# indianajohn/akaze-rust

Hardware: AMD Instinct MI355X
Metric: Mpix/s through extract_features (4 oct x 4 sub) (higher is better)
Workload: dtype f32

## Files before the change

akaze-rust_amd/csrc/akz_extract.hpp:

```cpp
#pragma once
#include "akz_ctx.hpp"
#include "akz_frames.hpp"

struct akz_result {
    akz_ctx* ctx = nullptr;
    akz_config cfg;
    uint32_t w = 0, h = 0, n = 0, flags = 0;
    uint64_t big_px = 0;
    std::vector<LevelPlan> plan;
    void* slab = nullptr;
    size_t slab_bytes = 0;
    float* planes[kMaxLevels][10];
    double* d_k = nullptr;
    std::vector<double> k_host;
    std::vector<std::vector<akz_keypoint>> kps;
    std::vector<uint8_t> rows64;
    uint8_t* d_desc64 = nullptr;
    size_t desc_block_bytes = 0;
    std::vector<uint64_t> desc_off;
    std::vector<uint64_t> n_extrema;
};

struct MaskSpec {
    const uint8_t* d = nullptr;
    uint64_t row_pitch = 0, frame_stride = 0;
};

struct ResultDeleter {
    void operator()(akz_result* r) const;
};
struct akz_job {
    std::unique_ptr<akz_result, ResultDeleter> r;
    int slot = -1;
    uint32_t cap = 0;
    Event nms_done;
    uint64_t seq = 0;
    double t_begin_ms = 0.0;
    std::shared_ptr<Finisher> fin;
    bool finished = false;
    int rc = 0;
    akz_result* out = nullptr;
    std::string err;
    std::shared_ptr<std::atomic<int>> in_hand;
    bool alone_at_begin = true;
    hipStream_t done_stream = nullptr;
    MaskSpec mask;
    ~akz_job() {
        if (in_hand) --*in_hand;
    }
};

inline uint64_t shape_key(uint32_t w, uint32_t h, uint32_t n) { return ((uint64_t)w << 40) | ((uint64_t)h << 16) | n; }
inline uint32_t like_last_job(uint32_t last, uint32_t pad, uint32_t cap) { return std::min<uint32_t>(cap, last + last / 4 + pad); }

constexpr uint32_t kSelHdrWords = 16;
enum SelHdr : uint32_t {
    kSelHdrKeypoints = 0,
    kSelHdrExtrema = 1,
    kSelHdrFallback = 2,
    kSelHdrRounds = 3,
    kSelHdrTicks = 4,
    kSelHdrTotal = 8,
    kSelHdrFlags = 9,
    kSelHdrContrast = 10,
};
inline const uint32_t* sel_hdr(const akz_ctx* c, uint32_t img) { return (const uint32_t*)c->pin[PIN_SEL_HDR].p + (size_t)img * kSelHdrWords; }

inline LevelTable level_table(const akz_result* r) {
    LevelTable tab;
    std::memset(&tab, 0, sizeof(tab));
    for (size_t l = 0; l < r->plan.size(); ++l)
        tab.lv[l] = {r->planes[l][AKZ_LT], r->planes[l][AKZ_LX], r->planes[l][AKZ_LY], r->plan[l].w, r->plan[l].h, (uint64_t)r->plan[l].w * r->plan[l].h};
    return tab;
}
inline KpParam kp_param(float x, float y, float size, uint32_t octave, uint32_t level, uint32_t img) {
    const float ratio = (float)(1u << octave);
    return KpParam{x / ratio, y / ratio, std::round(0.5f * size / ratio), level, img, {0, 0, 0}};
}

inline size_t align_up(size_t v, size_t a) { return (v + a - 1) / a * a; }
AKZ_LOCAL int slab_acquire(akz_ctx* c, size_t bytes, void** p, size_t* got);
AKZ_LOCAL void slab_release(akz_ctx* c, void* p, size_t bytes);
AKZ_LOCAL void result_delete(akz_result* r);
AKZ_LOCAL void job_release(akz_job* j);
AKZ_LOCAL void job_wait(akz_job* j);
AKZ_LOCAL void job_destroy(akz_job* j);
struct JobOpening {
    std::unique_ptr<akz_job> job;
    int slot = -1;
    bool drain_side = false;
    bool laid_out = false;
    ~JobOpening();
    akz_job* keep(uint32_t cap);
};
AKZ_LOCAL int free_slot(const akz_ctx* c, int want = -1);
AKZ_LOCAL int job_open(akz_ctx* c, const char* who, int want_slot, uint32_t w, uint32_t h, uint32_t n, uint32_t flags, const akz_config& cfg,
                       JobOpening& o);
AKZ_LOCAL int job_layout(JobOpening& o, const std::vector<std::pair<uint32_t, int>>& wanted);
AKZ_LOCAL int place_lanes(akz_ctx* c);
template <typename T>
AKZ_LOCAL int extract_begin(akz_ctx* c, const T* d_imgs, uint32_t w, uint32_t h, uint32_t n, const akz_config* cfgp, uint32_t flags, akz_job** out,
                            int want_slot = -1, hipEvent_t input_ready = nullptr, bool sync_call = false, const MaskSpec* mask = nullptr);
AKZ_LOCAL int mask_enqueue(akz_ctx* c, hipStream_t s, const akz_result* r, const MaskSpec& m, int slot, uint32_t cap, uint32_t* d_count);
AKZ_LOCAL int extract_finish_body(akz_job* jobp, akz_result** out);
AKZ_LOCAL int extract_begin_frames(akz_ctx* c, const uint8_t* d_src, const FrameSpec& fs, uint32_t n, const akz_config* cfg, uint32_t flags, akz_job** out,
                                   const MaskSpec* mask = nullptr);
AKZ_LOCAL int extract_frames(akz_ctx* c, const uint8_t* d_src, const FrameSpec& fs, uint32_t n, const akz_config* cfg, uint32_t flags, akz_result** out,
                             const MaskSpec* mask = nullptr);
AKZ_LOCAL int frames_enqueue(akz_ctx* c, hipStream_t s, const uint8_t* d_src, const FrameSpec& fs, uint32_t n, uint8_t* d_luma);
```

akaze-rust_amd/csrc/akz_extract_finish.cpp:

```cpp
#include "akz_extract.hpp"

int device_libm_mode(akz_ctx* c) {
    if (c->settings.dbg_device_libm == 0) return 0;
    static std::mutex m;
    static int mode = -1;
    std::lock_guard<std::mutex> lk(m);
    if (mode >= 0) return mode;
    mode = 0;
#if defined(__x86_64__) && defined(__GLIBC__)
    __builtin_cpu_init();
    const bool fma = __builtin_cpu_supports("fma") && __builtin_cpu_supports("avx2");
    if (!fma && __builtin_cpu_supports("fma4")) return mode;
    constexpr size_t kN = 1u << 21;
    std::vector<float> a(kN), b(kN);
    uint64_t st = 0x9E3779B97F4A7C15ull;
    auto next = [&]() {
        uint64_t z = (st += 0x9E3779B97F4A7C15ull);
        z = (z ^ (z >> 30)) * 0xBF58476D1CE4E5B9ull;
        z = (z ^ (z >> 27)) * 0x94D049BB133111EBull;
        return z ^ (z >> 31);
    };
    const float special[] = {0.0f, -0.0f, 1.0f, -1.0f, INFINITY, -INFINITY, NAN, 0x1p-126f, -0x1p-126f, 0x1p-149f, 0x1.fffffep127f, 0x1p-12f,
                             0x1.921fb6p-1f, 0x1.921fb6p0f, 0x1.921fb6p1f, -0x1.921fb6p1f, 0.4375f, 0.6875f, 1.1875f, 2.4375f, 0x1p25f, 0x1p-29f,
                             119.99f, 120.0f, 1e10f};
// ... 16 lines not shown
            std::memcpy(&a[i], &u, 4);
            std::memcpy(&b[i], &v, 4);
        }
    }
    DevBuf d_a, d_b, d_o;
    std::vector<float> got(3 * kN);
    const bool ok_dev = d_a.acquire(kN * 4, false) == hipSuccess && d_b.acquire(kN * 4, false) == hipSuccess &&
                        d_o.acquire(3 * kN * 4, false) == hipSuccess &&
                        hipMemcpy(d_a.p, a.data(), kN * 4, hipMemcpyHostToDevice) == hipSuccess &&
                        hipMemcpy(d_b.p, b.data(), kN * 4, hipMemcpyHostToDevice) == hipSuccess;
    if (ok_dev) {
        launch::libm_eval(nullptr, (const float*)d_a.p, (const float*)d_b.p, (float*)d_o.p, kN, fma, nullptr);
        const bool ran = hipGetLastError() == hipSuccess && hipMemcpy(got.data(), d_o.p, 3 * kN * 4, hipMemcpyDeviceToHost) == hipSuccess;
        std::atomic<uint64_t> bad{ran ? 0u : 1u};
        if (ran) {
            const size_t pieces = 64;
            c->pool().run(pieces, [&](size_t p) {
                uint64_t mine = 0;
                auto bits = [](float f) { uint32_t u; std::memcpy(&u, &f, 4); return u; };
                auto same = [&](float x, float y) { return bits(x) == bits(y) || (x != x && y != y); };
                for (size_t i = kN * p / pieces; i < kN * (p + 1) / pieces; ++i) {
                    mine += !same(got[3 * i], atan2f(a[i], b[i]));
                    if (std::fabs(a[i]) < 119.9f) mine += !same(got[3 * i + 1], cosf(a[i])) + !same(got[3 * i + 2], sinf(a[i]));
                }
                bad += mine;
            });
        }
        if (bad.load() == 0) mode = fma ? 1 : 2;
    }
    (void)hipGetLastError();
#endif
    return mode;
}


namespace {
constexpr size_t kRelRow = (size_t)(kRel1 + kRel2) * sizeof(uint16_t);

struct FinishState {
    explicit FinishState(akz_job* j) : job(j), r(j->r.get()), c(r->ctx), n(r->n), s(c->stream), cap(j->cap), d_count((uint32_t*)c->count_slot[j->slot].p) {}
    akz_job* job;
    akz_result* r;
    akz_ctx* c;
    uint32_t n;
    hipStream_t s;
    uint32_t cap;
    uint32_t* d_count;
    bool waited_for = false, want_rel = false, want_dev = false, device_sort = false;
    uint64_t shape = 0;
    bool sorted = false, dev_sel = false;
    uint32_t mldb_spec = 0;
    int libm_dev = 0;
    bool dev_angles_ok = true;
    bool mirrored = false;
    uint16_t* d_rel = nullptr;
    uint32_t* d_rel_flags = nullptr;
    uint32_t *d_sel_hdr = nullptr, *d_sel_total = nullptr;
    std::vector<float> lsize, lratio;
    LevelTable tab;
    unsigned long long wmask = 0;
    uint32_t nwin = 0;
    const Candidate* hc = nullptr;
    uint32_t total_c = 0, spec_kp = 0;
    uint64_t total_kp = 0;
    double t_counts = 0.0;
    std::vector<std::vector<Candidate>> cands;
    std::vector<std::pair<const Candidate*, size_t>> span;
    std::vector<std::vector<HostKeypoint>> hk;
    bool host_rows() const { return !(r->flags & AKZ_NO_HOST_DESCRIPTORS); }
    const Candidate* d_unsorted() const { return (const Candidate*)(job->mask.d ? c->cand_mask_slot : c->cand_slot)[job->slot].p; }
    uint32_t mask_redone = 0;
};

int grow_pinned_keep(akz_ctx* c, DevBuf& buf, size_t keep_bytes, size_t want_bytes) {
    std::vector<uint8_t> keep;
    if (keep_bytes) keep.assign((const uint8_t*)buf.p, (const uint8_t*)buf.p + keep_bytes);
    AKZ_TRY(ensure_pinned(c, buf, want_bytes));
    if (keep_bytes) std::memcpy(buf.p, keep.data(), keep_bytes);
    return AKZ_OK;
}
int fetch_rest(akz_ctx* c, hipStream_t s, DevBuf& buf, const void* d_src, size_t elem, size_t have, size_t total) {
    AKZ_TRY(grow_pinned_keep(c, buf, have * elem, total * elem));
    AKZ_HIP_TRY(hipMemcpyAsync((uint8_t*)buf.p + have * elem, (const uint8_t*)d_src + have * elem, (total - have) * elem, hipMemcpyDeviceToHost, s));
    return AKZ_OK;
}
void rows_to_result(akz_ctx* c, akz_result* r, uint64_t total_kp) {
    const uint8_t* rows = (const uint8_t*)c->pin[PIN_ROWS].p;
    r->rows64.resize(total_kp * 64);
    const size_t kRowChunk = 8192;
    c->pool().run((total_kp + kRowChunk - 1) / kRowChunk, [&](size_t j) {
        const size_t b = j * kRowChunk * 64, e = std::min<size_t>(total_kp * 64, b + kRowChunk * 64);
        std::memcpy(r->rows64.data() + b, rows + b, e - b);
    });
}
int hold_behind_next_fed(akz_ctx* c, const akz_job* job, hipStream_t s) {
    const akz_result* r = job->r.get();
    if ((uint64_t)r->w * r->h * r->n >= r->big_px && c->begin_seq.load() > job->seq)
        AKZ_HIP_TRY(hipStreamWaitEvent(s, c->fed_ev[(job->seq + 1) % akz_ctx::kFedRing], 0));
    return AKZ_OK;
}

int choose_paths(FinishState& f) {
    akz_ctx* c = f.c;
    akz_job* job = f.job;
    akz_result* r = f.r;
    const uint32_t n = f.n;
    f.s = c->stream;
    const bool in_order = !c->is_lane && job->done_stream && job->alone_at_begin && job->in_hand && job->in_hand->load() == 1 && (c->settings.sched[SCHED_FINISH_FORM] & 2) == 0;
    if (in_order) {
        f.s = job->done_stream;
    } else if (!(c->is_lane && job->fin)) {
        AKZ_TRY(ensure_aux(c));
        f.s = c->aux;
    }
    AKZ_HIP_TRY(hipStreamWaitEvent(f.s, job->nms_done, 0));
    f.waited_for = !c->is_lane && job->alone_at_begin;
    f.want_rel = c->settings.dbg_select == 1 || (c->settings.dbg_select < 0 && (c->pool().size() < gates::kFewHostThreads || (uint64_t)r->w * r->h * n < r->big_px ||
                                                                (uint64_t)r->w * r->h >= gates::kSelectDevicePx || n < gates::kFewHostThreads || f.waited_for));
    f.shape = shape_key(r->w, r->h, n);
    bool skip_dev = false;
    if (c->sel_skip.load() > 0 && c->sel_skip_shape.load() == f.shape) {
        skip_dev = true;
        --c->sel_skip;
    }
    f.want_dev = c->settings.dbg_select == 2 || (c->settings.dbg_select < 0 && f.want_rel && !skip_dev && (c->pool().size() < gates::kFewHostThreads || f.waited_for));
    if (!f.want_dev) {
        c->sel_last_rounds = 0;
        c->sel_last_fallback = 0;
    }
    f.device_sort = c->settings.dbg_host_sort == 0 || (c->settings.dbg_host_sort < 0 && (c->pool().size() < gates::kFewHostThreads || f.want_rel)) || f.want_dev;
    selection_level_constants(r->plan, r->cfg, f.lsize, f.lratio);
    f.tab = level_table(r);
    orientation_windows(&f.wmask, &f.nwin);
    return AKZ_OK;
}

int enqueue_device_descriptors(FinishState& f) {
    akz_ctx* c = f.c;
    akz_result* r = f.r;
    f.libm_dev = device_libm_mode(c);
    if (!f.libm_dev) return AKZ_OK;
    void* blk = nullptr;
    AKZ_TRY(slab_acquire(c, (size_t)f.cap * 64, &blk, &r->desc_block_bytes));
    r->d_desc64 = (uint8_t*)blk;
    f.mldb_spec = like_last_job(c->last_total_kp.load(), 256u, f.cap);
    launch::MldbMirror mir{};
    if ((c->settings.sched[SCHED_FINISH_FORM] & 1) == 0) {
        AKZ_TRY(ensure_pinned(c, c->pin[PIN_SEL_HDR], (size_t)f.n * 64));
        AKZ_TRY(ensure_pinned(c, c->pin[PIN_LIST], (size_t)f.mldb_spec * sizeof(SelKpHost)));
        if (f.host_rows()) AKZ_TRY(ensure_pinned(c, c->pin[PIN_ROWS], (size_t)f.mldb_spec * 64));
        mir = launch::MldbMirror{c->pin[PIN_LIST].p, f.d_sel_hdr, c->pin[PIN_SEL_HDR].p, f.n * 64u, f.host_rows() ? (uint8_t*)c->pin[PIN_ROWS].p : nullptr};
        f.mirrored = true;
    }
    launch::mldb_counted(f.s, f.tab, (const KpParam*)c->kp_in.p, f.d_sel_total, 0, f.mldb_spec, &((SelKpHost*)c->sel_recs.p)->sums, 2,
                         f.libm_dev == 1, nullptr, (uint32_t)r->cfg.descriptor_channels, r->d_desc64, f.mirrored ? &mir : nullptr);
    AKZ_HIP_TRY(hipGetLastError());
    return AKZ_OK;
}

int enqueue_device_side(FinishState& f) {
    if (!f.device_sort) return AKZ_OK;
    akz_ctx* c = f.c;
    akz_result* r = f.r;
    hipStream_t s = f.s;
    const uint32_t n = f.n, cap = f.cap, L = (uint32_t)r->plan.size();
    const uint64_t max_px = (uint64_t)r->plan[0].w * r->plan[0].h;
    Candidate* d_sorted = nullptr;
    AKZ_TRY(ensure(c, c->cand_sorted, (size_t)cap * sizeof(Candidate)));
    d_sorted = (Candidate*)c->cand_sorted.p;
    void* selp = nullptr;
    if (f.want_dev) {
        AKZ_TRY(ensure(c, c->sel_scratch, launch::select_device_bytes(cap, n)));
        selp = c->sel_scratch.p;
    }
    std::vector<uint32_t> lw(L), lh(L);
    for (size_t l = 0; l < L; ++l) {
        lw[l] = r->plan[l].w;
        lh[l] = r->plan[l].h;
    }
    uint32_t* d_zero = selp ? launch::select_device_revcnt(selp, cap, n) : nullptr;
    const bool want_lists = f.want_rel || f.want_dev;
    if (want_lists) AKZ_TRY(ensure(c, c->rel_scratch, launch::candidate_relations_bytes(cap, lh.data(), L, n)));
    const bool rows_sort = n == 1 && (f.waited_for || c->settings.dbg_select == 2) &&
                           launch::sort_candidates_rows(s, f.d_unsorted(), cap, f.d_count, lw.data(), lh.data(), L, d_sorted, d_zero,
                                                        want_lists ? c->rel_scratch.p : nullptr);
    f.sorted = rows_sort;
    bool buckets_sort = false;
    if (!f.sorted) {
        AKZ_TRY(ensure(c, c->bucket_scratch, launch::sort_candidates_buckets_scratch(cap)));
        buckets_sort = launch::sort_candidates_buckets(s, f.d_unsorted(), cap, f.d_count, lw.data(), lh.data(), L, n, c->bucket_scratch.p,
                                                       &c->bucket_scratch.known, d_sorted, d_zero, want_lists ? c->rel_scratch.p : nullptr);
        f.sorted = buckets_sort;
    }
    if (!f.sorted) {
        AKZ_TRY(ensure(c, c->sort_scratch, launch::sort_candidates_scratch(cap, max_px, L, n)));
        f.sorted = launch::sort_candidates_device(s, f.d_unsorted(), cap, f.d_count, max_px, L, n, c->sort_scratch.p, d_sorted, d_zero);
    }
    if (f.sorted)
        kernel_row_count(c, kStageSort, rows_sort ? AKZ_KR_SORT_ROWS : (buckets_sort ? AKZ_KR_SORT_BUCKETS : AKZ_KR_SORT_RADIX), r->plan[0].w,
                         r->plan[0].h, n, rows_sort ? 1 : (buckets_sort ? 4 : 3), cap);
    AKZ_HIP_TRY(hipGetLastError());
    if (!f.sorted || !want_lists) return AKZ_OK;
    launch::candidate_relations(s, d_sorted, cap, f.d_count, f.lsize.data(), f.lratio.data(), lw.data(), lh.data(), L, n, c->rel_scratch.p,
                                &f.d_rel, &f.d_rel_flags, selp, rows_sort || buckets_sort);
    AKZ_HIP_TRY(hipGetLastError());
    if (!f.want_dev) return AKZ_OK;
    AKZ_TRY(ensure(c, c->sel_recs, (size_t)cap * sizeof(SelKpHost)));
    AKZ_TRY(ensure(c, c->kp_in, (size_t)cap * sizeof(KpParam)));
    launch::select_device(s, d_sorted, cap, f.d_count, f.lsize.data(), f.lratio.data(), lw.data(), lh.data(), L, n, c->rel_scratch.p, selp,
                          r->d_k, c->sel_recs.p, (KpParam*)c->kp_in.p, &f.d_sel_hdr, &f.d_sel_total);
    AKZ_TRY(hold_behind_next_fed(c, f.job, s));
    launch::orientation_counted(s, f.tab, (const KpParam*)c->kp_in.p, f.d_sel_total, cap, f.wmask, f.nwin, &((SelKpHost*)c->sel_recs.p)->sums, 2);
    AKZ_HIP_TRY(hipGetLastError());
    f.dev_sel = true;
    return enqueue_device_descriptors(f);
}

int adopt_device_selection(FinishState& f) {
    akz_ctx* c = f.c;
    akz_result* r = f.r;
    hipStream_t s = f.s;
    uint32_t max_rounds = 0, fallen = 0;
    for (uint32_t img = 0; img < f.n; ++img) {
        const uint32_t* hdr = sel_hdr(c, img);
        if (hdr[kSelHdrFallback] != 0) {
            f.dev_sel = false;
            ++fallen;
            fallen |= hdr[kSelHdrFallback] << 16;
        }
        f.total_kp += hdr[kSelHdrKeypoints];
        max_rounds = std::max(max_rounds, hdr[kSelHdrRounds]);
    }
    for (int k = 0; k < 4; ++k) c->sel_last_ticks[k] = sel_hdr(c, 0)[kSelHdrTicks + k];
    c->sel_last_rounds = max_rounds;
    c->sel_last_fallback = fallen;
    if (fallen) {
        c->sel_skip = 8;
        c->sel_skip_shape = f.shape;
    }
    if (f.dev_sel && f.libm_dev && f.total_kp > f.mldb_spec) {
        launch::mldb_counted(s, f.tab, (const KpParam*)c->kp_in.p, f.d_sel_total, f.mldb_spec, (uint32_t)f.total_kp, &((SelKpHost*)c->sel_recs.p)->sums, 2,
                             f.libm_dev == 1, nullptr, (uint32_t)r->cfg.descriptor_channels, r->d_desc64);
        AKZ_HIP_TRY(hipGetLastError());
    }
    if (f.dev_sel && f.total_kp > f.spec_kp) {
        AKZ_TRY(fetch_rest(c, s, c->pin[PIN_LIST], c->sel_recs.p, sizeof(SelKpHost), f.spec_kp, f.total_kp));
        if (f.libm_dev && f.host_rows()) AKZ_TRY(fetch_rest(c, s, c->pin[PIN_ROWS], r->d_desc64, 64, f.spec_kp, f.total_kp));
        AKZ_HIP_TRY(hipStreamSynchronize(s));
    }
    if (!f.dev_sel) f.total_kp = 0;
    return AKZ_OK;
}

int fetch_candidates(FinishState& f) {
    akz_ctx* c = f.c;
    akz_job* job = f.job;
    akz_result* r = f.r;
    hipStream_t s = f.s;
    const uint32_t n = f.n;
    const std::vector<LevelPlan>& plan = r->plan;
    for (int attempt = 0;; ++attempt) {
        const Candidate* d_list = f.sorted ? (const Candidate*)c->cand_sorted.p : f.d_unsorted();
        AKZ_TRY(ensure_pinned(c, c->pin[PIN_COUNT_SUMS], 256));
        uint32_t* total_p = (uint32_t*)c->pin[PIN_COUNT_SUMS].p;
        const bool dev_fetch = attempt == 0 && f.dev_sel;
        const bool masked = job->mask.d != nullptr;
        if (!dev_fetch) AKZ_HIP_TRY(hipMemcpyAsync(total_p, f.d_count, (masked ? 2 : 1) * sizeof(uint32_t), hipMemcpyDeviceToHost, s));
        else if (masked) AKZ_HIP_TRY(hipMemcpyAsync(total_p + 1, f.d_count + 1, sizeof(uint32_t), hipMemcpyDeviceToHost, s));
        uint32_t spec = 0;
        if (dev_fetch) {
            f.spec_kp = f.libm_dev ? f.mldb_spec : like_last_job(c->last_total_kp.load(), 256u, f.cap);
            if (!f.mirrored) {
                AKZ_TRY(ensure_pinned(c, c->pin[PIN_SEL_HDR], (size_t)n * 64));
                AKZ_HIP_TRY(hipMemcpyAsync(c->pin[PIN_SEL_HDR].p, f.d_sel_hdr, (size_t)n * 64, hipMemcpyDeviceToHost, s));
                AKZ_TRY(ensure_pinned(c, c->pin[PIN_LIST], (size_t)f.spec_kp * sizeof(SelKpHost)));
                AKZ_HIP_TRY(hipMemcpyAsync(c->pin[PIN_LIST].p, c->sel_recs.p, (size_t)f.spec_kp * sizeof(SelKpHost), hipMemcpyDeviceToHost, s));
                if (f.libm_dev && f.host_rows()) {
                    AKZ_TRY(ensure_pinned(c, c->pin[PIN_ROWS], (size_t)f.spec_kp * 64));
                    AKZ_HIP_TRY(hipMemcpyAsync(c->pin[PIN_ROWS].p, r->d_desc64, (size_t)f.spec_kp * 64, hipMemcpyDeviceToHost, s));
                }
            }
            AKZ_TRY(ensure_pinned(c, c->pin[PIN_CONTRAST], (size_t)n * sizeof(double)));
            AKZ_TRY(ensure_pinned(c, c->pin[PIN_REL_FLAGS], (size_t)n * sizeof(uint32_t)));
        } else if (attempt == 0) {
            spec = like_last_job(c->last_total_cands.load(), 64u, f.cap);
            if ((size_t)spec * sizeof(Candidate) > (1u << 20)) spec = 0;
            AKZ_TRY(ensure_pinned(c, c->pin[PIN_CONTRAST], (size_t)n * sizeof(double)));
            AKZ_HIP_TRY(hipMemcpyAsync(c->pin[PIN_CONTRAST].p, r->d_k, (size_t)n * sizeof(double), hipMemcpyDeviceToHost, s));
            if (spec) {
                AKZ_TRY(ensure_pinned(c, c->pin[PIN_LIST], (size_t)spec * sizeof(Candidate)));
                AKZ_HIP_TRY(hipMemcpyAsync(c->pin[PIN_LIST].p, d_list, (size_t)spec * sizeof(Candidate), hipMemcpyDeviceToHost, s));
                if (f.d_rel) {
                    AKZ_TRY(ensure_pinned(c, c->pin[PIN_REL], (size_t)spec * kRelRow));
                    AKZ_HIP_TRY(hipMemcpyAsync(c->pin[PIN_REL].p, f.d_rel, (size_t)spec * kRelRow, hipMemcpyDeviceToHost, s));
                }
            }
            if (f.d_rel) {
                AKZ_TRY(ensure_pinned(c, c->pin[PIN_REL_FLAGS], (size_t)n * sizeof(uint32_t)));
                AKZ_HIP_TRY(hipMemcpyAsync(c->pin[PIN_REL_FLAGS].p, f.d_rel_flags, (size_t)n * sizeof(uint32_t), hipMemcpyDeviceToHost, s));
            }
        }
        AKZ_HIP_TRY(hipStreamSynchronize(s));
        f.t_counts = now_ms();
        if (dev_fetch) {
            *total_p = sel_hdr(c, 0)[kSelHdrTotal];
            for (uint32_t img = 0; img < n; ++img) {
                ((uint32_t*)c->pin[PIN_REL_FLAGS].p)[img] = sel_hdr(c, img)[kSelHdrFlags];
                std::memcpy((double*)c->pin[PIN_CONTRAST].p + img, &sel_hdr(c, img)[kSelHdrContrast], sizeof(double));
            }
        }
        f.total_c = *total_p;
        if (attempt == 0) r->k_host.assign((const double*)c->pin[PIN_CONTRAST].p, (const double*)c->pin[PIN_CONTRAST].p + n);
        const uint32_t unfiltered = masked ? std::max(total_p[1], f.total_c) : f.total_c;
        c->last_total_cands = unfiltered;
        c->last_cand_shape = f.shape;
        c->cand_cap_hint = std::max(c->cand_cap_hint.load(), (uint32_t)((uint64_t)unfiltered * 5 / 4 / n) + 64u);
        if (masked) {
            static std::atomic<uint64_t> stamp{0};
            c->mask_last[0] = unfiltered, c->mask_last[1] = f.total_c, c->mask_last[2] = f.mask_redone;
            c->mask_stamp = ++stamp;
        }
        if (f.total_c > f.cap) {
            if (attempt >= 3) {
                set_error("NMS candidate buffer overflow");
                return AKZ_ERR_OVERFLOW;
            }
            f.cap = f.total_c + f.total_c / 8;
            f.sorted = false;
            f.dev_sel = false;
            f.d_rel = nullptr;
            AKZ_HIP_TRY(hipStreamSynchronize(c->stream));
            AKZ_TRY(ensure(c, c->cand_slot[job->slot], (size_t)f.cap * sizeof(Candidate)));
            if (masked) AKZ_TRY(ensure(c, c->cand_mask_slot[job->slot], (size_t)f.cap * sizeof(Candidate)));
            AKZ_HIP_TRY(hipMemsetAsync(f.d_count, 0, sizeof(uint32_t), s));
            for (size_t l = 0; l < plan.size(); ++l)
                launch::nms(s, r->planes[l][AKZ_LDET], plan[l].w, plan[l].h, n, (uint64_t)plan[l].w * plan[l].h, (uint32_t)l,
                            (float)r->cfg.detector_threshold, border_margin(plan[l], r->cfg), (Candidate*)c->cand_slot[job->slot].p, f.cap, f.d_count);
            AKZ_HIP_TRY(hipGetLastError());
            if (masked) {
                AKZ_TRY(mask_enqueue(c, s, r, job->mask, job->slot, f.cap, f.d_count));
                ++f.mask_redone;
            }
            continue;
        }
        if (f.dev_sel) {
            AKZ_TRY(adopt_device_selection(f));
            if (f.dev_sel) return AKZ_OK;
        }
        const uint32_t have = std::min(spec, f.total_c);
        if (f.total_c > have) {
            AKZ_TRY(fetch_rest(c, s, c->pin[PIN_LIST], d_list, sizeof(Candidate), have, f.total_c));
            if (f.d_rel) AKZ_TRY(fetch_rest(c, s, c->pin[PIN_REL], f.d_rel, kRelRow, have, f.total_c));
            AKZ_HIP_TRY(hipStreamSynchronize(s));
        }
        AKZ_TRY(ensure_pinned(c, c->pin[PIN_LIST], sizeof(Candidate)));
        f.hc = (const Candidate*)c->pin[PIN_LIST].p;
        return AKZ_OK;
    }
}

void candidates_per_image(FinishState& f) {
    akz_ctx* c = f.c;
    const uint32_t n = f.n, total_c = f.total_c;
    const Candidate* hc = f.hc;
    f.span.assign(n, {nullptr, 0});
    if (f.dev_sel) {
    } else if (f.sorted) {
        size_t at = 0;
        for (uint32_t img = 0; img < n; ++img) {
            const Candidate* b = hc + at;
            const Candidate* e = std::partition_point(b, hc + total_c, [&](const Candidate& x) { return x.img <= img; });
            f.span[img] = {b, (size_t)(e - b)};
            at += (size_t)(e - b);
        }
    } else {
        f.cands.resize(n);
        const unsigned slices = (unsigned)std::min<size_t>((size_t)total_c / 16384 + 1, (size_t)c->pool().size());
        std::vector<std::vector<uint32_t>> at(slices, std::vector<uint32_t>(n, 0));
        auto slice_range = [&](unsigned t, size_t* b, size_t* e) {
            *b = (size_t)total_c * t / slices;
            *e = (size_t)total_c * (t + 1) / slices;
        };
        auto run_slices = [&](auto&& fn) { c->pool().run(slices, [&](size_t t) { fn((unsigned)t); }); };
        run_slices([&](unsigned t) {
            size_t b, e;
            slice_range(t, &b, &e);
            for (size_t i = b; i < e; ++i)
                if (hc[i].img < n) at[t][hc[i].img]++;
        });
        for (uint32_t img = 0; img < n; ++img) {
            uint32_t run = 0;
            for (unsigned t = 0; t < slices; ++t) {
                const uint32_t cnt = at[t][img];
                at[t][img] = run;
                run += cnt;
            }
            f.cands[img].resize(run);
        }
        run_slices([&](unsigned t) {
            size_t b, e;
            slice_range(t, &b, &e);
            for (size_t i = b; i < e; ++i)
                if (hc[i].img < n) f.cands[hc[i].img][at[t][hc[i].img]++] = hc[i];
        });
    }
    c->sel_last_mode = f.dev_sel ? 2 : (f.d_rel && f.sorted ? 1 : 0);
    c->slot_busy[f.job->slot] = false;
    f.job->slot = -1;
    if (c->settings.profiling) c->prof.ms[AKZ_ST_NMS] += now_ms() - f.t_counts;
}

void select_keypoints_stage(FinishState& f) {
    akz_ctx* c = f.c;
    akz_result* r = f.r;
    const uint32_t n = f.n;
    const std::vector<LevelPlan>& plan = r->plan;
    const double t_host0 = now_ms();
    f.hk.resize(n);
    r->n_extrema.assign(n, 0);
    r->desc_off.assign(n + 1, 0);
    if (f.dev_sel) {
        const SelKpHost* recs = (const SelKpHost*)c->pin[PIN_LIST].p;
        std::vector<uint64_t> first(n + 1, 0);
        for (uint32_t img = 0; img < n; ++img) first[img + 1] = first[img] + sel_hdr(c, img)[kSelHdrKeypoints];
        c->pool().run(n, [&](size_t img) {
            r->n_extrema[img] = sel_hdr(c, (uint32_t)img)[kSelHdrExtrema];
            f.hk[img].resize(sel_hdr(c, (uint32_t)img)[kSelHdrKeypoints]);
            for (size_t i = 0; i < f.hk[img].size(); ++i) {
                const sel::KpRec& q = recs[first[img] + i].rec;
                HostKeypoint& k = f.hk[img][i];
                k.x = q.x; k.y = q.y; k.response = q.response;
                k.size = f.lsize[q.level];
                k.octave = plan[q.level].octave;
                k.class_id = q.level;
                k.angle = 0.0f;
                if (f.libm_dev) std::memcpy(&k.angle, &recs[first[img] + i].sums.angle_bits, 4);
                k.lx = k.ly = 0;
                k.xp = k.xm = k.yp = k.ym = 0.0f;
            }
        });
        if (f.libm_dev)
            for (uint32_t img = 0; img < n && f.dev_angles_ok; ++img)
                for (const HostKeypoint& k : f.hk[img])
                    if (!(std::fabs(k.angle) < 119.9f)) {
                        f.dev_angles_ok = false;
                        break;
                    }
        c->last_total_kp = (uint32_t)f.total_kp;
    } else {
        c->pool().run(n, [&](size_t img) {
            if (!f.sorted) {
                sort_candidates(f.cands[img], plan);
                f.span[img] = {f.cands[img].data(), f.cands[img].size()};
            }
            if (f.d_rel && f.sorted && (((const uint32_t*)c->pin[PIN_REL_FLAGS].p)[img] & 1u) == 0)
                select_keypoints_rel(f.span[img].first, f.span[img].second, (const uint16_t*)c->pin[PIN_REL].p + (size_t)(f.span[img].first - f.hc) * (kRel1 + kRel2),
                                     kRel1, kRel2, plan, r->cfg, f.hk[img], &r->n_extrema[img]);
            else
                select_keypoints(f.span[img].first, f.span[img].second, plan, r->cfg, f.hk[img], &r->n_extrema[img]);
        });
    }
    f.total_kp = 0;
    for (uint32_t img = 0; img < n; ++img) {
        r->desc_off[img] = f.total_kp;
        f.total_kp += f.hk[img].size();
    }
    r->desc_off[n] = f.total_kp;
    if (c->settings.profiling) c->prof.ms[AKZ_ST_HOST_KP] += now_ms() - t_host0;
}

int describe_with_host_libm(FinishState& f, const KpParam* params) {
    akz_ctx* c = f.c;
    akz_result* r = f.r;
    hipStream_t s = f.s;
    const uint64_t total_kp = f.total_kp;
    const double t_or0 = now_ms();
    KpParam* d_kp = (KpParam*)c->kp_in.p;
    OrientOut* oo = nullptr;
    size_t oo_stride = 1;
    AKZ_TRY(ensure(c, c->cosi, total_kp * 2 * sizeof(float)));
    if (f.dev_sel) {
        oo = &((SelKpHost*)c->pin[PIN_LIST].p)->sums;
        oo_stride = 2;
    } else {
        AKZ_TRY(ensure(c, c->kp_in, total_kp * sizeof(KpParam)));
        AKZ_TRY(ensure(c, c->kp_out, total_kp * sizeof(OrientOut)));
        AKZ_TRY(ensure_pinned(c, c->pin[PIN_COUNT_SUMS], total_kp * std::max(sizeof(OrientOut), 2 * sizeof(float))));
        d_kp = (KpParam*)c->kp_in.p;
        OrientOut* d_oo = (OrientOut*)c->kp_out.p;
        AKZ_HIP_TRY(hipMemcpyAsync(d_kp, params, total_kp * sizeof(KpParam), hipMemcpyHostToDevice, s));
        AKZ_TRY(hold_behind_next_fed(c, f.job, s));
        launch::orientation(s, f.tab, d_kp, (uint32_t)total_kp, f.wmask, f.nwin, d_oo);
        AKZ_HIP_TRY(hipGetLastError());
        oo = (OrientOut*)c->pin[PIN_COUNT_SUMS].p;
        AKZ_HIP_TRY(hipMemcpyAsync(oo, d_oo, total_kp * sizeof(OrientOut), hipMemcpyDeviceToHost, s));
        AKZ_HIP_TRY(hipStreamSynchronize(s));
    }
    AKZ_TRY(ensure_pinned(c, c->pin[PIN_COSI], total_kp * 2 * sizeof(float)));
    float* cosi = (float*)c->pin[PIN_COSI].p;
    std::vector<float> angles(total_kp);
    const size_t kAngleChunk = 4096;
    c->pool().run((total_kp + kAngleChunk - 1) / kAngleChunk, [&](size_t j) {
        const size_t b = j * kAngleChunk, e = std::min<size_t>(total_kp, b + kAngleChunk);
        for (size_t g = b; g < e; ++g) {
            const OrientOut& og = oo[g * oo_stride];
            const float ang = og.found ? atan2f(og.sum_y, og.sum_x) : 0.0f;
            angles[g] = ang;
            cosi[2 * g] = cosf(ang);
            cosi[2 * g + 1] = sinf(ang);
        }
    });
    c->pool().run(f.n, [&](size_t img) {
        for (size_t i = 0; i < f.hk[img].size(); ++i) f.hk[img][i].angle = angles[r->desc_off[img] + i];
    });
    AKZ_HIP_TRY(hipMemcpyAsync(c->cosi.p, cosi, total_kp * 2 * sizeof(float), hipMemcpyHostToDevice, s));
    const double t_ml0 = now_ms();
    if (c->settings.profiling) c->prof.ms[AKZ_ST_ORIENT] += t_ml0 - t_or0;
    if (r->d_desc64 && r->desc_block_bytes < total_kp * 64) {
        slab_release(c, r->d_desc64, r->desc_block_bytes);
        r->d_desc64 = nullptr;
    }
    if (!r->d_desc64) {
        void* blk = nullptr;
        AKZ_TRY(slab_acquire(c, total_kp * 64, &blk, &r->desc_block_bytes));
        r->d_desc64 = (uint8_t*)blk;
    }
    launch::mldb(s, f.tab, d_kp, (const float*)c->cosi.p, (uint32_t)total_kp, (uint32_t)r->cfg.descriptor_channels, r->d_desc64);
    AKZ_HIP_TRY(hipGetLastError());
    if (f.host_rows()) {
        AKZ_TRY(ensure_pinned(c, c->pin[PIN_ROWS], total_kp * 64));
        AKZ_HIP_TRY(hipMemcpyAsync(c->pin[PIN_ROWS].p, r->d_desc64, total_kp * 64, hipMemcpyDeviceToHost, s));
        AKZ_HIP_TRY(hipStreamSynchronize(s));
        rows_to_result(c, r, total_kp);
    } else {
        AKZ_HIP_TRY(hipStreamSynchronize(s));
    }
    if (c->settings.profiling) c->prof.ms[AKZ_ST_MLDB] += now_ms() - t_ml0;
    return AKZ_OK;
}

int describe(FinishState& f) {
    akz_ctx* c = f.c;
    akz_result* r = f.r;
    KpParam* params = nullptr;
    if (!f.dev_sel) {
        AKZ_TRY(ensure_pinned(c, c->pin[PIN_PARAMS], std::max<size_t>(1, f.total_kp) * sizeof(KpParam)));
        params = (KpParam*)c->pin[PIN_PARAMS].p;
        c->pool().run(f.n, [&](size_t img) {
            for (size_t i = 0; i < f.hk[img].size(); ++i) {
                const HostKeypoint& k = f.hk[img][i];
                params[r->desc_off[img] + i] = kp_param(k.x, k.y, k.size, k.octave, k.class_id, (uint32_t)img);
            }
        });
    }
    r->kps.assign(f.n, {});
    const bool dev_desc = f.dev_sel && f.libm_dev != 0 && f.dev_angles_ok;
    c->libm_last = dev_desc ? f.libm_dev : 0;
    if (f.total_kp && dev_desc) {
        const double t_ml0 = now_ms();
        if (f.host_rows()) rows_to_result(c, r, f.total_kp);
        if (c->settings.profiling) c->prof.ms[AKZ_ST_MLDB] += now_ms() - t_ml0;
    } else if (f.total_kp) {
        AKZ_TRY(describe_with_host_libm(f, params));
    }
    return AKZ_OK;
}

void publish(FinishState& f) {
    akz_ctx* c = f.c;
    akz_result* r = f.r;
    c->pool().run(f.n, [&](size_t img) {
        r->kps[img].resize(f.hk[img].size());
        for (size_t i = 0; i < f.hk[img].size(); ++i) {
            const HostKeypoint& k = f.hk[img][i];
            r->kps[img][i] = akz_keypoint{k.x, k.y, k.response, k.size, k.octave, k.class_id, k.angle, 0};
        }
    });
    if (c->settings.profiling) {
        resolve_spans(c);
        c->prof.ms[AKZ_ST_TOTAL] += now_ms() - f.job->t_begin_ms;
        c->prof.calls += 1;
        c->prof.pixels += (uint64_t)r->w * r->h * f.n;
    }
    ev_put(c, std::move(f.job->nms_done));
}
}

int extract_finish_body(akz_job* jobp, akz_result** out) {
    *out = nullptr;
    std::unique_ptr<akz_job, void (*)(akz_job*)> job(jobp, job_release);
    AKZ_TRY(bind(job->r->ctx, false));
    FinishState f(jobp);
    AKZ_TRY(choose_paths(f));
    AKZ_TRY(enqueue_device_side(f));
    AKZ_TRY(fetch_candidates(f));
    candidates_per_image(f);
    select_keypoints_stage(f);
    AKZ_TRY(describe(f));
    publish(f);
    *out = job->r.release();
    (void)job.release();
    return AKZ_OK;
}
```

akaze-rust_amd/csrc/akz_internal.hpp:

```cpp
#pragma once
#include <hip/hip_runtime.h>

#include <cstdint>
#include <functional>
#include <string>
#include <vector>

#include "../../include/akaze_hip.h"
#include "../../include/akaze_hip_debug.h"

namespace akz {

void set_error(const std::string& msg);
unsigned host_cpu_share();

using TrialsOnDevice = std::function<int(const float*, const float*, const float*, const float*, uint32_t, const uint32_t*, uint32_t,
                                         float, float, float*, int32_t*)>;
int remove_outliers_impl(const akz_keypoint* keypoints_0, uint64_t n0, const akz_keypoint* keypoints_1, uint64_t n1,
                         const akz_match* matches, uint64_t n_matches, uint64_t num_trials, float epsilon_model,
                         float epsilon_inlier, akz_match* out, uint64_t* n_out, const TrialsOnDevice& trials_on_device);

#define AKZ_HIP_TRY(expr)                                                                          \
    do {                                                                                           \
        hipError_t _e = (expr);                                                                    \
        if (_e != hipSuccess) {                                                                    \
            ::akz::set_error(std::string(#expr) + " failed: " + hipGetErrorString(_e));            \
            return AKZ_ERR_HIP;                                                                    \
        }                                                                                          \
    } while (0)

struct DefaultSource {
    uint64_t s0 = 42, s1 = 69;
    uint64_t next() {
        uint64_t x = s0;
        const uint64_t y = s1;
        s0 = y;
        x ^= x << 23;
        x ^= x >> 17;
        x ^= y ^ (y >> 26);
        s1 = x;
        return x + y;
    }
};
DefaultSource& default_source();
template <int K, class T>
void draw_samples(DefaultSource& src, uint64_t n_matches, uint64_t trials, T* out);

int refuse_bad_matches(const char* name, const akz_keypoint* keypoints_0, uint64_t n0, const akz_keypoint* keypoints_1, uint64_t n1,
                       const akz_match* matches, uint64_t n_matches, const akz_match* out, const uint64_t* n_out);
struct MatchPoints {
    std::vector<float> v;
    const float *x0, *y0, *x1, *y1;
    MatchPoints(const akz_keypoint* keypoints_0, const akz_keypoint* keypoints_1, const akz_match* matches, uint64_t n) : v((size_t)n * 4) {
        float* p = v.data();
        x0 = p; y0 = p + n; x1 = p + 2 * n; y1 = p + 3 * n;
        for (uint64_t i = 0; i < n; ++i) {
            p[i] = keypoints_0[matches[i].index_0].x; p[n + i] = keypoints_0[matches[i].index_0].y;
            p[2 * n + i] = keypoints_1[matches[i].index_1].x; p[3 * n + i] = keypoints_1[matches[i].index_1].y;
        }
    }
};


#define AKZ_TRY(expr)            \
    do {                         \
        int _s = (expr);         \
        if (_s != AKZ_OK) return _s; \
    } while (0)

int match_sets_at(akz_ctx* c, const uint8_t* d_q, uint64_t n0, const uint8_t* d_rows, const uint64_t* set_first,
                  const uint64_t* set_rows, uint64_t n_sets, uint64_t distance_threshold, double lowes_ratio, akz_match* d_out,
                  uint64_t* d_n_out, akz_match* d_out_cols, uint64_t* d_n_cols, int side = 0);
hipStream_t match_side_stream(akz_ctx* c);

int place_streams_beside(akz_ctx* c, hipStream_t* slots, int n_slots, int* still_shared);
enum { kPlaceQueue = 1, kPlacePipe = 2, kPlaceAmbiguous = 4 };
int placement_verdict(float spin_pair_ms, float tiny_pair_ms, float tiny_alone_ms, float spin_ms);

struct LevelPlan {
    double etime = 0, esigma = 0;
    uint32_t octave = 0, sublevel = 0, sigma_size = 0;
    uint32_t w = 0, h = 0;
    uint32_t det_sigma = 0;
    std::vector<double> tau;
};
int config_validate(const akz_config& c);
int fed_tau_by_process_time(double T, int M, double tau_max, bool reordering, std::vector<double>& tau);
std::vector<float> gaussian_kernel(float sigma, size_t kernel_size);
size_t gaussian_kernel_size(float sigma);
void scharr_kernels(uint32_t scale, std::vector<float>& main_axis, std::vector<float>& off_axis);
int build_plan(uint32_t w, uint32_t h, const akz_config& cfg, std::vector<LevelPlan>& plan);

constexpr int kMaxTaps = 13;
struct Taps {
    int n = 0;
    int hw = 0;
    int off[kMaxTaps] = {0};
    float wgt[kMaxTaps] = {0};
};
int taps_from_dense(const float* k, uint32_t ntaps, Taps& t);
Taps taps_scharr_main(uint32_t scale);
Taps taps_scharr_off(uint32_t scale);

struct Candidate {
    uint32_t level;
    uint32_t idx;
    float v, xp, xm, yp, ym;
    uint32_t img;
};
struct KpParam {
    float xf, yf;
    float scale;
    uint32_t level;
    uint32_t img;
    uint32_t _pad[3];
};
struct OrientOut {
    float sum_x, sum_y;
    uint32_t found;
    uint32_t angle_bits;
};
struct MatchRec {
    uint32_t min_d, second_d, min_j, _pad;
};
struct LevelPtrs {
    const float* lt;
    const float* lx;
    const float* ly;
    uint32_t w, h;
    uint64_t stride;
};
constexpr int kMaxLevels = 64;
constexpr int kRel1 = 12, kRel2 = 6;
struct LevelTable {
    LevelPtrs lv[kMaxLevels];
};

namespace launch {
void filter_h_f32(hipStream_t s, const float* in, float* out, uint32_t w, uint32_t h, uint32_t n, const Taps& t);
void filter_h_u8(hipStream_t s, const uint8_t* in, float* out, uint32_t w, uint32_t h, uint32_t n, const Taps& t);
void filter_v_f32(hipStream_t s, const float* in, float* out, uint32_t w, uint32_t h, uint32_t n, const Taps& t);
void delay(hipStream_t s, uint32_t microseconds);
void half_size(hipStream_t s, const float* in, float* out, uint32_t w, uint32_t h, uint32_t n);
void pm_g2(hipStream_t s, const float* lx, const float* ly, float* out, uint32_t w, uint32_t h, uint32_t n,
           const double* d_k, uint32_t k_scale_pow);
void flow(hipStream_t s, const float* lsmooth, float* lflow, uint32_t w, uint32_t h, uint32_t n, const double* d_k,
          uint32_t k_scale_pow);
void fed_step(hipStream_t s, const float* lt_in, const float* lflow, float* lt_out, float* lstep, uint32_t w,
              uint32_t h, uint32_t n, float half_tau);
struct FedNextPrep {
    float* lsmooth;
    float* lflow;
    const float* g3;
    const double* d_k;
    uint32_t k_pow;
};
bool fed_epilogue_supported(uint32_t w, uint32_t h, uint32_t n_steps);
void fed_fused(hipStream_t s, const float* lt_in, const float* lflow, float* lt_out, float* lstep, uint32_t w, uint32_t h,
               uint32_t n, const float* half_taus, uint32_t n_steps, const FedNextPrep* next = nullptr);
uint64_t fed_deep_workgroups(uint32_t w, uint32_t h, uint32_t n);
void contrast_max(hipStream_t s, const float* blurred, uint32_t w, uint32_t h, uint32_t n,
                  unsigned long long* d_hmax_bits);
void contrast_hist(hipStream_t s, const float* blurred, uint32_t w, uint32_t h, uint32_t n,
                   const unsigned long long* d_hmax_bits, uint32_t nbins, uint32_t* d_hist);
void contrast_final(hipStream_t s, const unsigned long long* d_hmax_bits, const uint32_t* d_hist, uint32_t nbins,
                    double percentile, uint32_t n, double* d_k);
bool blur_fused_supported(uint32_t ntaps);
void blur_fused_f32(hipStream_t s, const float* in, float* out, uint32_t w, uint32_t h, uint32_t n, const float* k,
                    uint32_t ntaps);
void blur_fused_u8(hipStream_t s, const uint8_t* in, float* out, uint32_t w, uint32_t h, uint32_t n, const float* k,
                   uint32_t ntaps);
void prep_fused(hipStream_t s, const float* prev, bool half, float* lt_out, float* lsmooth, float* lflow, uint32_t w,
                uint32_t h, uint32_t pw, uint32_t ph, uint32_t n, const float* g3, const double* d_k, uint32_t k_pow);
bool detector_fused_supported(uint32_t sigma);
void detector_fused(hipStream_t s, const float* lsmooth, uint32_t sigma, float* lx, float* ly, float* lxx, float* lyy,
                    float* lxy, float* ldet_out, uint32_t w, uint32_t h, uint32_t n);
bool detector_tiled_fused_supported(uint32_t sigma);
struct DetLevelDesc {
    const float* lsmooth;
    float *lx, *ly, *lxx, *lyy, *lxy, *ldet;
    uint32_t w, h, level;
    float border_m;
};
uint32_t detector_tiled_set_max();
void detector_tiled_set(hipStream_t s, uint32_t sigma, const DetLevelDesc* levels, uint32_t nlevels, uint32_t n, float thr,
                        Candidate* d_cand, uint32_t cap, uint32_t* d_count);
void detector_tiled_fused(hipStream_t s, const float* lsmooth, uint32_t sigma, float* lx, float* ly, float* lxx,
                          float* lyy, float* lxy, float* ldet_out, uint32_t w, uint32_t h, uint32_t n, uint32_t level,
                          float thr, float border_m, Candidate* d_cand, uint32_t cap, uint32_t* d_count);
bool blur5_stream_supported(uint32_t w, uint32_t h, uint32_t ntaps, bool is_u8);
void blur5_stream_u8(hipStream_t s, const uint8_t* in, float* out, uint32_t w, uint32_t h, uint32_t n, const float* k);
void blur5_stream_f32(hipStream_t s, const float* in, float* out, uint32_t w, uint32_t h, uint32_t n, const float* k);
uint32_t march_band_rows(int kind, uint32_t w, uint32_t h, uint32_t n, int S, int32_t* cs_ce, uint32_t cap);
bool blur5_march_supported(uint32_t w, uint32_t h, uint32_t ntaps);
void blur5_march_u8(hipStream_t s, const uint8_t* in, float* out, uint32_t w, uint32_t h, uint32_t n, const float* k);
void blur5_march_f32(hipStream_t s, const float* in, float* out, uint32_t w, uint32_t h, uint32_t n, const float* k);
bool contrast_march_supported(uint32_t w, uint32_t h, uint32_t ntaps, uint32_t nbins);
void contrast_march(hipStream_t s, const float* in, uint32_t w, uint32_t h, uint32_t n, const float* g3,
                    unsigned long long* d_hmax_bits, uint32_t nbins, uint32_t* d_hist, double* d_thr);
void contrast_thresholds(hipStream_t s, const unsigned long long* d_hmax_bits, uint32_t nbins, uint32_t n, double* d_thr);
bool contrast_stream_supported(uint32_t w, uint32_t h, uint32_t ntaps, uint32_t nbins);
void contrast_stream(hipStream_t s, const float* in, uint32_t w, uint32_t h, uint32_t n, const float* g3,
                     unsigned long long* d_hmax_bits, uint32_t nbins, uint32_t* d_hist, double* d_thr);
bool prep_stream_supported(uint32_t w, uint32_t h);
void prep_stream(hipStream_t s, const float* prev, bool half, float* lt_out, float* lsmooth, float* lflow, uint32_t w,
                 uint32_t h, uint32_t pw, uint32_t ph, uint32_t n, const float* g3, const double* d_k, uint32_t k_pow);
bool detector_march_supported(uint32_t sigma, uint32_t w, uint32_t h, float border_m, bool nms);
void detector_march(hipStream_t s, const float* lsmooth, uint32_t sigma, float* lx, float* ly, float* lxx, float* lyy,
                    float* lxy, float* ldet_out, uint32_t w, uint32_t h, uint32_t n, uint32_t level, float thr,
                    float border_m, Candidate* d_cand, uint32_t cap, uint32_t* d_count);
uint32_t detector_march_set_max();
void detector_march_set(hipStream_t s, uint32_t sigma, const DetLevelDesc* levels, uint32_t nlevels, uint32_t n, float thr,
                        Candidate* d_cand, uint32_t cap, uint32_t* d_count);
void detector_set_waves(int waves);
uint32_t detector_set_cells(int S, const uint32_t* w, const uint32_t* h, uint32_t nlv, uint32_t n, int32_t* cells, uint32_t cap,
                            int32_t* grids);
bool head_fused_supported(uint32_t w, uint32_t h, uint32_t ntaps0, uint32_t ntaps1);
void head_fused_u8(hipStream_t s, const uint8_t* in, float* lt0, float* blurred, float* gx, float* gy, uint32_t w, uint32_t h, uint32_t n,
                   const float* k5, const float* g3, unsigned long long* d_smax_bits, uint32_t* d_zero_word = nullptr);
void head_fused_f32(hipStream_t s, const float* in, float* lt0, float* blurred, float* gx, float* gy, uint32_t w, uint32_t h, uint32_t n,
                    const float* k5, const float* g3, unsigned long long* d_smax_bits, uint32_t* d_zero_word = nullptr);
void contrast_hist_final(hipStream_t s, const float* gx, const float* gy, uint32_t w, uint32_t h, uint32_t n, unsigned long long* d_smax_bits,
                         uint32_t nbins, uint32_t* d_hist, uint32_t* d_done, double percentile, double* d_k);
void flow_from_pair(hipStream_t s, const float* gx, const float* gy, float* lflow, uint32_t w, uint32_t h, uint32_t n, const double* d_k,
                    uint32_t k_pow);
void march_min_band_rows(int detector, int level);
bool level_march_supported(uint32_t w, uint32_t h);
bool level_march_half_supported(uint32_t w, uint32_t h, uint32_t pw, uint32_t ph, uint32_t n_steps);
void level_march(hipStream_t s, const float* prev, float* lsmooth, float* lflow, float* lt_out, float* lstep, uint32_t w,
                 uint32_t h, uint32_t n, const float* g3, const double* d_k, uint32_t k_pow, const float* half_taus,
                 uint32_t n_steps, uint32_t pw = 0, uint32_t ph = 0);
struct ResidentLevel {
    float *lt, *lsmooth, *lflow, *lstep;
    uint32_t w, h;
    bool half;
    uint32_t n_tau;
    const float* half_tau;
    uint32_t k_pow;
};
constexpr int kResidentMaxLevels = 10;
constexpr int kResidentMaxSteps = 448;
bool octave_resident_supported(uint32_t w, uint32_t h);
void octave_resident(hipStream_t s, const float* prev, uint32_t pw, uint32_t ph, uint32_t n, const ResidentLevel* levels,
                     uint32_t n_levels, const float* g3, const double* d_k);
bool detector_nms_fused_supported(uint32_t sigma);
void detector_nms_fused(hipStream_t s, const float* lsmooth, uint32_t sigma, float* lx, float* ly, float* lxx,
                        float* lyy, float* lxy, float* ldet_out, uint32_t w, uint32_t h, uint32_t n, uint32_t level,
                        float thr, float border_m, Candidate* d_cand, uint32_t cap, uint32_t* d_count);
void rcp_f64_to_f32(hipStream_t s, const double* x, float* out, uint64_t n);
void accumulate(hipStream_t s, float* a, const float* b, uint64_t count);
void ldet(hipStream_t s, const float* lxx, const float* lyy, const float* lxy, float* out, uint64_t count,
          float sigma_quat);
size_t sort_candidates_scratch(uint32_t cap, uint64_t max_px, uint32_t n_levels, uint32_t n_images);
uint32_t sort_small_capacity();
size_t sort_candidates_buckets_scratch(uint32_t cap);
size_t sort_candidates_buckets_counters();
bool sort_candidates_buckets(hipStream_t s, const Candidate* d_cand, uint32_t cap, const uint32_t* d_count, const uint32_t* level_w,
                             const uint32_t* level_h, uint32_t n_levels, uint32_t n_images, void* scratch, size_t* counters_zero,
                             Candidate* d_sorted, uint32_t* d_zero, void* rel_scratch);
bool sort_candidates_rows(hipStream_t s, const Candidate* d_cand, uint32_t cap, const uint32_t* d_count, const uint32_t* level_w,
                          const uint32_t* level_h, uint32_t n_levels, Candidate* d_sorted, uint32_t* d_zero, void* rel_scratch);
bool sort_candidates_device(hipStream_t s, const Candidate* d_cand, uint32_t cap, const uint32_t* d_count, uint64_t max_px,
                            uint32_t n_levels, uint32_t n_images, void* scratch, Candidate* d_sorted, uint32_t* d_zero = nullptr);
size_t candidate_relations_bytes(uint32_t cap, const uint32_t* level_h, uint32_t n_levels, uint32_t n_images);
void candidate_relations(hipStream_t s, const Candidate* d_sorted, uint32_t cap, const uint32_t* d_count, const float* size, const float* ratio,
                         const uint32_t* level_w, const uint32_t* level_h, uint32_t n_levels, uint32_t n_images, void* scratch,
                         uint16_t** d_rel_out, uint32_t** d_flags_out, void* sel_scratch = nullptr, bool tables_ready = false);
size_t select_device_bytes(uint32_t cap, uint32_t n_images);
uint32_t* select_device_revcnt(void* sel_scratch, uint32_t cap, uint32_t n_images);
void select_device(hipStream_t s, const Candidate* d_sorted, uint32_t cap, const uint32_t* d_count, const float* size, const float* ratio,
                   const uint32_t* level_w, const uint32_t* level_h, uint32_t n_levels, uint32_t n_images, const void* rel_scratch,
                   void* sel_scratch, const double* d_k, void* d_recs, KpParam* d_pars, uint32_t** d_hdr_out, uint32_t** d_total_out);
void nms(hipStream_t s, const float* ldet, uint32_t w, uint32_t h, uint32_t n, uint64_t img_stride, uint32_t level,
         float thr, float border_m, Candidate* d_cand, uint32_t cap, uint32_t* d_count);
void mask_candidates(hipStream_t s, const Candidate* d_in, Candidate* d_out, uint32_t cap, uint32_t* d_cnt, const uint8_t* d_mask,
                     uint64_t row_pitch, uint64_t frame_stride, const uint32_t* level_w, const uint32_t* level_h,
                     const uint32_t* level_octave, uint32_t n_levels, uint32_t n_images);
void orientation(hipStream_t s, const LevelTable& lt, const KpParam* d_kp, uint32_t nkp,
                 unsigned long long window_mask, uint32_t n_windows, OrientOut* d_out);
void orientation_counted(hipStream_t s, const LevelTable& lt, const KpParam* d_kp, const uint32_t* d_nkp, uint32_t max_kp,
                         unsigned long long window_mask, uint32_t n_windows, OrientOut* d_out, uint32_t out_stride);
void mldb(hipStream_t s, const LevelTable& lt, const KpParam* d_kp, const float* d_cosi, uint32_t nkp,
          uint32_t channels, uint8_t* d_desc64);
struct MldbMirror {
    void* host_recs;
    const void* d_hdr;
    void* host_hdr;
    uint32_t hdr_bytes;
    uint8_t* host_desc;
};
void mldb_counted(hipStream_t s, const LevelTable& lt, const KpParam* d_kp, const uint32_t* d_nkp, uint32_t first, uint32_t last, OrientOut* d_sums,
                  uint32_t sums_stride, bool libm_fma, uint32_t* d_flag, uint32_t channels, uint8_t* d_desc64, const MldbMirror* mirror = nullptr);
void libm_eval(hipStream_t s, const float* a, const float* b, float* out3, uint64_t n, bool fma, uint32_t* d_flag);
uint32_t match_num_chunks(uint32_t n0, uint32_t n1);
void match(hipStream_t s, const uint8_t* d0, uint32_t n0, const uint8_t* d1, uint32_t n1, uint32_t threshold,
           bool rows_le_61, uint32_t chunks, MatchRec* d_rec);
uint32_t match_mfma_rows(uint32_t n, bool queries);
uint32_t match_mfma_chunks(uint32_t n0, uint32_t n1, uint32_t forced = 0);
uint32_t match_mfma_multi_chunks(uint32_t n0, uint32_t n_sets, uint32_t avg_tiles, uint32_t forced = 0);
void unpack_bits(hipStream_t s, const uint8_t* d, uint32_t n, uint32_t n_pad, bool query, uint8_t* out8, uint32_t* pop,
                 uint32_t* bound, uint32_t threshold, uint32_t n_bound, const uint32_t* d_tiles, bool fp4 = false);
void ransac_trials(hipStream_t s, const float* d_pts, uint32_t n_matches, const uint32_t* d_samples, uint32_t trials, float epsilon_model,
                   float epsilon_inlier, float* d_models, int32_t* d_inliers);
struct PairJobHost {
    uint64_t raw_off, kp0_off, kp1_off, trial_off, keep_off, n_trials;
    uint32_t cnt_idx, pad;
};
static_assert(sizeof(PairJobHost) == 56, "the device reads 56-byte pair records");
enum class RansacModel { Fundamental, Homography, FundamentalNormalised };
void pair_points(hipStream_t s, const PairJobHost* d_pairs, uint32_t n_pairs, const void* d_raw, const uint64_t* d_raw_cnt,
                 const float* d_kx, const float* d_ky, float* d_pts, uint64_t pts_stride);
void pairs_trials(hipStream_t s, RansacModel model, const PairJobHost* d_pairs, const uint32_t* d_trials, uint64_t first_trial,
                  uint32_t n_trials, const uint64_t* d_raw_cnt, const float* d_pts, uint64_t pts_stride, float epsilon_model,
                  float epsilon_inlier, float* d_models, int32_t* d_inliers);
void pairs_pick_filter(hipStream_t s, RansacModel model, const PairJobHost* d_pairs, uint32_t n_pairs, const void* d_raw,
                       const uint64_t* d_raw_cnt, const float* d_pts, uint64_t pts_stride, const float* d_models, const int32_t* d_inliers,
                       float epsilon_inlier, void* d_keep, uint64_t* d_keep_cnt, float* d_h, int32_t* d_found);
void model_refit(hipStream_t s, RansacModel model, const PairJobHost* d_pairs, uint32_t n_pairs, const void* d_raw, const uint64_t* d_raw_cnt,
                      const float* d_pts, uint64_t pts_stride, float epsilon_model, float epsilon_inlier, uint32_t max_iterations,
                      void* d_keep, uint64_t* d_keep_cnt, float* d_h, const int32_t* d_found, uint32_t* d_iterations);
void pairs_pose(hipStream_t s, const PairJobHost* d_pairs, uint32_t n_pairs, const akz_camera* d_cameras,
                const float* d_kx, const float* d_ky, const float* d_f, const int32_t* d_found, void* d_keep, uint64_t* d_keep_cnt,
                akz_pose* d_poses, float* d_points);
void seeded_round(hipStream_t s, RansacModel model, const PairJobHost* d_pairs, uint32_t n_pairs, const uint32_t* d_done, uint64_t k1,
                  uint64_t stream_base, uint32_t round, uint32_t max_trials, const uint64_t* d_raw_cnt, const float* d_pts, uint64_t pts_stride,
                  float epsilon_model, float epsilon_inlier, float* d_ring_mdl, int32_t* d_ring_inl);
void seeded_update(hipStream_t s, uint32_t n_pairs, uint32_t round, uint32_t max_trials, const uint32_t* d_need, uint32_t need_stride,
                   uint32_t need_index, const float* d_ring_mdl, const int32_t* d_ring_inl, uint32_t* d_done, int32_t* d_best_inl, float* d_best_mdl,
                   uint32_t* d_trials_run, uint32_t* d_running);
void unpack_pair(hipStream_t s, const uint8_t* dq, uint32_t nq, uint32_t q_pad, uint8_t* outq, uint32_t* popq, uint32_t* bound, uint32_t threshold,
                 const uint8_t* dt, uint32_t nt, uint32_t t_pad, uint8_t* outt, uint32_t* popt, bool fp4);
uint32_t match_mfma_tile_rows();
uint32_t match_mfma_query_block();
struct MatchChunkHost {
    uint32_t t_begin, t_end, row0, n_rows, bound_off, record;
};
void match_mfma_multi(hipStream_t s, const uint8_t* q8, const uint32_t* qpop, uint32_t n0, const uint8_t* t8,
                      const void* d_table, uint32_t n_chunks, uint32_t threshold, uint32_t* bound, MatchRec* d_out, bool fp4 = false);
void match_mfma(hipStream_t s, const uint8_t* q8, const uint32_t* qpop, uint32_t n0, const uint8_t* t8, uint32_t n1,
                uint32_t threshold, uint32_t* bound, uint32_t chunks, MatchRec* d_rec, bool fp4 = false);
struct MatchColSetHost {
    uint32_t row0, rows, out0;
};
uint32_t match_cols_seed_rows(uint32_t n0);
void match_cols_seed(hipStream_t s, const uint8_t* q4, uint32_t n0, const uint8_t* t4, uint32_t t_rows, uint32_t threshold,
                     uint32_t* d_bound, MatchRec* d_seed, unsigned long long* cbest, uint32_t* csecond);
void match_fp4_multi_mutual(hipStream_t s, const uint8_t* q4, uint32_t n0, const uint8_t* t4, const void* d_table, uint32_t n_chunks,
                            uint32_t threshold, uint32_t* bound, MatchRec* d_out, unsigned long long* cbest, uint32_t* csecond);
void match_compact_cols(hipStream_t s, const unsigned long long* cbest, const uint32_t* csecond, const void* d_sets, uint32_t n_sets,
                        uint32_t threshold, double ratio2, akz_match* d_out, unsigned long long* d_n_out);
void match_compact_sets(hipStream_t s, const MatchRec* d_rec, uint32_t n0, uint32_t n_sets, uint32_t chunks, uint32_t threshold,
                        double ratio2, akz_match* d_out, unsigned long long* d_n_out);
void match_compact(hipStream_t s, const MatchRec* d_rec, uint32_t n0, uint32_t chunks, uint32_t threshold, double ratio2,
                   akz_match* d_out, unsigned long long* d_n_out);
void match_merge(hipStream_t s, const MatchRec* d_part, uint32_t n0, uint32_t chunks, uint32_t threshold, MatchRec* d_out);
size_t match_merge_compact_state_bytes(uint32_t n0);
void match_merge_compact(hipStream_t s, const MatchRec* d_part, uint32_t n0, uint32_t chunks, uint32_t threshold, double ratio2,
                         akz_match* d_out, unsigned long long* d_n_out, void* d_state, uint32_t epoch);
struct GuidedPairHost {
    uint64_t rec_off;
    uint32_t q_row0, n0, t_row0, n1, wg0, chunks, chunk_rows, model;
};
uint32_t match_guided_block();
void match_guided(hipStream_t s, int kind, const uint8_t* d_rows, const float* d_kx, const float* d_ky, const GuidedPairHost* d_tab,
                  uint32_t n_tab, uint32_t n_workgroups, const float* d_models, const int32_t* d_found, float radius,
                  uint32_t threshold, MatchRec* d_rec);
struct CrossJobHost {
    uint64_t fwd_off, rev_off;
    uint32_t fwd_cnt_idx, rev_cnt_idx, fwd_cap, rev_cap;
};
static_assert(sizeof(CrossJobHost) == 32, "the device reads 32-byte cross records");
void pairs_cross_filter(hipStream_t s, const CrossJobHost* d_tab, uint32_t n_pairs, akz_match* d_fwd, uint64_t* d_fwd_cnt,
                        const akz_match* d_rev, const uint64_t* d_rev_cnt);
void pair_cross_filter(hipStream_t s, const CrossJobHost& job, akz_match* d_fwd, uint64_t* d_fwd_cnt, const akz_match* d_rev,
                       const uint64_t* d_rev_cnt);
struct BankSeg {
    const uint8_t* src_rows;
    uint64_t n_rows, dst_row0;
};
static_assert(sizeof(BankSeg) == 24, "the device reads 24-byte segment records");
constexpr uint64_t kBankMaxRows = 0x7fffffffull * 64;
void bank_gather(hipStream_t s, const BankSeg* d_tab, uint32_t n_seg, uint64_t total_rows, uint32_t desc_bytes, uint8_t* d_dst);
uint32_t knn_list_len(uint32_t k);
uint32_t knn_chunks(uint32_t n0, uint32_t n1, uint32_t forced = 0);
size_t knn_part_bytes(uint32_t n0, uint32_t chunks, uint32_t k);
bool knn(hipStream_t s, const uint8_t* q4, uint32_t n0, const uint8_t* t4, uint32_t n1, uint32_t threshold, uint32_t chunks, uint32_t k,
         uint32_t* d_part, akz_match* d_out, uint32_t* d_counts);
struct BudgetSet {
    uint32_t base, n, keep, out_off;
};
struct BudgetBlock {
    uint32_t set, q0, t0, t1;
};
static_assert(sizeof(BudgetSet) == 16 && sizeof(BudgetBlock) == 16, "the device reads 16-byte budget records");
uint32_t budget_query_tile();
uint32_t budget_train_tile();
void budget(hipStream_t s, bool spread, float robust, const float* d_x, const float* d_y, const float* d_r, uint32_t total,
            const BudgetSet* d_sets, uint32_t n_sets, const BudgetBlock* d_blocks, uint32_t n_blocks, float* d_radius2, uint32_t* d_rank,
            uint32_t* d_idx);
}

struct HostKeypoint {
    float x, y, response, size;
    uint32_t octave, class_id;
    float angle;
    uint32_t lx, ly;
    float xp, xm, yp, ym;
};
void sort_candidates(std::vector<Candidate>& cands, const std::vector<LevelPlan>& plan);
void select_keypoints(const Candidate* cands_sorted, size_t n_cands, const std::vector<LevelPlan>& plan,
                      const akz_config& cfg, std::vector<HostKeypoint>& out, uint64_t* n_extrema);
void select_keypoints_rel(const Candidate* cands_sorted, size_t n_cands, const uint16_t* rel, int k1, int k2, const std::vector<LevelPlan>& plan,
                          const akz_config& cfg, std::vector<HostKeypoint>& out, uint64_t* n_extrema);
void selection_level_constants(const std::vector<LevelPlan>& plan, const akz_config& cfg, std::vector<float>& size, std::vector<float>& ratio);
void orientation_windows(unsigned long long* mask, uint32_t* n_windows);
float border_margin(const LevelPlan& lv, const akz_config& cfg);

}

#if defined(__HIPCC__)
namespace akz {
typedef float akz_f4a __attribute__((ext_vector_type(4)));
typedef float akz_f4u __attribute__((ext_vector_type(4), aligned(4)));
__device__ __forceinline__ void plane_store(float* p, float v) { *p = v; }
__device__ __forceinline__ void plane_store4(float* p, float a, float b, float c, float d) {
    const akz_f4a t = {a, b, c, d};
    *reinterpret_cast<akz_f4a*>(p) = t;
}
__device__ __forceinline__ void plane_store4u(float* p, akz_f4a t) {
    *reinterpret_cast<akz_f4u*>(p) = t;
}
}
#endif
```

akaze-rust_amd/csrc/akz_kernels.hip:

```cpp
#include <hip/hip_runtime.h>

#include <algorithm>
#include <cstdlib>

#include "akz_internal.hpp"
#include "akz_pm_g2.hpp"
#include "akz_libm.hpp"
#include "akz_prep_passes.hpp"

namespace akz {
namespace {

constexpr int BX = 64, BY = 4;

__device__ __forceinline__ int clampi(int v, int lo, int hi) { return v < lo ? lo : (v > hi ? hi : v); }

__device__ __forceinline__ float px(const float* p, long i) { return p[i]; }
__device__ __forceinline__ float px(const uint8_t* p, long i) { return ((float)p[i] * 1.0f) / 255.0f; }

template <typename T>
__global__ void k_filter_h(const T* __restrict__ in, float* __restrict__ out, int w, int h, Taps t) {
    const int x = blockIdx.x * BX + threadIdx.x, y = blockIdx.y * BY + threadIdx.y;
    if (x >= w || y >= h) return;
    const size_t base = (size_t)blockIdx.z * (size_t)w * (size_t)h;
// ... 469 lines not shown
            const float4 a = *reinterpret_cast<const float4*>(GX + i0), b = *reinterpret_cast<const float4*>(GY + i0);
            ax[0] = a.x; ax[1] = a.y; ax[2] = a.z; ax[3] = a.w;
            ay[0] = b.x; ay[1] = b.y; ay[2] = b.z; ay[3] = b.w;
        } else {
#pragma unroll
            for (int e = 0; e < 4; ++e) {
                ax[e] = i0 + e < px ? GX[i0 + e] : 0.0f;
                ay[e] = i0 + e < px ? GY[i0 + e] : 0.0f;
            }
        }
        int y = (int)(i0 / (size_t)w), x = (int)(i0 - (size_t)y * w);
#pragma unroll
        for (int e = 0; e < 4; ++e) {
            if (x >= 1 && x < w - 1 && y >= 1 && y < h - 1) {
                const double dx = (double)ax[e], dy = (double)ay[e];
                const double g = sqrt(dx * dx + dy * dy);
                if (g != 0.0) {
                    const double f = floor((double)nbins * (g / hmax));
                    const unsigned b = f >= (double)nbins ? nbins - 1u : (f > 0.0 ? (unsigned)f : 0u);
                    atomicAdd(&mine[b], 1u);
                }
            }
            if (++x == w) {
                x = 0;
                ++y;
            }
        }
    }
    __syncthreads();
    unsigned* hist = d_hist + (size_t)img * nbins;
    for (unsigned b = tid; b < nbins; b += NTH) {
        unsigned v = 0;
        for (unsigned c = 0; c < copies; ++c) v += s_hist[c * nbins + b];
        if (v) {
            const unsigned before = atomicAdd(&hist[b], v);
            asm volatile("" ::"v"(before));
        }
    }
    __builtin_amdgcn_fence(__ATOMIC_RELEASE, "workgroup");
    __builtin_amdgcn_s_waitcnt(0);
    __syncthreads();
    if (tid == 0) s_last = atomicAdd(&d_done[img], 1u) == gridDim.x - 1u ? 1u : 0u;
    __syncthreads();
    if (!s_last) return;
    for (unsigned b = tid; b < nbins; b += NTH) {
        s_hist[b] = __hip_atomic_load(&hist[b], __ATOMIC_RELAXED, __HIP_MEMORY_SCOPE_AGENT);
        hist[b] = 0u;
    }
    __syncthreads();
    if (tid != 0) return;
    unsigned long long num_points = 0;
    for (unsigned b = 0; b < nbins; ++b) num_points += s_hist[b];
    const unsigned long long threshold = sat_usize((double)num_points * percentile);
    unsigned long long k = 0, num_elements = 0;
    while (num_elements < threshold && k < nbins) {
        num_elements += s_hist[k];
        k += 1;
    }
    d_k[img] = num_elements >= threshold ? hmax * (double)k / (double)nbins : 0.03;
    d_smax_bits[img] = 0ull;
    d_done[img] = 0u;
}
__global__ void __launch_bounds__(256)
k_flow_pair(const float* __restrict__ gxp, const float* __restrict__ gyp, float* __restrict__ lflow, size_t px, const double* __restrict__ d_k,
            unsigned k_pow) {
    const unsigned img = blockIdx.z;
    const double kc = octave_contrast(d_k[img], k_pow);
    const double inverse_k = 1.0 / (kc * kc);
    const float* GX = gxp + (size_t)img * px;
    const float* GY = gyp + (size_t)img * px;
    float* out = lflow + (size_t)img * px;
    const size_t i0 = ((size_t)blockIdx.x * 256 + threadIdx.x) * 4;
    if (i0 >= px) return;
    if ((px & 3u) == 0) {
        const float4 a = *reinterpret_cast<const float4*>(GX + i0), b = *reinterpret_cast<const float4*>(GY + i0);
        float4 o;
        o.x = pm_g2_px(a.x, b.x, inverse_k);
        o.y = pm_g2_px(a.y, b.y, inverse_k);
        o.z = pm_g2_px(a.z, b.z, inverse_k);
        o.w = pm_g2_px(a.w, b.w, inverse_k);
        *reinterpret_cast<float4*>(out + i0) = o;
    } else {
        for (size_t i = i0; i < i0 + 4 && i < px; ++i) out[i] = pm_g2_px(GX[i], GY[i], inverse_k);
    }
}

__global__ void k_ldet(const float* __restrict__ lxx, const float* __restrict__ lyy, const float* __restrict__ lxy,
                       float* __restrict__ out, size_t count, float q) {
    const size_t i = (size_t)blockIdx.x * blockDim.x + threadIdx.x;
    if (i >= count) return;
    out[i] = ((lxx[i] * lyy[i]) - (lxy[i] * lxy[i])) * q;
}

__global__ void k_accumulate(float* a, const float* b, size_t count) {
    const size_t i = (size_t)blockIdx.x * blockDim.x + threadIdx.x;
    if (i >= count) return;
    a[i] = a[i] + b[i];
}

__device__ __forceinline__ void nms_emit(float v, float xp, float xm, float yp, float ym, int x, int y, int w, int h,
                                         unsigned level, unsigned img, float thr, float border_m,
                                         Candidate* __restrict__ cand, unsigned cap, unsigned* __restrict__ count) {
    if (!(v > thr)) return;
    if (!(v > xp && v > xm && v > ym && v > yp)) return;
    const float fx = (float)x, fy = (float)y;
    const bool is_out = (roundf(fx - border_m) - 1.0f) < 0.0f || (roundf(fx + border_m) + 1.0f) >= (float)w ||
                        (roundf(fy - border_m) - 1.0f) < 0.0f || (roundf(fy + border_m) + 1.0f) >= (float)h;
    if (is_out) return;
    const unsigned slot = atomicAdd(count, 1u);
    if (slot < cap) {
        Candidate c;
        c.level = level;
        c.idx = (unsigned)(y * w + x);
        c.v = v; c.xp = xp; c.xm = xm; c.yp = yp; c.ym = ym;
        c.img = img;
        cand[slot] = c;
    }
}
__global__ void k_nms(const float* __restrict__ ldet, int w, int h, size_t img_stride, unsigned level, float thr,
                      float border_m, Candidate* __restrict__ cand, unsigned cap, unsigned* __restrict__ count) {
    const int x0 = (blockIdx.x * BX + threadIdx.x) * 4, y = blockIdx.y * BY + threadIdx.y;
    if (x0 >= w || y < 1 || y >= h - 1) return;
    const float* D = ldet + (size_t)blockIdx.z * img_stride;
    const float* row = D + (size_t)y * w;
    float c[6], up[4], dn[4];
    if ((w & 3) == 0 && x0 + 3 < w) {
        const float4 vc = *reinterpret_cast<const float4*>(row + x0);
        const float4 vu = *reinterpret_cast<const float4*>(row - w + x0);
        const float4 vd = *reinterpret_cast<const float4*>(row + w + x0);
        c[1] = vc.x; c[2] = vc.y; c[3] = vc.z; c[4] = vc.w;
        up[0] = vu.x; up[1] = vu.y; up[2] = vu.z; up[3] = vu.w;
        dn[0] = vd.x; dn[1] = vd.y; dn[2] = vd.z; dn[3] = vd.w;
    } else {
#pragma unroll
        for (int e = 0; e < 4; ++e) {
            const bool in = x0 + e < w;
            c[e + 1] = in ? row[x0 + e] : 0.0f;
            up[e] = in ? row[x0 + e - w] : 0.0f;
            dn[e] = in ? row[x0 + e + w] : 0.0f;
        }
    }
    c[0] = x0 > 0 ? row[x0 - 1] : 0.0f;
    c[5] = (x0 + 4 < w) ? row[x0 + 4] : 0.0f;
    const long last = (long)w * h - w - 1;
#pragma unroll
    for (int e = 0; e < 4; ++e) {
        const int x = x0 + e;
        if (x < 1 || x >= w) continue;
        if ((long)y * w + x >= last) continue;
        nms_emit(c[e + 1], c[e + 2], c[e], dn[e], up[e], x, y, w, h, level, blockIdx.z, thr, border_m, cand, cap, count);
    }
}

__constant__ float c_gauss25[7][7] = {
    {0.02546481f, 0.02350698f, 0.01849125f, 0.01239505f, 0.00708017f, 0.00344629f, 0.00142946f},
    {0.02350698f, 0.02169968f, 0.01706957f, 0.01144208f, 0.00653582f, 0.00318132f, 0.00131956f},
    {0.01849125f, 0.01706957f, 0.01342740f, 0.00900066f, 0.00514126f, 0.00250252f, 0.00103800f},
    {0.01239505f, 0.01144208f, 0.00900066f, 0.00603332f, 0.00344629f, 0.00167749f, 0.00069579f},
    {0.00708017f, 0.00653582f, 0.00514126f, 0.00344629f, 0.00196855f, 0.00095820f, 0.00039744f},
    {0.00344629f, 0.00318132f, 0.00250252f, 0.00167749f, 0.00095820f, 0.00046640f, 0.00019346f},
    {0.00142946f, 0.00131956f, 0.00103800f, 0.00069579f, 0.00039744f, 0.00019346f, 0.00008024f}};

struct OriTable {
    signed char a[112], b[112];
};
constexpr OriTable make_ori_table() {
    OriTable t{};
    int idx = 0;
    for (int i = -6; i <= 6; ++i)
        for (int j = -6; j <= 6; ++j)
            if (i * i + j * j < 36) {
                t.a[idx] = (signed char)i;
                t.b[idx] = (signed char)j;
                ++idx;
            }
    for (; idx < 112; ++idx) { t.a[idx] = 0; t.b[idx] = 0; }
    return t;
}
__constant__ OriTable c_ori = make_ori_table();
struct OriOrder {
    unsigned char k[112];
};
constexpr OriOrder make_ori_order() {
    OriOrder o{};
    const OriTable t = make_ori_table();
    int n = 0;
    for (int b = -6; b <= 6; ++b)
        for (int a = -6; a <= 6; ++a)
            for (int k = 0; k < 109; ++k)
                if (t.a[k] == a && t.b[k] == b) o.k[n++] = (unsigned char)k;
    for (; n < 112; ++n) o.k[n] = 0;
    return o;
}
__constant__ OriOrder c_ori_rows = make_ori_order();

__device__ __forceinline__ unsigned xcd_contiguous_group(unsigned b, unsigned nb) {
    return (b & 7u) * (nb >> 3) + (b >> 3);
}

constexpr int ORI_KPB = 32, ORI_NS = 109, ORI_NT = 256;
__global__ void __launch_bounds__(ORI_NT)
k_orientation(LevelTable tab, const KpParam* __restrict__ kps, unsigned nkp, const unsigned* __restrict__ d_nkp,
              unsigned long long window_mask, unsigned n_windows, OrientOut* __restrict__ out, unsigned out_stride) {
    __shared__ float s_rx[ORI_KPB * ORI_NS];
    __shared__ float s_ry[ORI_KPB * ORI_NS + 16];
    if (d_nkp) nkp = min(nkp, *d_nkp);
    const unsigned base = xcd_contiguous_group(blockIdx.x, gridDim.x) * ORI_KPB;
    if (base >= nkp) return;
    constexpr int ORI_IT = (ORI_KPB * ORI_NS + ORI_NT - 1) / ORI_NT, ORI_UB = 7;
    static_assert(ORI_IT % ORI_UB == 0, "whole batches");
    for (int it0 = 0; it0 < ORI_IT; it0 += ORI_UB) {
        float vx[ORI_UB], vy[ORI_UB], gw[ORI_UB];
        unsigned slot[ORI_UB];
#pragma unroll
        for (int u = 0; u < ORI_UB; ++u) {
            const unsigned idx = threadIdx.x + (unsigned)(it0 + u) * ORI_NT;
            const unsigned j = idx / ORI_NS, k = c_ori_rows.k[idx - j * ORI_NS];
            vx[u] = 0.0f; vy[u] = 0.0f; gw[u] = 0.0f;
            slot[u] = j * ORI_NS + k;
            if (idx < ORI_KPB * ORI_NS && base + j < nkp) {
                const KpParam kp = kps[base + j];
                const LevelPtrs lv = tab.lv[kp.level];
                const float* lx = lv.lx + (size_t)kp.img * lv.stride;
                const float* ly = lv.ly + (size_t)kp.img * lv.stride;
                const int a = c_ori.a[k], b = c_ori.b[k];
                const float fy = roundf(kp.yf + (float)b * kp.scale);
                const float fx = roundf(kp.xf + (float)a * kp.scale);
                const int iy = clampi(fy > 0.0f ? (int)fy : 0, 0, (int)lv.h - 1);
                const int ix = clampi(fx > 0.0f ? (int)fx : 0, 0, (int)lv.w - 1);
                gw[u] = c_gauss25[a < 0 ? -a : a][b < 0 ? -b : b];
                const size_t p = (size_t)iy * lv.w + ix;
                vx[u] = lx[p];
                vy[u] = ly[p];
            }
        }
#pragma unroll
        for (int u = 0; u < ORI_UB; ++u) {
            const unsigned idx = threadIdx.x + (unsigned)(it0 + u) * ORI_NT;
            const unsigned j = idx / ORI_NS;
            if (idx < ORI_KPB * ORI_NS) {
                const bool have = base + j < nkp;
                s_rx[slot[u]] = have ? gw[u] * vx[u] : 0.0f;
                s_ry[slot[u]] = have ? gw[u] * vy[u] : 0.0f;
            }
        }
    }
    __syncthreads();
    if (threadIdx.x >= 64) return;
    const unsigned lane = threadIdx.x, j = lane >> 1;
    const bool is_y = (lane & 1u) != 0;
    const float* py = s_ry + j * ORI_NS;
    const float* pa = is_y ? py : s_rx + j * ORI_NS;
    float t[ORI_NS];
#pragma unroll
    for (int k = 0; k < ORI_NS; ++k) t[k] = py[k] > 0.0f ? pa[k] : -0.0f;
    float sum = 0.0f, maxv = 0.0f, bx = 0.0f, by = 0.0f;
    unsigned found = 0;
    for (unsigned wdw = 0; wdw < n_windows; ++wdw) {
        if ((window_mask >> wdw) & 1ull) {
#pragma unroll
            for (int k = 0; k < ORI_NS; ++k) sum = sum + t[k];
        }
        const float other = __shfl_xor(sum, 1, 64);
        const float sx = is_y ? other : sum, sy = is_y ? sum : other;
        const float val = sx * sx + sy * sy;
        if (val > maxv) {
            maxv = val;
            bx = sx;
            by = sy;
            found = 1;
        }
    }
    if (!is_y && base + j < nkp) {
        OrientOut o;
        o.sum_x = bx; o.sum_y = by; o.found = found; o.angle_bits = 0;
        out[(size_t)(base + j) * out_stride] = o;
    }
}

struct PairTable {
    unsigned char a[162], b[162];
};
constexpr PairTable make_pairs() {
    PairTable t{};
    int p = 0;
    const int counts[3] = {4, 9, 16}, base[3] = {0, 4, 13};
    for (int g = 0; g < 3; ++g)
        for (int i = 0; i < counts[g]; ++i)
            for (int j = i + 1; j < counts[g]; ++j) {
                t.a[p] = (unsigned char)(base[g] + i);
                t.b[p] = (unsigned char)(base[g] + j);
                ++p;
            }
    return t;
}
__constant__ PairTable c_pairs = make_pairs();
struct BitTable3 {
    unsigned short e[512];
};
constexpr BitTable3 make_bits3() {
    BitTable3 t{};
    const PairTable p = make_pairs();
    const int npairs[3] = {6, 36, 120}, pbase[3] = {0, 6, 42};
    int b = 0;
    for (int g = 0; g < 3; ++g)
        for (int pos = 0; pos < 3; ++pos)
            for (int q = 0; q < npairs[g]; ++q)
                t.e[b++] = (unsigned short)((pos << 10) | (p.a[pbase[g] + q] << 5) | p.b[pbase[g] + q]);
    for (; b < 512; ++b) t.e[b] = 0;
    return t;
}
__constant__ BitTable3 c_bits3 = make_bits3();

constexpr int MLDB_KPB = 4;
constexpr int MLDB_LAT = 21, MLDB_NS = MLDB_LAT * MLDB_LAT;
struct DeviceAngles {
    OrientOut* sums;
    unsigned stride;
    unsigned fma;
    unsigned* flag;
};
struct MldbHostMirror {
    uint4* recs;
    const uint4* hdr;
    uint4* hdr_host;
    unsigned hdr_vec;
    uint8_t* desc;
};
__device__ __forceinline__ float2 device_angle(const DeviceAngles& da, unsigned kpi, bool write, const MldbHostMirror& hm) {
    OrientOut* o = da.sums + (size_t)kpi * da.stride;
    const float ang = o->found ? libm::atan2f_glibc(o->sum_y, o->sum_x) : 0.0f;
    bool bad = false;
    float co, si;
    if (da.fma) {
        co = libm::cosf_glibc<true>(ang, &bad);
        si = libm::sinf_glibc<true>(ang, &bad);
    } else {
        co = libm::cosf_glibc<false>(ang, &bad);
        si = libm::sinf_glibc<false>(ang, &bad);
    }
    if (write) {
        o->angle_bits = __float_as_uint(ang);
        if (bad && da.flag) atomicOr(da.flag, 1u);
        if (hm.recs) {
            const uint4* rec = reinterpret_cast<const uint4*>(da.sums) + (size_t)kpi * 2u - 1u;
            uint4 r0 = rec[0], r1 = rec[1];
            r1.w = __float_as_uint(ang);
            hm.recs[(size_t)kpi * 2u] = r0;
            hm.recs[(size_t)kpi * 2u + 1u] = r1;
        }
    }
    return float2{co, si};
}
__global__ void __launch_bounds__(64 * MLDB_KPB)
k_mldb(LevelTable tab, const KpParam* __restrict__ kps, const float2* __restrict__ cosi, unsigned nkp, const unsigned* __restrict__ d_nkp,
       DeviceAngles da, unsigned channels, uint8_t* __restrict__ desc64, unsigned first, MldbHostMirror hm) {
    __shared__ float s_win[MLDB_KPB][3][MLDB_NS + 7];
    __shared__ float s_val[MLDB_KPB][3][32];
    if (hm.recs && blockIdx.x == 0)
        for (unsigned i = threadIdx.x; i < hm.hdr_vec; i += 64 * MLDB_KPB) hm.hdr_host[i] = hm.hdr[i];
    if (d_nkp) nkp = min(nkp, *d_nkp);
    const unsigned lane = threadIdx.x & 63u, wv = threadIdx.x >> 6;
    const unsigned group0 = first + xcd_contiguous_group(blockIdx.x, gridDim.x) * MLDB_KPB;
    const unsigned kpi = group0 + wv;
    if (group0 >= nkp) return;
    const bool live = kpi < nkp;
    KpParam kp = kps[live ? kpi : 0];
    const float2 cs = da.sums ? device_angle(da, live ? kpi : 0, live && lane == 0, hm) : cosi[live ? kpi : 0];
    const LevelPtrs lv = tab.lv[__builtin_amdgcn_readfirstlane(kp.level)];
    const size_t ioff = (size_t)kp.img * lv.stride;
    const float* Lt = lv.lt + ioff;
    const float* Lx = lv.lx + ioff;
    const float* Ly = lv.ly + ioff;
    const float co = cs.x, si = cs.y, scale = kp.scale;
    unsigned short bits3[8];
#pragma unroll
    for (int r = 0; r < 8; ++r) bits3[r] = c_bits3.e[r * 64 + (int)lane];
    if (live) {
        constexpr int NIT = (MLDB_NS + 63) / 64;
        const bool k_fast = fabsf(co) >= fabsf(si);
        unsigned pidx[NIT];
        int widx[NIT];
#pragma unroll
        for (int it = 0; it < NIT; ++it) {
            const int sidx = min((int)lane + 64 * it, MLDB_NS - 1);
            const int qa = sidx / MLDB_LAT, qb = sidx - qa * MLDB_LAT;
            const int kk = k_fast ? qb : qa, ll = k_fast ? qa : qb;
            const int k = kk - 10, l = ll - 10;
            const float lf = (float)l + 0.5f, kf = (float)k + 0.5f;
            const float sample_y = kp.yf + (lf * co * scale + kf * si * scale);
            const float sample_x = kp.xf + (-lf * si * scale + kf * co * scale);
            const int y1 = clampi((int)roundf(sample_y), 0, (int)lv.h - 1);
            const int x1 = clampi((int)roundf(sample_x), 0, (int)lv.w - 1);
            pidx[it] = (unsigned)y1 * (unsigned)lv.w + (unsigned)x1;
            widx[it] = kk * MLDB_LAT + ll;
        }
        float vt[NIT], vx[NIT], vy[NIT];
#pragma unroll
        for (int it = 0; it < NIT; ++it) {
            vt[it] = Lt[pidx[it]];
            vx[it] = channels > 1 ? Lx[pidx[it]] : 0.0f;
            vy[it] = channels > 1 ? Ly[pidx[it]] : 0.0f;
        }
#pragma unroll
        for (int it = 0; it < NIT; ++it) {
            const int sidx = (int)lane + 64 * it;
            if (sidx >= MLDB_NS) continue;
            float v1 = 0.0f, v2 = 0.0f;
            if (channels > 1) {
                const float rx = vx[it], ry = vy[it];
                if (channels == 2) {
                    v1 = sqrtf(rx * rx + ry * ry);
                } else {
                    v2 = rx * co + ry * si;
                    v1 = -rx * si + ry * co;
                }
            }
            s_win[wv][0][widx[it]] = vt[it];
            s_win[wv][1][widx[it]] = v1;
            s_win[wv][2][widx[it]] = v2;
        }
    }
    __syncthreads();
    const unsigned cl = lane & 31u, ckp = 2u * wv + (lane >> 5);
    if (wv < MLDB_KPB / 2 && cl < 29 && group0 + ckp < nkp) {
        const int g = cl < 4 ? 0 : (cl < 13 ? 1 : 2);
        const int step = g == 0 ? 10 : (g == 1 ? 7 : 5), ng = g + 2;
        const int ci = (int)cl - (g == 0 ? 0 : (g == 1 ? 4 : 13));
        const int kk0 = (ci / ng) * step, ll0 = (ci % ng) * step;
        const int per_cell = step * step;
        const float* b0 = &s_win[ckp][0][0];
        const float* b1 = &s_win[ckp][1][0];
        const float* b2 = &s_win[ckp][2][0];
        float di = 0.0f, dx = 0.0f, dy = 0.0f;
#pragma unroll
        for (int dk = 0; dk < 10; ++dk) {
            const int o = (kk0 + min(dk, step - 1)) * MLDB_LAT + ll0;
            float r0[10], r1[10], r2[10];
#pragma unroll
            for (int dl = 0; dl < 10; ++dl) {
                r0[dl] = b0[o + dl];
                r1[dl] = b1[o + dl];
                r2[dl] = b2[o + dl];
            }
#pragma unroll
            for (int dl = 0; dl < 10; ++dl)
                if (dk < step && dl < step) {
                    di = di + r0[dl];
                    dx = dx + r1[dl];
                    dy = dy + r2[dl];
                }
        }
        const float ns = (float)per_cell;
        s_val[ckp][0][cl] = di / ns;
        s_val[ckp][1][cl] = dx / ns;
        s_val[ckp][2][cl] = dy / ns;
    }
    __syncthreads();
    const unsigned seg0 = 6u * channels, seg1 = seg0 + 36u * channels, total = seg1 + 120u * channels;
    unsigned long long words[8];
#pragma unroll
    for (int r = 0; r < 8; ++r) {
        const unsigned b = (unsigned)r * 64u + lane;
        bool bit = false;
        if (channels == 3) {
            const unsigned e = bits3[r];
            bit = s_val[wv][e >> 10][(e >> 5) & 31u] > s_val[wv][e >> 10][e & 31u];
        } else if (b < total) {
            unsigned rel, npairs, pbase;
            if (b < seg0) { rel = b; npairs = 6; pbase = 0; }
            else if (b < seg1) { rel = b - seg0; npairs = 36; pbase = 6; }
            else { rel = b - seg1; npairs = 120; pbase = 42; }
            const unsigned pos = rel / npairs, p = rel % npairs;
            bit = s_val[wv][pos][c_pairs.a[pbase + p]] > s_val[wv][pos][c_pairs.b[pbase + p]];
        }
        words[r] = __ballot(bit);
    }
    if (live && lane < 8) {
        unsigned long long wvw = words[0];
#pragma unroll
        for (int r = 1; r < 8; ++r)
            if (lane == (unsigned)r) wvw = words[r];
        reinterpret_cast<unsigned long long*>(desc64 + (size_t)kpi * 64)[lane] = wvw;
        if (hm.desc) reinterpret_cast<unsigned long long*>(hm.desc + (size_t)kpi * 64)[lane] = wvw;
    }
}

constexpr int MT = 256;

__device__ __forceinline__ unsigned hamming64(const uint4 (&q)[4], const uint4* __restrict__ row, unsigned tail_mask) {
    unsigned d = 0;
#pragma unroll
    for (int k = 0; k < 4; ++k) {
        const uint4 t = row[k];
        d += __popc(q[k].x ^ t.x);
        d += __popc(q[k].y ^ t.y);
        d += __popc(q[k].z ^ t.z);
        d += __popc((q[k].w ^ t.w) & (k == 3 ? tail_mask : 0xffffffffu));
    }
    return d;
}
__device__ __forceinline__ void top2_feed(unsigned d, unsigned j, unsigned& min_d, unsigned& second, unsigned& min_j) {
    if (d < min_d) {
        second = min_d;
        min_d = d;
        min_j = j;
    } else if (d < second) {
        second = d;
    }
}
__global__ void __launch_bounds__(MT) k_match(const uint4* __restrict__ d0, unsigned n0, const uint4* __restrict__ d1,
                                             unsigned n1, unsigned chunk_rows, unsigned threshold, unsigned tail_mask,
                                             MatchRec* __restrict__ out) {
    __shared__ uint4 s_tile[MT * 4];
    const unsigned i = blockIdx.x * MT + threadIdx.x;
    uint4 q[4];
    const bool live = i < n0;
#pragma unroll
    for (int k = 0; k < 4; ++k) q[k] = live ? d0[(size_t)i * 4 + k] : make_uint4(0, 0, 0, 0);
    unsigned min_d = threshold, second = threshold, min_j = 0;
    const unsigned begin = blockIdx.y * chunk_rows, end = min(n1, begin + chunk_rows);
    for (unsigned base = begin; base < end; base += MT) {
        const unsigned rows = min((unsigned)MT, end - base);
        __syncthreads();
        for (unsigned e = threadIdx.x; e < rows * 4; e += MT) s_tile[e] = d1[(size_t)base * 4 + e];
        __syncthreads();
        unsigned r = 0;
        for (; r + 4 <= rows; r += 4) {
            const unsigned da = hamming64(q, s_tile + (r + 0) * 4, tail_mask), db = hamming64(q, s_tile + (r + 1) * 4, tail_mask);
            const unsigned dc = hamming64(q, s_tile + (r + 2) * 4, tail_mask), dd = hamming64(q, s_tile + (r + 3) * 4, tail_mask);
            top2_feed(da, base + r + 0, min_d, second, min_j);
            top2_feed(db, base + r + 1, min_d, second, min_j);
            top2_feed(dc, base + r + 2, min_d, second, min_j);
            top2_feed(dd, base + r + 3, min_d, second, min_j);
        }
        for (; r < rows; ++r) top2_feed(hamming64(q, s_tile + r * 4, tail_mask), base + r, min_d, second, min_j);
    }
    if (live) {
        MatchRec m;
        m.min_d = min_d; m.second_d = second; m.min_j = min_j; m._pad = 0;
        out[(size_t)blockIdx.y * n0 + i] = m;
    }
}
__global__ void k_match_merge(const MatchRec* __restrict__ part, unsigned n0, unsigned chunks, unsigned threshold,
                              MatchRec* __restrict__ out) {
    const unsigned i = blockIdx.x * blockDim.x + threadIdx.x;
    if (i >= n0) return;
    unsigned min_d = threshold, second = threshold, min_j = 0;
    for (unsigned c = 0; c < chunks; ++c) {
        const MatchRec m = part[(size_t)c * n0 + i];
        top2_feed(m.min_d, m.min_j, min_d, second, min_j);
        if (m.second_d < second) second = m.second_d;
    }
    MatchRec o;
    o.min_d = min_d; o.second_d = second; o.min_j = min_j; o._pad = 0;
    out[i] = o;
}

__global__ void __launch_bounds__(1024) k_match_compact(const MatchRec* __restrict__ rec, unsigned n0, unsigned chunks,
                                                        unsigned threshold, double ratio2,
                                                        akz_match* __restrict__ out,
                                                        unsigned long long* __restrict__ n_out) {
    constexpr int IT = 16;
    __shared__ unsigned s_cnt[IT][16];
    __shared__ unsigned s_base;
    rec += (size_t)blockIdx.x * chunks * n0;
    out += (size_t)blockIdx.x * n0;
    n_out += blockIdx.x;
    const unsigned lane = threadIdx.x & 63u, wave = threadIdx.x >> 6;
    if (threadIdx.x == 0) s_base = 0;
    __syncthreads();
    for (unsigned start = 0; start < n0; start += IT * 1024u) {
        unsigned md[IT], mj[IT], keepmask = 0u;
#pragma unroll
        for (int it = 0; it < IT; ++it) {
            const unsigned i = start + (unsigned)it * 1024u + threadIdx.x;
            bool keep = false;
            md[it] = mj[it] = 0u;
            if (i < n0) {
                unsigned min_d = threshold, second = threshold, min_j = 0;
                for (unsigned c = 0; c < chunks; ++c) {
                    const MatchRec p = rec[(size_t)c * n0 + i];
                    top2_feed(p.min_d, p.min_j, min_d, second, min_j);
                    if (p.second_d < second) second = p.second_d;
                }
                md[it] = min_d; mj[it] = min_j;
                keep = ((double)min_d < (double)second * ratio2) && (min_d < threshold);
            }
            const unsigned long long bal = __ballot(keep);
            if (lane == 0) s_cnt[it][wave] = (unsigned)__popcll(bal);
            keepmask |= keep ? 1u << it : 0u;
        }
        __syncthreads();
        unsigned off = s_base;
#pragma unroll
        for (int it = 0; it < IT; ++it) {
            unsigned row = 0, below = 0;
#pragma unroll
            for (unsigned w = 0; w < 16; ++w) {
                const unsigned c = s_cnt[it][w];
                row += c;
                below += w < wave ? c : 0u;
            }
            const bool keep = (keepmask >> it) & 1u;
            const unsigned long long bal = __ballot(keep);
            if (keep) {
                akz_match o;
                o.index_0 = start + (unsigned)it * 1024u + threadIdx.x; o.index_1 = mj[it]; o.distance = (double)md[it];
                out[off + below + (unsigned)__popcll(bal & ((1ull << lane) - 1ull))] = o;
            }
            off += row;
        }
        __syncthreads();
        if (threadIdx.x == 0) s_base = off;
        __syncthreads();
    }
    if (threadIdx.x == 0) *n_out = s_base;
}

__global__ void __launch_bounds__(256) k_match_merge_compact(const MatchRec* __restrict__ part, unsigned n0, unsigned chunks,
                                                             unsigned threshold, double ratio2, akz_match* __restrict__ out,
                                                             unsigned long long* __restrict__ n_out,
                                                             unsigned long long* __restrict__ state, unsigned epoch) {
    __shared__ unsigned s_cnt[4];
    __shared__ unsigned s_prefix;
    const unsigned b = blockIdx.x, tid = threadIdx.x, lane = tid & 63u, wave = tid >> 6;
    const unsigned i = b * 256u + tid;
    unsigned min_d = threshold, second = threshold, min_j = 0;
    bool keep = false;
    if (i < n0) {
        for (unsigned c = 0; c < chunks; ++c) {
// ... 40 lines not shown

inline dim3 grid2d(uint32_t w, uint32_t h, uint32_t n) { return dim3((w + BX - 1) / BX, (h + BY - 1) / BY, n); }

}

namespace launch {

static Scharr1 scharr1() {
    const Taps m = taps_scharr_main(1);
    return Scharr1{m.wgt[0], m.wgt[1]};
}

void filter_h_f32(hipStream_t s, const float* in, float* out, uint32_t w, uint32_t h, uint32_t n, const Taps& t) {
    hipLaunchKernelGGL(k_filter_h<float>, grid2d(w, h, n), dim3(BX, BY), 0, s, in, out, (int)w, (int)h, t);
}
void filter_h_u8(hipStream_t s, const uint8_t* in, float* out, uint32_t w, uint32_t h, uint32_t n, const Taps& t) {
    hipLaunchKernelGGL(k_filter_h<uint8_t>, grid2d(w, h, n), dim3(BX, BY), 0, s, in, out, (int)w, (int)h, t);
}
void filter_v_f32(hipStream_t s, const float* in, float* out, uint32_t w, uint32_t h, uint32_t n, const Taps& t) {
    hipLaunchKernelGGL(k_filter_v, grid2d(w, h, n), dim3(BX, BY), 0, s, in, out, (int)w, (int)h, t);
}
void delay(hipStream_t s, uint32_t microseconds) {
    hipLaunchKernelGGL(k_delay, dim3(1), dim3(64), 0, s, (unsigned long long)microseconds * 100ull, (unsigned*)nullptr);
}
void half_size(hipStream_t s, const float* in, float* out, uint32_t w, uint32_t h, uint32_t n) {
    if ((w & 7u) == 0 && (((uintptr_t)in | (uintptr_t)out) & 15u) == 0) {
        hipLaunchKernelGGL(k_half_size4, grid2d(w / 4, h / 2, n), dim3(BX, BY), 0, s, in, out, (int)w, (int)h);
        return;
    }
    hipLaunchKernelGGL(k_half_size, grid2d(w / 2, h / 2, n), dim3(BX, BY), 0, s, in, out, (int)w, (int)h);
}
void pm_g2(hipStream_t s, const float* lx, const float* ly, float* out, uint32_t w, uint32_t h, uint32_t n,
           const double* d_k, uint32_t k_scale_pow) {
    const size_t plane = (size_t)w * h;
    hipLaunchKernelGGL(k_pm_g2, dim3((unsigned)((plane + 255) / 256), 1, n), dim3(256), 0, s, lx, ly, out, plane, d_k,
                       k_scale_pow);
}
void flow(hipStream_t s, const float* lsmooth, float* lflow, uint32_t w, uint32_t h, uint32_t n, const double* d_k,
          uint32_t k_scale_pow) {
    hipLaunchKernelGGL(k_flow, grid2d(w, h, n), dim3(BX, BY), 0, s, lsmooth, lflow, (int)w, (int)h, scharr1(), d_k,
                       k_scale_pow);
}
void fed_step(hipStream_t s, const float* lt_in, const float* lflow, float* lt_out, float* lstep, uint32_t w,
              uint32_t h, uint32_t n, float half_tau) {
    hipLaunchKernelGGL(k_fed_step, grid2d(w, h, n), dim3(BX, BY), 0, s, lt_in, lflow, lt_out, lstep, (int)w, (int)h,
                       half_tau);
}
constexpr int kFedDeepTh = 10;
uint64_t fed_deep_workgroups(uint32_t w, uint32_t h, uint32_t n) {
    return (uint64_t)((w + 63) / 64) * ((h + kFedDeepTh - 1) / kFedDeepTh) * n;
}
bool fed_epilogue_supported(uint32_t w, uint32_t h, uint32_t n_steps) {
    if (n_steps == 0 || n_steps > 14 || w < 8 || h < 8 || (w - 1) % 64 == 0) return false;
    const uint32_t th = n_steps <= 6 ? 32u : (uint32_t)kFedDeepTh;
    return (h - 1) % th != 0;
}
void fed_fused(hipStream_t s, const float* lt_in, const float* lflow, float* lt_out, float* lstep, uint32_t w,
               uint32_t h, uint32_t n, const float* half_taus, uint32_t n_steps, const FedNextPrep* next) {
    constexpr int TW = 64, TH = 32, NT = 512;
    FedTaus ht;
    ht.n = (int)n_steps;
    for (uint32_t i = 0; i < 16; ++i) ht.half_tau[i] = i < n_steps ? half_taus[i] : 0.0f;
    const dim3 grid((w + TW - 1) / TW, (h + TH - 1) / TH, n);
    FedEpi ep{};
    if (next) {
        const Taps m = taps_scharr_main(1);
        ep.lsmooth = next->lsmooth;
        ep.lflow = next->lflow;
        ep.taps = PrepTaps{next->g3[0], next->g3[1], next->g3[2], m.wgt[0], m.wgt[1]};
        ep.d_k = next->d_k;
        ep.k_pow = next->k_pow;
        if (n_steps <= 6) {
            hipLaunchKernelGGL((k_fed_own<TW, TH, 8, NT, true>), grid, dim3(NT), 0, s, lt_in, lflow, lt_out, lstep, (int)w, (int)h, ht, ep);
        } else {
            const dim3 g10((w + TW - 1) / TW, (h + kFedDeepTh - 1) / kFedDeepTh, n);
            hipLaunchKernelGGL((k_fed_own<TW, kFedDeepTh, 16, NT, true>), g10, dim3(NT), 0, s, lt_in, lflow, lt_out, lstep, (int)w, (int)h, ht,
                               ep);
        }
        return;
    }
    {
        if (n_steps <= 4) {
            if (h >= 48) {
                const dim3 g48((w + TW - 1) / TW, (h + 47) / 48, n);
                hipLaunchKernelGGL((k_fed_own<TW, 48, 4, NT>), g48, dim3(NT), 0, s, lt_in, lflow, lt_out, lstep, (int)w,
                                   (int)h, ht, ep);
            } else
                hipLaunchKernelGGL((k_fed_own<TW, TH, 4, NT>), grid, dim3(NT), 0, s, lt_in, lflow, lt_out, lstep, (int)w,
                                   (int)h, ht, ep);
        } else if (n_steps <= 8)
            hipLaunchKernelGGL((k_fed_own<TW, TH, 8, NT>), grid, dim3(NT), 0, s, lt_in, lflow, lt_out, lstep, (int)w,
                               (int)h, ht, ep);
        else {
            const dim3 g10((w + TW - 1) / TW, (h + kFedDeepTh - 1) / kFedDeepTh, n);
            hipLaunchKernelGGL((k_fed_own<TW, kFedDeepTh, 16, NT>), g10, dim3(NT), 0, s, lt_in, lflow, lt_out, lstep,
                               (int)w, (int)h, ht, ep);
        }
    }
}
#ifndef AKZ_HIST_BLOCKS
#define AKZ_HIST_BLOCKS 128u
#endif
static unsigned contrast_blocks(uint32_t h, uint32_t n) {
    constexpr uint32_t target = 512u;
    const uint32_t per_image = std::max<uint32_t>(128u, target / std::max<uint32_t>(n, 1u));
    return h > 2 ? std::min<uint32_t>(h - 2, per_image) : 1u;
}
void contrast_max(hipStream_t s, const float* blurred, uint32_t w, uint32_t h, uint32_t n,
                  unsigned long long* d_hmax_bits) {
    hipLaunchKernelGGL(k_contrast_max, dim3(contrast_blocks(h, n), 1, n), dim3(CT), 0, s, blurred, (int)w, (int)h,
                       scharr1(), d_hmax_bits);
}
void contrast_hist(hipStream_t s, const float* blurred, uint32_t w, uint32_t h, uint32_t n,
                   const unsigned long long* d_hmax_bits, uint32_t nbins, uint32_t* d_hist) {
    const unsigned copies = nbins <= 512 ? 8u : (nbins <= 2048 ? 2u : 1u);
    hipLaunchKernelGGL(k_contrast_hist, dim3(contrast_blocks(h, n), 1, n), dim3(CT), nbins * copies * sizeof(unsigned), s,
                       blurred, (int)w, (int)h, scharr1(), d_hmax_bits, nbins, copies, d_hist);
}
void contrast_final(hipStream_t s, const unsigned long long* d_hmax_bits, const uint32_t* d_hist, uint32_t nbins,
                    double percentile, uint32_t n, double* d_k) {
    hipLaunchKernelGGL(k_contrast_final, dim3(n), dim3(256), nbins * sizeof(unsigned), s, d_hmax_bits, d_hist, nbins, percentile,
                       n, d_k);
}
constexpr int HT = 1024;
void contrast_hist_final(hipStream_t s, const float* gx, const float* gy, uint32_t w, uint32_t h, uint32_t n, unsigned long long* d_smax_bits,
                         uint32_t nbins, uint32_t* d_hist, uint32_t* d_done, double percentile, double* d_k) {
    const unsigned copies = nbins <= 512 ? 8u : (nbins <= 2048 ? 2u : 1u);
    const uint64_t quads = ((uint64_t)w * h + 3) / 4;
    const unsigned blocks = (unsigned)std::max<uint64_t>(1, std::min<uint64_t>((quads + HT - 1) / HT, std::max<uint32_t>(32u, AKZ_HIST_BLOCKS / std::max<uint32_t>(n, 1u))));
    hipLaunchKernelGGL(k_contrast_hist_final<HT>, dim3(blocks, 1, n), dim3(HT), nbins * copies * sizeof(unsigned), s, gx, gy, (int)w, (int)h,
                       d_smax_bits, nbins, copies, d_hist, d_done, percentile, d_k);
}
void flow_from_pair(hipStream_t s, const float* gx, const float* gy, float* lflow, uint32_t w, uint32_t h, uint32_t n, const double* d_k,
                    uint32_t k_pow) {
    const uint64_t px = (uint64_t)w * h;
    hipLaunchKernelGGL(k_flow_pair, dim3((unsigned)((px + 1023) / 1024), 1, n), dim3(256), 0, s, gx, gy, lflow, (size_t)px, d_k, k_pow);
}
void ldet(hipStream_t s, const float* lxx, const float* lyy, const float* lxy, float* out, uint64_t count,
          float sigma_quat) {
    hipLaunchKernelGGL(k_ldet, dim3((unsigned)((count + 255) / 256)), dim3(256), 0, s, lxx, lyy, lxy, out,
                       (size_t)count, sigma_quat);
}
void rcp_f64_to_f32(hipStream_t s, const double* x, float* out, uint64_t n) {
    hipLaunchKernelGGL(k_rcp_f64_to_f32, dim3((unsigned)((n + 255) / 256)), dim3(256), 0, s, x, out, (size_t)n);
}
void accumulate(hipStream_t s, float* a, const float* b, uint64_t count) {
    hipLaunchKernelGGL(k_accumulate, dim3((unsigned)((count + 255) / 256)), dim3(256), 0, s, a, b, (size_t)count);
}
void nms(hipStream_t s, const float* ldet_p, uint32_t w, uint32_t h, uint32_t n, uint64_t img_stride, uint32_t level,
         float thr, float border_m, Candidate* d_cand, uint32_t cap, uint32_t* d_count) {
    hipLaunchKernelGGL(k_nms, grid2d((w + 3) / 4, h, n), dim3(BX, BY), 0, s, ldet_p, (int)w, (int)h, (size_t)img_stride,
                       level, thr, border_m, d_cand, cap, d_count);
}
void orientation(hipStream_t s, const LevelTable& lt, const KpParam* d_kp, uint32_t nkp,
                 unsigned long long window_mask, uint32_t n_windows, OrientOut* d_out) {
    if (nkp == 0) return;
    const uint32_t groups = (nkp + ORI_KPB - 1) / ORI_KPB;
    hipLaunchKernelGGL(k_orientation, dim3((groups + 7u) / 8u * 8u), dim3(ORI_NT), 0, s, lt, d_kp, nkp, (const unsigned*)nullptr,
                       window_mask, n_windows, d_out, 1u);
}
void orientation_counted(hipStream_t s, const LevelTable& lt, const KpParam* d_kp, const uint32_t* d_nkp, uint32_t max_kp,
                         unsigned long long window_mask, uint32_t n_windows, OrientOut* d_out, uint32_t out_stride) {
    if (max_kp == 0) return;
    const uint32_t groups = (max_kp + ORI_KPB - 1) / ORI_KPB;
    hipLaunchKernelGGL(k_orientation, dim3((groups + 7u) / 8u * 8u), dim3(ORI_NT), 0, s, lt, d_kp, max_kp, d_nkp, window_mask, n_windows,
                       d_out, out_stride);
}

void mldb(hipStream_t s, const LevelTable& lt, const KpParam* d_kp, const float* d_cosi, uint32_t nkp,
          uint32_t channels, uint8_t* d_desc64) {
    if (nkp == 0) return;
    const uint32_t groups = (nkp + MLDB_KPB - 1) / MLDB_KPB;
    hipLaunchKernelGGL(k_mldb, dim3((groups + 7u) / 8u * 8u), dim3(64 * MLDB_KPB), 0, s, lt, d_kp,
                       reinterpret_cast<const float2*>(d_cosi), nkp, (const unsigned*)nullptr, DeviceAngles{nullptr, 0u, 0u, nullptr}, channels,
                       d_desc64, 0u, MldbHostMirror{nullptr, nullptr, nullptr, 0u, nullptr});
}
void mldb_counted(hipStream_t s, const LevelTable& lt, const KpParam* d_kp, const uint32_t* d_nkp, uint32_t first, uint32_t last, OrientOut* d_sums,
                  uint32_t sums_stride, bool libm_fma, uint32_t* d_flag, uint32_t channels, uint8_t* d_desc64, const MldbMirror* mirror) {
    first = first / MLDB_KPB * MLDB_KPB;
    MldbHostMirror hm{nullptr, nullptr, nullptr, 0u, nullptr};
    if (mirror && sums_stride == 2)
        hm = MldbHostMirror{(uint4*)mirror->host_recs, (const uint4*)mirror->d_hdr, (uint4*)mirror->host_hdr, mirror->hdr_bytes / 16u, mirror->host_desc};
    if (last <= first && !hm.recs) return;
    const uint32_t groups = last > first ? (last - first + MLDB_KPB - 1) / MLDB_KPB : 1u;
    hipLaunchKernelGGL(k_mldb, dim3((groups + 7u) / 8u * 8u), dim3(64 * MLDB_KPB), 0, s, lt, d_kp, (const float2*)nullptr, last, d_nkp,
                       DeviceAngles{d_sums, sums_stride, libm_fma ? 1u : 0u, d_flag}, channels, d_desc64, first, hm);
}
void libm_eval(hipStream_t s, const float* a, const float* b, float* out3, uint64_t n, bool fma, uint32_t* d_flag) {
    if (n == 0) return;
    hipLaunchKernelGGL(k_libm_eval, dim3((unsigned)((n + 255) / 256)), dim3(256), 0, s, a, b, out3, (size_t)n, fma ? 1u : 0u, d_flag);
}
uint32_t match_num_chunks(uint32_t n0, uint32_t n1) {
    const uint32_t qblocks = (n0 + MT - 1) / MT, tiles = std::max<uint32_t>(1, (n1 + MT - 1) / MT);
    const uint32_t want = std::max<uint32_t>(1, 2048u / std::max<uint32_t>(1, qblocks));
    return std::max<uint32_t>(1, std::min<uint32_t>({want, (tiles + 3) / 4, 64u}));
}
void match(hipStream_t s, const uint8_t* d0, uint32_t n0, const uint8_t* d1, uint32_t n1, uint32_t threshold,
           bool rows_le_61, uint32_t chunks, MatchRec* d_rec) {
    if (n0 == 0) return;
    const uint32_t tiles = std::max<uint32_t>(1, (n1 + MT - 1) / MT);
    const uint32_t chunk_rows = ((tiles + chunks - 1) / chunks) * MT;
    hipLaunchKernelGGL(k_match, dim3((n0 + MT - 1) / MT, chunks), dim3(MT), 0, s, reinterpret_cast<const uint4*>(d0), n0,
                       reinterpret_cast<const uint4*>(d1), n1, chunk_rows, threshold, rows_le_61 ? 0xffu : 0xffffffffu, d_rec);
}
size_t match_merge_compact_state_bytes(uint32_t n0) { return ((size_t)(n0 + 255) / 256 + 1) * sizeof(unsigned long long); }
void match_merge_compact(hipStream_t s, const MatchRec* d_part, uint32_t n0, uint32_t chunks, uint32_t threshold, double ratio2,
                         akz_match* d_out, unsigned long long* d_n_out, void* d_state, uint32_t epoch) {
    hipLaunchKernelGGL(k_match_merge_compact, dim3((n0 + 255) / 256), dim3(256), 0, s, d_part, n0, chunks, threshold, ratio2, d_out,
                       d_n_out, (unsigned long long*)d_state, epoch);
}
void match_merge(hipStream_t s, const MatchRec* d_part, uint32_t n0, uint32_t chunks, uint32_t threshold, MatchRec* d_out) {
    hipLaunchKernelGGL(k_match_merge, dim3((n0 + 255) / 256), dim3(256), 0, s, d_part, n0, chunks, threshold, d_out);
}
void match_compact(hipStream_t s, const MatchRec* d_rec, uint32_t n0, uint32_t chunks, uint32_t threshold, double ratio2,
                   akz_match* d_out, unsigned long long* d_n_out) {
    hipLaunchKernelGGL(k_match_compact, dim3(1), dim3(1024), 0, s, d_rec, n0, chunks, threshold, ratio2, d_out, d_n_out);
}
void match_compact_sets(hipStream_t s, const MatchRec* d_rec, uint32_t n0, uint32_t n_sets, uint32_t chunks, uint32_t threshold,
                        double ratio2, akz_match* d_out, unsigned long long* d_n_out) {
    hipLaunchKernelGGL(k_match_compact, dim3(n_sets), dim3(1024), 0, s, d_rec, n0, chunks, threshold, ratio2, d_out, d_n_out);
}

}
}
```

akaze-rust_amd/csrc/akz_result.cpp:

```cpp
#include "akz_extract.hpp"

int slab_acquire(akz_ctx* c, size_t bytes, void** p, size_t* got) {
    bytes = align_up(std::max<size_t>(bytes, 256), 256);
    std::lock_guard<std::mutex> lk(c->slab_m);
    DevBuf b;
    for (size_t i = 0; i < c->slab_pool.size() && !b.p; ++i)
        if (c->slab_pool[i].bytes >= bytes && c->slab_pool[i].bytes <= bytes + bytes / 4 + 65536) {
            b = std::move(c->slab_pool[i]);
            c->slab_pool.erase(c->slab_pool.begin() + (long)i);
        }
    if (!b.p) {
        bytes += bytes / 8;
        AKZ_HIP_TRY(b.acquire(bytes, false));
        AKZ_HIP_TRY(alloc_fill(c, b.p, bytes));
    }
    *got = b.bytes;
    *p = b.detach();
    return AKZ_OK;
}
void slab_release(akz_ctx* c, void* p, size_t bytes) {
    std::lock_guard<std::mutex> lk(c->slab_m);
    if (c->slab_pool.size() >= 8) {
        (void)sync_all_streams(c);
        c->slab_pool.erase(c->slab_pool.begin());
// ... 27 lines not shown
    if (j->slot >= 0) c->slot_busy[j->slot] = false;
    j->slot = -1;
    ev_put(c, std::move(j->nms_done));
    result_release_device(j->r.get());
}
void job_wait(akz_job* j) {
    if (!j->fin) return;
    std::unique_lock<std::mutex> lk(j->fin->m);
    j->fin->done.wait(lk, [&] { return j->finished; });
}
void job_destroy(akz_job* j) {
    if (!j) return;
    if (j->fin) {
        job_wait(j);
        if (j->out) result_delete(j->out);
    } else {
        job_release(j);
    }
    delete j;
}

int free_slot(const akz_ctx* c, int want) {
    for (int i = 0; i < akz_ctx::kSlots && want < 0; ++i)
        if (!c->slot_busy[i]) want = i;
    return want >= 0 && !c->slot_busy[want] ? want : -1;
}
int job_open(akz_ctx* c, const char* who, int want_slot, uint32_t w, uint32_t h, uint32_t n, uint32_t flags, const akz_config& cfg, JobOpening& o) {
    o.slot = free_slot(c, want_slot);
    if (o.slot < 0) {
        set_error(std::string(who) + ": too many extractions in flight on this context (finish one first)");
        return AKZ_ERR_INVALID_ARG;
    }
    o.job.reset(new akz_job);
    o.job->in_hand = c->in_hand;
    o.job->alone_at_begin = o.job->in_hand->fetch_add(1) == 0;
    o.job->r.reset(new akz_result);
    akz_result* r = o.job->r.get();
    r->ctx = c;
    ++c->live_results;
    r->cfg = cfg;
    r->w = w; r->h = h; r->n = n; r->flags = flags;
    return build_plan(w, h, r->cfg, r->plan);
}
int job_layout(JobOpening& o, const std::vector<std::pair<uint32_t, int>>& wanted) {
    akz_result* r = o.job->r.get();
    std::memset(r->planes, 0, sizeof(r->planes));
    size_t off = 0;
    std::vector<size_t> at;
    for (const auto& lp : wanted) {
        at.push_back(off);
        off += align_up(plane_bytes(r->plan[lp.first].w, r->plan[lp.first].h, r->n), 256);
    }
    const size_t k_off = off;
    off += align_up((size_t)r->n * sizeof(double), 256);
    AKZ_TRY(slab_acquire(r->ctx, off, &r->slab, &r->slab_bytes));
    o.laid_out = true;
    for (size_t i = 0; i < wanted.size(); ++i) r->planes[wanted[i].first][wanted[i].second] = (float*)((char*)r->slab + at[i]);
    if (!r->planes[0][AKZ_LSMOOTH]) r->planes[0][AKZ_LSMOOTH] = r->planes[0][AKZ_LT];
    r->d_k = (double*)((char*)r->slab + k_off);
    return AKZ_OK;
}
JobOpening::~JobOpening() {
    if (!laid_out || !job) return;
    if (drain_side) (void)sync_all_streams(job->r->ctx, kSyncSide);
    result_release_device(job->r.get());
}
akz_job* JobOpening::keep(uint32_t cap) {
    job->slot = slot;
    job->cap = cap;
    job->r->ctx->slot_busy[slot] = true;
    laid_out = false;
    return job.release();
}

extern "C" {

int akz_result_free(akz_result* r) {
    if (!r) return AKZ_OK;
    (void)hipSetDevice(r->ctx->device);
    result_delete(r);
    return AKZ_OK;
}
int akz_result_num_images(const akz_result* r, uint64_t* n) {
    if (!r || !n) return AKZ_ERR_INVALID_ARG;
    *n = r->n;
    return AKZ_OK;
}
static int check_img(const akz_result* r, uint64_t img) {
    if (!r || img >= r->n) {
        set_error("null result or image index out of range");
        return AKZ_ERR_INVALID_ARG;
    }
    return AKZ_OK;
}
int akz_result_counts(const akz_result* r, uint64_t img, uint64_t* n_levels, uint64_t* n_keypoints,
                      uint64_t* desc_bytes) {
    AKZ_TRY(check_img(r, img));
    if (n_levels) *n_levels = r->plan.size();
    if (n_keypoints) *n_keypoints = r->kps[(size_t)img].size();
    if (desc_bytes) *desc_bytes = ((6 + 36 + 120) * r->cfg.descriptor_channels + 7) / 8;
    return AKZ_OK;
}
int akz_result_keypoints(const akz_result* r, uint64_t img, akz_keypoint* out) {
    AKZ_TRY(check_img(r, img));
    const auto& k = r->kps[(size_t)img];
    if (!k.empty()) {
        if (!out) return AKZ_ERR_INVALID_ARG;
        std::memcpy(out, k.data(), k.size() * sizeof(akz_keypoint));
    }
    return AKZ_OK;
}
int akz_result_descriptors(const akz_result* r, uint64_t img, uint8_t* out) {
    AKZ_TRY(check_img(r, img));
    if (r->flags & AKZ_NO_HOST_DESCRIPTORS) {
        set_error("descriptors were kept on the device (AKZ_NO_HOST_DESCRIPTORS)");
        return AKZ_ERR_INVALID_ARG;
    }
    const size_t nk = r->kps[(size_t)img].size();
    if (nk) {
        if (!out) return AKZ_ERR_INVALID_ARG;
        const size_t nb = ((6 + 36 + 120) * r->cfg.descriptor_channels + 7) / 8;
        const uint8_t* rows = r->rows64.data() + r->desc_off[(size_t)img] * 64;
        for (size_t i = 0; i < nk; ++i) std::memcpy(out + i * nb, rows + i * 64, nb);
    }
    return AKZ_OK;
}
int akz_result_describe_keypoints(const akz_result* r, uint64_t img, akz_keypoint* kps, uint64_t n_kp,
                                  int compute_orientation, uint8_t* descriptors) {
    AKZ_TRY(check_img(r, img));
    akz_ctx* c = r->ctx;
    AKZ_TRY(bind(c));
    if (n_kp == 0) return AKZ_OK;
    if (!kps || !descriptors) {
        set_error("akz_result_describe_keypoints: null argument");
        return AKZ_ERR_INVALID_ARG;
    }
    const size_t L = r->plan.size();
    const LevelTable tab = level_table(r);
    AKZ_TRY(ensure_aux(c));
    hipStream_t s = c->aux;
    bool own_octave = false;
    if (compute_orientation)
        for (uint64_t i = 0; i < n_kp && !own_octave; ++i)
            own_octave = kps[i].class_id < L && kps[i].octave != r->plan[(size_t)kps[i].class_id].octave;
    const uint64_t n_par = own_octave ? 2 * n_kp : n_kp;
    AKZ_TRY(ensure_pinned(c, c->pin[PIN_PARAMS], n_par * sizeof(KpParam)));
    KpParam* params = (KpParam*)c->pin[PIN_PARAMS].p;
    for (uint64_t i = 0; i < n_kp; ++i) {
        const akz_keypoint& k = kps[i];
        if (k.class_id >= L || k.octave > 30) {
            set_error("akz_result_describe_keypoints: keypoint class_id / octave out of range");
            return AKZ_ERR_INVALID_ARG;
        }
        params[i] = kp_param(k.x, k.y, k.size, k.octave, (uint32_t)k.class_id, (uint32_t)img);
        if (own_octave) params[n_kp + i] = kp_param(k.x, k.y, k.size, r->plan[(size_t)k.class_id].octave, (uint32_t)k.class_id, (uint32_t)img);
    }
    AKZ_TRY(ensure(c, c->kp_in, n_par * sizeof(KpParam)));
    AKZ_TRY(ensure(c, c->kp_out, n_kp * sizeof(OrientOut)));
    AKZ_TRY(ensure(c, c->cosi, n_kp * 2 * sizeof(float)));
    AKZ_TRY(ensure_pinned(c, c->pin[PIN_COUNT_SUMS], n_kp * std::max(sizeof(OrientOut), 2 * sizeof(float))));
    KpParam* d_kp = (KpParam*)c->kp_in.p;
    AKZ_HIP_TRY(hipMemcpyAsync(d_kp, params, n_par * sizeof(KpParam), hipMemcpyHostToDevice, s));
    if (compute_orientation) {
        unsigned long long wmask = 0;
        uint32_t nwin = 0;
        orientation_windows(&wmask, &nwin);
        OrientOut* d_oo = (OrientOut*)c->kp_out.p;
        launch::orientation(s, tab, own_octave ? d_kp + n_kp : d_kp, (uint32_t)n_kp, wmask, nwin, d_oo);
        AKZ_HIP_TRY(hipGetLastError());
        OrientOut* oo = (OrientOut*)c->pin[PIN_COUNT_SUMS].p;
        AKZ_HIP_TRY(hipMemcpyAsync(oo, d_oo, n_kp * sizeof(OrientOut), hipMemcpyDeviceToHost, s));
        AKZ_HIP_TRY(hipStreamSynchronize(s));
        for (uint64_t i = 0; i < n_kp; ++i)
            if (oo[i].found) kps[i].angle = atan2f(oo[i].sum_y, oo[i].sum_x);
    }
    AKZ_TRY(ensure_pinned(c, c->pin[PIN_COSI], n_kp * 2 * sizeof(float)));
    float* cosi = (float*)c->pin[PIN_COSI].p;
    for (uint64_t i = 0; i < n_kp; ++i) {
        cosi[2 * i] = cosf(kps[i].angle);
        cosi[2 * i + 1] = sinf(kps[i].angle);
    }
    AKZ_HIP_TRY(hipMemcpyAsync(c->cosi.p, cosi, n_kp * 2 * sizeof(float), hipMemcpyHostToDevice, s));
    AKZ_TRY(ensure(c, c->match_a, n_kp * 64));
    uint8_t* d_rows = (uint8_t*)c->match_a.p;
    launch::mldb(s, tab, d_kp, (const float*)c->cosi.p, (uint32_t)n_kp, (uint32_t)r->cfg.descriptor_channels, d_rows);
    AKZ_HIP_TRY(hipGetLastError());
    AKZ_TRY(ensure_pinned(c, c->pin[PIN_ROWS], n_kp * 64));
    uint8_t* rows = (uint8_t*)c->pin[PIN_ROWS].p;
    AKZ_HIP_TRY(hipMemcpyAsync(rows, d_rows, n_kp * 64, hipMemcpyDeviceToHost, s));
    AKZ_HIP_TRY(hipStreamSynchronize(s));
    const size_t nb = ((6 + 36 + 120) * r->cfg.descriptor_channels + 7) / 8;
    for (uint64_t i = 0; i < n_kp; ++i) std::memcpy(descriptors + i * nb, rows + i * 64, nb);
    return AKZ_OK;
}
int akz_result_device_descriptors(const akz_result* r, uint64_t img, const uint8_t** d_desc, uint64_t* n_keypoints) {
    AKZ_TRY(check_img(r, img));
    if (d_desc) *d_desc = r->d_desc64 ? r->d_desc64 + r->desc_off[(size_t)img] * 64 : nullptr;
    if (n_keypoints) *n_keypoints = r->kps[(size_t)img].size();
    return AKZ_OK;
}
int akz_result_copy_device_descriptors(const akz_result* r, uint8_t* d_dst, uint64_t capacity_rows, uint64_t* rows) {
    if (!r) return AKZ_ERR_INVALID_ARG;
    const uint64_t total = r->desc_off.empty() ? 0 : r->desc_off.back();
    if (rows) *rows = total;
    if (total == 0) return AKZ_OK;
    if (!d_dst || capacity_rows < total) {
        set_error("copy_device_descriptors: destination too small");
        return AKZ_ERR_BUFFER;
    }
    AKZ_TRY(bind(r->ctx, true, false));
    akz_ctx* c = r->ctx;
    AKZ_TRY(ensure_aux(c));
    AKZ_HIP_TRY(hipMemcpyAsync(d_dst, r->d_desc64, total * 64, hipMemcpyDeviceToDevice, c->aux));
    AKZ_HIP_TRY(hipStreamSynchronize(c->aux));
    return AKZ_OK;
}
int akz_result_contrast(const akz_result* r, uint64_t img, double* k) {
    AKZ_TRY(check_img(r, img));
    if (!k) return AKZ_ERR_INVALID_ARG;
    *k = r->k_host[(size_t)img];
    return AKZ_OK;
}
int akz_result_level_info(const akz_result* r, uint64_t level, double* etime, double* esigma, uint32_t* octave,
                          uint32_t* sublevel, uint32_t* sigma_size, uint32_t* w, uint32_t* h, uint64_t* n_tau,
                          double* tau, uint64_t tau_cap) {
    if (!r) return AKZ_ERR_INVALID_ARG;
    return level_info_out(r->plan, level, etime, esigma, octave, sublevel, sigma_size, w, h, nullptr, n_tau, tau,
                          tau_cap);
}
int akz_result_device_plane(const akz_result* r, uint64_t img, uint64_t level, akz_plane plane,
                            const float** d_plane) {
    AKZ_TRY(check_img(r, img));
    if (level >= r->plan.size() || (int)plane < 0 || (int)plane > 9 || !d_plane) {
        set_error("level/plane out of range");
        return AKZ_ERR_INVALID_ARG;
    }
    const float* base = r->planes[(size_t)level][(int)plane];
    const LevelPlan& lv = r->plan[(size_t)level];
    *d_plane = base ? base + (size_t)img * lv.w * lv.h : nullptr;
    return AKZ_OK;
}
static int recompute_plane(const akz_result* r, uint64_t img, uint64_t level, akz_plane plane, const float** d_out) {
    akz_ctx* c = r->ctx;
    AKZ_TRY(bind(c));
    const JobForm f = no_job_form(c);
    const LevelPlan& lv = r->plan[(size_t)level];
    const size_t px = (size_t)lv.w * lv.h, pb = px * sizeof(float);
    auto img_plane = [&](uint64_t l, int p) { return r->planes[(size_t)l][p] + (size_t)img * r->plan[(size_t)l].w * r->plan[(size_t)l].h; };
    *d_out = nullptr;
    if (plane == AKZ_LXX || plane == AKZ_LYY || plane == AKZ_LXY) {
        for (int k = 0; k < 6; ++k) AKZ_TRY(ensure(c, c->lazy[k], pb));
        float* b[6];
        for (int k = 0; k < 6; ++k) b[k] = (float*)c->lazy[k].p;
        AKZ_TRY(detector_impl(c, f, img_plane(level, AKZ_LSMOOTH), lv.det_sigma, b[0], b[1], b[2], b[3], b[4], b[5], lv.w, lv.h, 1));
        *d_out = plane == AKZ_LXX ? b[2] : plane == AKZ_LYY ? b[3] : b[4];
        return AKZ_OK;
    }
    if (plane == AKZ_LSTEP && level > 0) {
        const LevelPlan& pv = r->plan[(size_t)level - 1];
        for (int k = 0; k < 4; ++k) AKZ_TRY(ensure(c, c->lazy[k], std::max(pb, (size_t)4)));
        float *A = (float*)c->lazy[0].p, *B = (float*)c->lazy[1].p, *step = (float*)c->lazy[2].p;
        const float* in = img_plane(level - 1, AKZ_LT);
        if (lv.octave > pv.octave) {
            launch::half_size(c->stream, in, (float*)c->lazy[3].p, pv.w, pv.h, 1);
            in = (const float*)c->lazy[3].p;
        }
        AKZ_HIP_TRY(hipMemsetAsync(step, 0, pb, c->stream));
        AKZ_TRY(fed_impl(c, f, in, A, B, img_plane(level, AKZ_LFLOW), step, lv.w, lv.h, 1, lv.tau.data(), (uint32_t)lv.tau.size()));
        *d_out = step;
        return AKZ_OK;
    }
    return AKZ_OK;
}

int akz_fetch_plane(const akz_result* r, uint64_t img, uint64_t level, akz_plane plane, float* out, uint64_t* n_px) {
    const float* d = nullptr;
    AKZ_TRY(akz_result_device_plane(r, img, level, plane, &d));
    const LevelPlan& lv = r->plan[(size_t)level];
    const bool lazy = !d && (plane == AKZ_LXX || plane == AKZ_LYY || plane == AKZ_LXY || (plane == AKZ_LSTEP && level > 0));
    if (lazy && !out) {
        if (n_px) *n_px = (uint64_t)lv.w * lv.h;
        return AKZ_OK;
    }
    if (lazy) AKZ_TRY(recompute_plane(r, img, level, plane, &d));
    const uint64_t npx = d ? (uint64_t)lv.w * lv.h : 0;
    if (n_px) *n_px = npx;
    if (out && npx) {
        AKZ_TRY(bind(r->ctx));
        AKZ_HIP_TRY(hipMemcpyAsync(out, d, npx * sizeof(float), hipMemcpyDeviceToHost, r->ctx->stream));
        AKZ_HIP_TRY(hipStreamSynchronize(r->ctx->stream));
    }
    return AKZ_OK;
}

static constexpr int kFetchStageBufs = 3;
static constexpr size_t kFetchStageBytes = (size_t)8 << 20;
static_assert(kFetchStageBufs <= 4, "akz_ctx::fetch_chunk has 4 events");
static constexpr size_t kFetchHostPiece = (size_t)512 << 10;

static bool pinned_range(const void* p, size_t bytes) {
    hipPointerAttribute_t a;
    if (hipPointerGetAttributes(&a, p) != hipSuccess) {
        (void)hipGetLastError();
        return false;
    }
    if (a.type != hipMemoryTypeHost) return false;
    void* start = nullptr;
    size_t size = 0;
    if (hipPointerGetAttribute(&start, HIP_POINTER_ATTRIBUTE_RANGE_START_ADDR, (hipDeviceptr_t)p) != hipSuccess ||
        hipPointerGetAttribute(&size, HIP_POINTER_ATTRIBUTE_RANGE_SIZE, (hipDeviceptr_t)p) != hipSuccess) {
        (void)hipGetLastError();
        return false;
    }
    const uintptr_t b = (uintptr_t)start, q = (uintptr_t)p;
    return q >= b && q + bytes <= b + size;
}

static int fetch_events(akz_ctx* c) {
    for (Stream& s : c->fetch) AKZ_TRY(s.ensure());
    for (Event* e : {&c->fetch_chunk[0], &c->fetch_chunk[1], &c->fetch_chunk[2], &c->fetch_chunk[3], &c->fetch_start,
                     &c->fetch_join, &c->fetch_ready[0], &c->fetch_ready[1], &c->fetch_free[0], &c->fetch_free[1]})
        AKZ_TRY(e->ensure());
    return AKZ_OK;
}

namespace {
struct FetchEngine {
    explicit FetchEngine(akz_ctx* ctx) : c(ctx) {}
    akz_ctx* c;
    struct Piece { size_t off; float* dst; size_t bytes; };
    std::vector<Piece> pieces[kFetchStageBufs];
    size_t used = 0;
    uint64_t filled = 0, drained = 0;
    uint64_t direct = 0;
    char* stage(uint64_t chunk) const { return (char*)c->fetch_stage.p + (chunk % kFetchStageBufs) * kFetchStageBytes; }

    int copy(const float* src, float* dst, size_t bytes) {
        if (pinned_range(dst, bytes)) {
// ... 152 lines not shown
```

akaze-rust_amd/csrc/akz_sort.hip:

```cpp
#include <hip/hip_runtime.h>

#include <cstring>
#include <vector>
#include <type_traits>

#include <rocprim/device/device_radix_sort.hpp>

#include "akz_internal.hpp"
#include "akz_gates.hpp"
#include "akz_select.hpp"

namespace akz {
namespace {

struct KeyBits {
    unsigned idx_bits, level_bits, total;
};
__host__ __device__ inline unsigned bits_for(unsigned long long n) {
    unsigned b = 1;
    while (b < 63 && (1ull << b) < n) ++b;
    return b;
}

__global__ void k_candidate_keys(const Candidate* __restrict__ cand, unsigned cap, const unsigned* __restrict__ d_count,
// ... 197 lines not shown
}
__global__ void __launch_bounds__(256) k_bucket_place(const Candidate* __restrict__ cand, unsigned cap, const unsigned* __restrict__ d_count,
                                                      const unsigned* __restrict__ start, const unsigned* __restrict__ bucket_of,
                                                      const unsigned* __restrict__ slot_of, unsigned* __restrict__ row_keys) {
    const unsigned i = blockIdx.x * blockDim.x + threadIdx.x;
    if (i >= min(*d_count, cap)) return;
    row_keys[start[bucket_of[i]] + slot_of[i]] = cand[i].idx;
}
__global__ void __launch_bounds__(256) k_bucket_rank(const Candidate* __restrict__ cand, unsigned cap, const unsigned* __restrict__ d_count,
                                                     const unsigned* __restrict__ start, const unsigned* __restrict__ bucket_of,
                                                     const unsigned* __restrict__ row_keys, Candidate* __restrict__ out,
                                                     unsigned* __restrict__ zero) {
    const unsigned i = blockIdx.x * blockDim.x + threadIdx.x;
    if (i >= min(*d_count, cap)) return;
    const Candidate c = cand[i];
    const unsigned b = bucket_of[i], lo = start[b], hi = start[b + 1];
    unsigned rank = 0;
    for (unsigned j = lo; j < hi; ++j) rank += row_keys[j] < c.idx ? 1u : 0u;
    out[lo + rank] = c;
    if (zero) zero[lo + rank] = 0u;
}

constexpr int REL_WAVES = 4;
__global__ void __launch_bounds__(64 * REL_WAVES) k_relations(const Candidate* __restrict__ sorted, const unsigned* __restrict__ d_count, unsigned cap,
                                                              RelLevels lv, const unsigned* __restrict__ offs, const unsigned* __restrict__ rows,
                                                              unsigned short* __restrict__ rel, unsigned* __restrict__ img_flags,
                                                              unsigned* __restrict__ revcnt, unsigned short* __restrict__ rev) {
    __shared__ unsigned short s_out[REL_WAVES][kRel1 + kRel2 + 2];
    const unsigned lane = threadIdx.x & 63u;
    const unsigned wv = __builtin_amdgcn_readfirstlane(threadIdx.x >> 6);
    const unsigned i = blockIdx.x * REL_WAVES + wv;
    if (i >= min(*d_count, cap)) return;
    const Candidate c = sorted[i];
    if (c.img >= lv.n_images || c.level >= lv.n_levels) return;
    const unsigned L = lv.n_levels, l = c.level;
    const unsigned* o = offs + (size_t)c.img * (L + 1);
    const unsigned img0 = o[0];
    unsigned short* const mine = s_out[wv];
    if (lane < (unsigned)(kRel1 + kRel2)) mine[lane] = 0xffffu;
    const bool too_many = o[L] - img0 > 65533u;
    bool over1 = false, over2 = false;
    const float size = lv.size[l], size2 = size * size, ratio = lv.ratio[l];
    const unsigned ly = c.idx / lv.w[l], lx = c.idx - ly * lv.w[l];
    const float qx = (float)lx * ratio, qy = (float)ly * ratio;
    const float px = qx + 0.5f * (ratio - 1.0f), py = qy + 0.5f * (ratio - 1.0f);
    const unsigned* rowI = rows + (size_t)c.img * lv.row_base[L];
    auto scan = [&](unsigned pl, unsigned b, unsigned e, float x0, float y0, int first, int room, int& used, bool& overflow) {
        if (b >= e) return;
        const float pr = lv.ratio[pl], off = 0.5f * (pr - 1.0f);
        const unsigned pw = lv.w[pl], ph = lv.h[pl];
        const float reach = size + 1.0f;
        const float ylo = (y0 - reach - off) / pr - 1.0f, yhi = (y0 + reach - off) / pr + 1.0f;
        const unsigned r0 = ylo <= 0.0f ? 0u : (unsigned)ylo;
        if (yhi < 0.0f || r0 >= ph) return;
        const unsigned r1 = min((unsigned)yhi + 1u, ph);
        const unsigned* rt = rowI + lv.row_base[pl];
        const unsigned jb = max(b, rt[r0]), je = min(e, rt[r1]);
        for (unsigned j0 = jb; j0 < je; j0 += 64u) {
            const unsigned j = j0 + lane;
            bool hit = false;
            if (j < je) {
                const unsigned pidx = sorted[j].idx;
                const unsigned py_i = pidx / pw, px_i = pidx - py_i * pw;
                const float sx = (float)px_i * pr + off, sy = (float)py_i * pr + off;
                const float dist = (x0 - sx) * (x0 - sx) + (y0 - sy) * (y0 - sy);
                hit = dist <= size2;
            }
            const unsigned long long m = __ballot(hit);
            if (hit) {
                const int at_list = used + (int)__popcll(m & ((1ull << lane) - 1ull));
                if (at_list < room) mine[first + at_list] = (unsigned short)(j - img0);
                if (first == 0 && revcnt) {
                    const unsigned at = atomicAdd(&revcnt[j], 1u);
                    if (at < (unsigned)sel::kRev) rev[(size_t)j * sel::kRev + at] = (unsigned short)(i - img0);
                }
            }
            used += (int)__popcll(m);
            if (used > room) overflow = true;
        }
    };
    int used1 = 0, used2 = 0;
    if (l > 0) scan(l - 1, o[l - 1], o[l], qx, qy, 0, kRel1, used1, over1);
    scan(l, o[l], i, qx, qy, 0, kRel1, used1, over1);
    if (l + 1 < L) scan(l + 1, o[l + 1], o[l + 2], px, py, kRel1, kRel2, used2, over2);
    if (lane == 0) {
        if (over1) mine[0] = 0xfffeu;
        if (over2) mine[kRel1] = 0xfffeu;
        if (too_many) img_flags[c.img] = 1u;
    }
    unsigned short* out = rel + (size_t)i * (kRel1 + kRel2);
    if (lane < (unsigned)(kRel1 + kRel2)) out[lane] = mine[lane];
}


typedef sel::Row<kRel1, kRel2> SelRow;
static_assert(sizeof(SelRow) == 64 && kRel1 == 12 && kRel2 == 6, "four 16-byte loads; k_select knows where the fields are");
__global__ void __launch_bounds__(256) k_sel_prepare(const Candidate* __restrict__ sorted, const unsigned* __restrict__ d_count, unsigned cap,
                                                     unsigned n_levels, unsigned n_images, const unsigned* __restrict__ offs,
                                                     const unsigned short* __restrict__ rel, const unsigned* __restrict__ revcnt,
                                                     const unsigned short* __restrict__ rev, SelRow* __restrict__ rows,
                                                     unsigned char* __restrict__ state0, unsigned* __restrict__ img_flags) {
    const unsigned i = blockIdx.x * blockDim.x + threadIdx.x;
    if (i >= min(*d_count, cap)) return;
    const Candidate c = sorted[i];
    if (c.img >= n_images || c.level >= n_levels) return;
    const unsigned img0 = offs[(size_t)c.img * (n_levels + 1)];
    const unsigned me = i - img0;
    const unsigned short* row = rel + (size_t)i * (kRel1 + kRel2);
    const bool over = row[0] == sel::kListOverflow || revcnt[i] > (unsigned)sel::kRev;
    SelRow out;
    const float mine = fabsf(c.v);
    unsigned wins = 0;
    bool open = true;
#pragma unroll
    for (int j = 0; j < kRel1; ++j) {
        const unsigned short q = row[j];
        unsigned pred = sel::kNone;
        if (!open || q >= sel::kListOverflow) {
            open = false;
        } else {
            const unsigned qi = img0 + q, cnt = min(revcnt[qi], (unsigned)sel::kRev);
            for (unsigned m = 0; m < cnt; ++m) {
                const unsigned e = rev[(size_t)qi * sel::kRev + m];
                if (e < me && (pred == sel::kNone || e > pred)) pred = e;
            }
            if (mine > fabsf(sorted[qi].v)) wins |= 1u << j;
        }
        out.rel1[j] = open ? q : sel::kNone;
        out.pred[j] = (unsigned short)pred;
    }
    out.wins = (unsigned short)wins;
#pragma unroll
    for (int j = 0; j < kRel2; ++j) out.rel2[j] = row[kRel1 + j];
    {
        const float d_x = 0.5f * (c.xp - c.xm), d_y = 0.5f * (c.yp - c.ym);
        unsigned len = 0;
#pragma unroll
        for (int j = 0; j < kRel1; ++j) len += out.rel1[j] != sel::kNone ? 1u : 0u;
        out.refined = (unsigned short)((fabsf(-d_x) <= 1.0f && fabsf(-d_y) <= 1.0f ? 1u : 0u) | (len << 8));
    }
    rows[i] = out;
    state0[i] = row[0] == sel::kNone ? (unsigned char)1 : (unsigned char)0;
    if (over) atomicOr(&img_flags[c.img], (row[0] == sel::kListOverflow ? 2u : 0u) | (revcnt[i] > (unsigned)sel::kRev ? 16u : 0u));
}

constexpr int SEL_NT = 1024;
constexpr unsigned SEL_MAX_CANDS = 65536;
constexpr unsigned SEL_MAX_LOOKS = 4u << 20;
struct SelKp {
    sel::KpRec rec;
    OrientOut sums;
};
static_assert(sizeof(SelKp) == 32, "akz_api.cpp fetches 32-byte records");
struct SelOut {
    unsigned* hdr;
    SelKp* recs;
    KpParam* pars;
    unsigned* total;
    const unsigned* d_count;
    const double* d_k;
};
__device__ __forceinline__ void sel_header_extras(const SelOut& out, unsigned img, unsigned flags) {
    out.hdr[img * 16 + 8] = *out.d_count;
    out.hdr[img * 16 + 9] = flags;
    const double k = out.d_k[img];
    out.hdr[img * 16 + 10] = (unsigned)((unsigned long long)__double_as_longlong(k) & 0xffffffffull);
    out.hdr[img * 16 + 11] = (unsigned)((unsigned long long)__double_as_longlong(k) >> 32);
}
struct SelPacked {
    uint4 v[4];
};
__device__ __forceinline__ SelPacked sel_load_row(const SelRow* __restrict__ p) {
    SelPacked r;
    const uint4* q = reinterpret_cast<const uint4*>(p);
    r.v[0] = q[0]; r.v[1] = q[1]; r.v[2] = q[2]; r.v[3] = q[3];
    return r;
}
__device__ __forceinline__ void sel_compiler_fence() { __asm__ volatile("" ::: "memory"); }
__device__ __forceinline__ unsigned short sel_word_load(const unsigned short* p) {
    return __hip_atomic_load(p, __ATOMIC_RELAXED, __HIP_MEMORY_SCOPE_WORKGROUP);
}
__device__ __forceinline__ void sel_word_store(unsigned short* p, unsigned short v) {
    __hip_atomic_store(p, v, __ATOMIC_RELAXED, __HIP_MEMORY_SCOPE_WORKGROUP);
}
__global__ void __launch_bounds__(SEL_NT) k_select(const Candidate* __restrict__ sorted, RelLevels lv, const unsigned* __restrict__ offs,
                                                   const SelRow* __restrict__ rows, const unsigned char* __restrict__ state0,
                                                   const unsigned* __restrict__ img_flags, const unsigned* __restrict__ row_table,
                                                   SelOut out) {
    __shared__ unsigned short s_word[SEL_MAX_CANDS];
    __shared__ unsigned s_bits[SEL_MAX_CANDS / 32];
    __shared__ unsigned s_pref[SEL_MAX_CANDS / 32];
    __shared__ unsigned s_part[SEL_NT / 64];
    __shared__ unsigned s_extrema, s_abort, s_looks;
    __shared__ float s_ratio[kMaxLevels], s_size[kMaxLevels];
    __shared__ unsigned s_w[kMaxLevels];
    const unsigned img = blockIdx.x, tid = threadIdx.x, lane = tid & 63u, wv = tid >> 6;
    if (tid < (unsigned)kMaxLevels) {
        s_ratio[tid] = lv.ratio[tid];
        s_size[tid] = lv.size[tid];
        s_w[tid] = lv.w[tid];
    }
    const unsigned L = lv.n_levels;
    const unsigned* o = offs + (size_t)img * (L + 1);
    const unsigned img0 = o[0], n = o[L] - img0;
    unsigned status = img_flags[img];
    if (n > 65533u) status |= 1u;
    if (status != 0u || n == 0u) {
        if (tid == 0) {
            out.hdr[img * 16 + 0] = 0u; out.hdr[img * 16 + 1] = 0u; out.hdr[img * 16 + 2] = status; out.hdr[img * 16 + 3] = 0u;
            sel_header_extras(out, img, img_flags[img]);
            if (out.total) *out.total = 0u;
        }
        return;
    }
    const Candidate* cand = sorted + img0;
    const SelRow* rowI = rows + img0;
    const unsigned long long t0 = wall_clock64();
    if (tid == 0) { s_extrema = 0u; s_abort = 0u; s_looks = 0u; }
    const unsigned per = (n + SEL_NT - 1) / SEL_NT;
    auto cand_of = [&](unsigned k) -> unsigned { return k >= per ? 0xffffffffu : tid + k * SEL_NT; };
    unsigned long long mask = 0ull;
    constexpr int U = 8;
    for (unsigned k0 = 0; k0 < per; k0 += U) {
        unsigned char st[U];
#pragma unroll
        for (int u = 0; u < U; ++u) {
            const unsigned c = cand_of(k0 + u);
            st[u] = c < n ? state0[img0 + c] : (unsigned char)1;
        }
#pragma unroll
        for (int u = 0; u < U; ++u) {
            const unsigned c = cand_of(k0 + u);
            if (c < n) {
                s_word[c] = st[u] ? (unsigned short)c : sel::kUndecided;
                if (!st[u]) mask |= 1ull << (k0 + u);
            }
        }
    }
    __syncthreads();
    const unsigned long long t1 = wall_clock64();
    auto WORD = [&](unsigned short q) -> unsigned short { return s_word[q]; };
    for (unsigned i = tid; i < SEL_MAX_CANDS / 32; i += SEL_NT) s_bits[i] = 0u;
    SelPacked nxt;
    int b_cur = -1, b_nxt = -1;
    auto fetch = [&](SelPacked& r, int& b) {
        b = -1;
        if (mask) {
            b = __ffsll((long long)mask) - 1;
            mask &= mask - 1ull;
            r = sel_load_row(rowI + cand_of((unsigned)b));
        }
    };
    unsigned wq[6], wp[6], wins = 0, len = 0, hit_q = 0;
    sel::Progress prog;
    auto open_row = [&](const SelPacked& r) {
        wq[0] = r.v[0].x; wq[1] = r.v[0].y; wq[2] = r.v[0].z; wq[3] = r.v[0].w; wq[4] = r.v[1].x; wq[5] = r.v[1].y;
        wp[0] = r.v[1].z; wp[1] = r.v[1].w; wp[2] = r.v[2].x; wp[3] = r.v[2].y; wp[4] = r.v[2].z; wp[5] = r.v[2].w;
        wins = r.v[3].x & 0xffffu;
        len = (r.v[3].w >> 24) & 15u;
#pragma unroll
        for (int i = 0; i < 6; ++i) {
            AKZ_SEL_KEEP(wq[i]);
            AKZ_SEL_KEEP(wp[i]);
        }
        AKZ_SEL_KEEP(wins);
        AKZ_SEL_KEEP(len);
        sel::start(&prog);
    };
    {
        SelPacked first;
        fetch(first, b_cur);
        if (b_cur >= 0) open_row(first);
    }
    __builtin_amdgcn_s_waitcnt(0x0F70);
    fetch(nxt, b_nxt);
    unsigned looks = 0, waited = 0;
    while (b_cur >= 0) {
        ++looks;
        while ((unsigned)prog.through < len) {
            const unsigned q = wq[0] & 0xffffu, pr = wp[0] & 0xffffu;
            const bool has_pred = pr != sel::kNone;
            sel_compiler_fence();
            const unsigned wpred = sel_word_load(&s_word[has_pred ? pr : 0u]);
            sel_compiler_fence();
            const unsigned wq_now = sel_word_load(&s_word[q]);
            sel_compiler_fence();
            const int before = prog.at;
            if (!sel::advance(&prog, has_pred, (unsigned short)wpred, (unsigned short)wq_now)) break;
            if (prog.at != before) hit_q = q;
#pragma unroll
            for (int i = 0; i < 5; ++i) {
                wq[i] = __builtin_amdgcn_alignbit(wq[i + 1], wq[i], 16);
                wp[i] = __builtin_amdgcn_alignbit(wp[i + 1], wp[i], 16);
            }
            wq[5] >>= 16;
            wp[5] >>= 16;
        }
        if ((unsigned)prog.through == len) {
            const unsigned short c = (unsigned short)cand_of((unsigned)b_cur);
            bool replaces;
            const unsigned short mine = sel::turn(prog, c, (unsigned short)wins, &replaces);
            if (replaces) sel_word_store(&s_word[hit_q], sel::kGone);
            sel_compiler_fence();
            sel_word_store(&s_word[c], mine);
            sel_compiler_fence();
            b_cur = b_nxt;
            if (b_cur >= 0) open_row(nxt);
            fetch(nxt, b_nxt);
            waited = 0;
        } else if ((++waited & 255u) == 0u) {
            sel_compiler_fence();
            if (waited > SEL_MAX_LOOKS || __hip_atomic_load(&s_abort, __ATOMIC_RELAXED, __HIP_MEMORY_SCOPE_WORKGROUP) != 0u) {
                __hip_atomic_store(&s_abort, 1u, __ATOMIC_RELAXED, __HIP_MEMORY_SCOPE_WORKGROUP);
                break;
            }
        }
    }
    atomicMax(&s_looks, looks);
    __syncthreads();
    const unsigned long long t2 = wall_clock64();
    if (s_abort) status = 4u;
    if (status != 0u) {
        if (tid == 0) {
            out.hdr[img * 16 + 0] = 0u; out.hdr[img * 16 + 1] = 0u; out.hdr[img * 16 + 2] = status; out.hdr[img * 16 + 3] = s_looks;
            sel_header_extras(out, img, img_flags[img]);
            if (out.total) *out.total = 0u;
        }
        return;
    }
    unsigned long long surv = 0ull;
    unsigned my_extrema = 0;
    constexpr int U2 = 4, U3 = 4;
    for (unsigned k0 = 0; k0 < per; k0 += U3) {
        uint4 tail[U3];
#pragma unroll
        for (int u = 0; u < U3; ++u) {
            const unsigned c = cand_of(k0 + u);
            tail[u] = make_uint4(0u, 0u, 0u, 0u);
            if (c < n && sel::alive(s_word[c])) tail[u] = reinterpret_cast<const uint4*>(rowI + c)[3];
        }
#pragma unroll
        for (int u = 0; u < U3; ++u) {
            const unsigned c = cand_of(k0 + u);
            if (c >= n || !sel::alive(s_word[c])) continue;
            union { uint4 v; unsigned short h[8]; } t;
            t.v = tail[u];
            const unsigned short* r2 = &t.h[1];
            const unsigned short mine = s_word[c];
            bool repeated;
            if (r2[0] == sel::kListOverflow) {
                repeated = false;
                const Candidate cd = cand[c];
                const unsigned l = cd.level, w = s_w[l];
                if (l + 1 < L) {
                    const float ratio = s_ratio[l], size = s_size[l], size2 = size * size;
                    const unsigned ly = cd.idx / w, lx = cd.idx - ly * w;
                    const float px = (float)lx * ratio + 0.5f * (ratio - 1.0f), py = (float)ly * ratio + 0.5f * (ratio - 1.0f);
                    const float pr = s_ratio[l + 1], off = 0.5f * (pr - 1.0f), reach = size + 1.0f;
                    const unsigned pw = s_w[l + 1], ph = lv.h[l + 1];
                    const float ylo = (py - reach - off) / pr - 1.0f, yhi = (py + reach - off) / pr + 1.0f;
                    const unsigned r0 = ylo <= 0.0f ? 0u : (unsigned)ylo;
                    if (yhi >= 0.0f && r0 < ph) {
                        const unsigned* rt = row_table + (size_t)img * lv.row_base[L] + lv.row_base[l + 1];
                        const unsigned jb = rt[r0], je = rt[min((unsigned)yhi + 1u, ph)];
                        for (unsigned j = jb; j < je && !repeated; ++j) {
                            const Candidate p = sorted[j];
                            const unsigned q = j - img0;
                            if (!sel::alive(s_word[q]) || s_word[q] < mine) continue;
                            const unsigned qy = p.idx / pw, qx = p.idx - qy * pw;
                            const float sx = (float)qx * pr + off, sy = (float)qy * pr + off;
                            const float dist = (px - sx) * (px - sx) + (py - sy) * (py - sy);
                            repeated = dist <= size2;
                        }
                    }
                }
            } else {
                repeated = sel::repeated_later<kRel2>(mine, r2, WORD);
            }
            if (repeated) continue;
            ++my_extrema;
            if (t.h[7] & 1u) surv |= 1ull << (k0 + u);
        }
    }
#pragma unroll
    for (int off = 32; off > 0; off >>= 1) my_extrema += __shfl_xor(my_extrema, off, 64);
    if (lane == 0 && my_extrema) atomicAdd(&s_extrema, my_extrema);
    __syncthreads();
    const unsigned long long t3 = wall_clock64();
    for (unsigned long long m = surv; m; m &= m - 1ull) {
        const unsigned org = s_word[cand_of((unsigned)(__ffsll((long long)m) - 1))];
        atomicOr(&s_bits[org >> 5], 1u << (org & 31u));
    }
    __syncthreads();
    constexpr unsigned WPT = SEL_MAX_CANDS / 32 / SEL_NT;
    unsigned cnt[WPT], mine_n = 0;
#pragma unroll
    for (unsigned k = 0; k < WPT; ++k) {
        cnt[k] = __popc(s_bits[tid * WPT + k]);
        mine_n += cnt[k];
    }
    unsigned incl = mine_n;
#pragma unroll
    for (int off = 1; off < 64; off <<= 1) {
        const unsigned v = __shfl_up(incl, off, 64);
        if ((int)lane >= off) incl += v;
    }
    if (lane == 63) s_part[wv] = incl;
    __syncthreads();
    unsigned before = 0, total = 0;
    for (unsigned w = 0; w < SEL_NT / 64; ++w) {
        const unsigned v = s_part[w];
        if (w < wv) before += v;
        total += v;
    }
    unsigned run = before + incl - mine_n;
#pragma unroll
    for (unsigned k = 0; k < WPT; ++k) {
        s_pref[tid * WPT + k] = run;
        run += cnt[k];
    }
    __syncthreads();
    for (unsigned long long m = surv; m;) {
        unsigned cs[U2];
        Candidate cds[U2];
        int nb = 0;
#pragma unroll
        for (int u = 0; u < U2; ++u) {
            cs[u] = 0xffffffffu;
            if (m) {
                cs[u] = cand_of((unsigned)(__ffsll((long long)m) - 1));
                m &= m - 1ull;
                cds[u] = cand[cs[u]];
                ++nb;
            }
        }
#pragma unroll
        for (int u = 0; u < U2; ++u) {
            if (cs[u] == 0xffffffffu) continue;
            const Candidate cd = cds[u];
            const unsigned org = s_word[cs[u]];
            const unsigned at = s_pref[org >> 5] + __popc(s_bits[org >> 5] & ((1u << (org & 31u)) - 1u));
            const unsigned l = cd.level, w = s_w[l];
            const unsigned ly = cd.idx / w, lx = cd.idx - ly * w;
            const float ratio = s_ratio[l];
            sel::KpRec rec;
            rec.level = l;
            (void)sel::refine(lx, ly, cd.v, cd.xp, cd.xm, cd.yp, cd.ym, ratio, &rec);
            KpParam p;
            p.xf = rec.x / ratio;
            p.yf = rec.y / ratio;
            p.scale = roundf(0.5f * s_size[l] / ratio);
            p.level = l;
            p.img = img;
            p._pad[0] = p._pad[1] = p._pad[2] = 0u;
            out.recs[img0 + at].rec = rec;
            out.pars[img0 + at] = p;
        }
        (void)nb;
    }
    if (tid == 0) {
        out.hdr[img * 16 + 0] = total; out.hdr[img * 16 + 1] = s_extrema; out.hdr[img * 16 + 2] = 0u; out.hdr[img * 16 + 3] = s_looks;
        out.hdr[img * 16 + 4] = (unsigned)(t1 - t0); out.hdr[img * 16 + 5] = (unsigned)(t2 - t1); out.hdr[img * 16 + 6] = (unsigned)(t3 - t2);
        out.hdr[img * 16 + 7] = (unsigned)(wall_clock64() - t3);
        sel_header_extras(out, img, img_flags[img]);
        if (out.total) *out.total = total;
    }
}

__global__ void __launch_bounds__(256) k_sel_pack(const unsigned* __restrict__ offs, unsigned n_levels, unsigned n_images,
                                                  const unsigned* __restrict__ hdr, const SelKp* __restrict__ recs_in,
                                                  const KpParam* __restrict__ pars_in, SelKp* __restrict__ recs, KpParam* __restrict__ pars,
                                                  unsigned* __restrict__ total) {
    __shared__ unsigned s_red[256];
    const unsigned img = blockIdx.x, tid = threadIdx.x;
    unsigned part = 0;
    for (unsigned j = tid; j < img; j += 256) part += hdr[j * 16];
    s_red[tid] = part;
    __syncthreads();
    for (int off = 128; off > 0; off >>= 1) {
        if ((int)tid < off) s_red[tid] += s_red[tid + off];
        __syncthreads();
    }
    const unsigned base = s_red[0], cnt = hdr[img * 16], img0 = offs[(size_t)img * (n_levels + 1)];
    for (unsigned i = blockIdx.y * 256 + tid; i < cnt; i += gridDim.y * 256) {
        recs[base + i].rec = recs_in[img0 + i].rec;
        pars[base + i] = pars_in[img0 + i];
    }
    if (img + 1 == n_images && blockIdx.y == 0 && tid == 0) *total = base + cnt;
}

}

namespace launch {

static size_t up256(size_t b) { return (b + 255) / 256 * 256; }
static uint32_t rows_per_image(const uint32_t* level_h, uint32_t n_levels) {
    uint32_t r = 0;
    for (uint32_t l = 0; l < n_levels; ++l) r += level_h[l] + 1;
    return r;
}
size_t candidate_relations_bytes(uint32_t cap, const uint32_t* level_h, uint32_t n_levels, uint32_t n_images) {
    return up256((size_t)n_images * (n_levels + 1) * 4) + up256((size_t)n_images * 4) + up256((size_t)cap * (kRel1 + kRel2) * sizeof(uint16_t)) +
           up256(((size_t)n_images * rows_per_image(level_h, n_levels) + 1) * 4) + 256;
}
static void fill_levels(RelLevels& lv, const float* size, const float* ratio, const uint32_t* level_w, const uint32_t* level_h, uint32_t n_levels,
                        uint32_t n_images) {
    std::memset(&lv, 0, sizeof(lv));
    uint32_t base = 0;
    for (uint32_t l = 0; l < n_levels && l < (uint32_t)kMaxLevels; ++l) {
        lv.size[l] = size[l];
        lv.ratio[l] = ratio[l];
        lv.w[l] = level_w[l];
        lv.h[l] = level_h[l];
        lv.row_base[l] = base;
        base += level_h[l] + 1;
    }
    lv.row_base[std::min<uint32_t>(n_levels, kMaxLevels)] = base;
    lv.n_levels = n_levels;
    lv.n_images = n_images;
}
struct SelLayout {
    size_t revcnt, rev, rows, state0, hdr, total, recs_tmp, pars_tmp, end;
};
static SelLayout sel_layout(uint32_t cap, uint32_t n_images) {
    SelLayout l;
    size_t at = 0;
    auto take = [&](size_t bytes) { const size_t b = at; at += up256(bytes); return b; };
    l.revcnt = take((size_t)cap * 4);
    l.rev = take((size_t)cap * sel::kRev * 2);
    l.rows = take((size_t)cap * sizeof(SelRow));
    l.state0 = take(cap);
    l.hdr = take((size_t)n_images * 64);
    l.total = take(4);
    l.recs_tmp = take(n_images > 1 ? (size_t)cap * sizeof(SelKp) : 0);
    l.pars_tmp = take(n_images > 1 ? (size_t)cap * sizeof(KpParam) : 0);
    l.end = at;
    return l;
}
size_t select_device_bytes(uint32_t cap, uint32_t n_images) { return sel_layout(cap, n_images).end + 256; }
uint32_t* select_device_revcnt(void* sel_scratch, uint32_t cap, uint32_t n_images) {
    return (uint32_t*)((char*)sel_scratch + sel_layout(cap, n_images).revcnt);
}
void select_device(hipStream_t s, const Candidate* d_sorted, uint32_t cap, const uint32_t* d_count, const float* size, const float* ratio,
                   const uint32_t* level_w, const uint32_t* level_h, uint32_t n_levels, uint32_t n_images, const void* rel_scratch,
                   void* sel_scratch, const double* d_k, void* d_recs, KpParam* d_pars, uint32_t** d_hdr_out, uint32_t** d_total_out) {
    const SelLayout l = sel_layout(cap, n_images);
    char* p = (char*)sel_scratch;
    const size_t offs_b = up256((size_t)n_images * (n_levels + 1) * 4), flags_b = up256((size_t)n_images * 4);
    const unsigned* offs = (const unsigned*)rel_scratch;
    unsigned* flags = (unsigned*)((char*)rel_scratch + offs_b);
    const unsigned short* rel = (const unsigned short*)((const char*)rel_scratch + offs_b + flags_b);
    const unsigned* row_table = (const unsigned*)((const char*)rel_scratch + offs_b + flags_b + up256((size_t)cap * (kRel1 + kRel2) * sizeof(uint16_t)));
    RelLevels lv;
    fill_levels(lv, size, ratio, level_w, level_h, n_levels, n_images);
    hipLaunchKernelGGL(k_sel_prepare, dim3((cap + 255) / 256), dim3(256), 0, s, d_sorted, d_count, cap, n_levels, n_images, offs, rel,
                       (const unsigned*)(p + l.revcnt), (const unsigned short*)(p + l.rev), (SelRow*)(p + l.rows),
                       (unsigned char*)(p + l.state0), flags);
    SelOut out;
    out.hdr = (unsigned*)(p + l.hdr);
    unsigned* total = (unsigned*)(p + l.total);
    const bool one = n_images == 1;
    out.recs = one ? (SelKp*)d_recs : (SelKp*)(p + l.recs_tmp);
    out.d_count = d_count;
    out.d_k = d_k;
    out.pars = one ? d_pars : (KpParam*)(p + l.pars_tmp);
    out.total = one ? total : nullptr;
    hipLaunchKernelGGL(k_select, dim3(n_images), dim3(SEL_NT), 0, s, d_sorted, lv, offs, (const SelRow*)(p + l.rows),
                       (const unsigned char*)(p + l.state0), (const unsigned*)flags, row_table, out);
    if (!one)
        hipLaunchKernelGGL(k_sel_pack, dim3(n_images, 4), dim3(256), 0, s, offs, n_levels, n_images, (const unsigned*)out.hdr,
                           (const SelKp*)out.recs, (const KpParam*)out.pars, (SelKp*)d_recs, d_pars, total);
    *d_hdr_out = out.hdr;
    *d_total_out = total;
}
void candidate_relations(hipStream_t s, const Candidate* d_sorted, uint32_t cap, const uint32_t* d_count, const float* size, const float* ratio,
                         const uint32_t* level_w, const uint32_t* level_h, uint32_t n_levels, uint32_t n_images, void* scratch,
                         uint16_t** d_rel_out, uint32_t** d_flags_out, void* sel_scratch, bool tables_ready) {
    const size_t offs_b = up256((size_t)n_images * (n_levels + 1) * 4), flags_b = up256((size_t)n_images * 4),
                 rel_b = up256((size_t)cap * (kRel1 + kRel2) * sizeof(uint16_t));
    unsigned* offs = (unsigned*)scratch;
    unsigned* flags = (unsigned*)((char*)scratch + offs_b);
    unsigned short* rel = (unsigned short*)((char*)scratch + offs_b + flags_b);
    unsigned* rows = (unsigned*)((char*)scratch + offs_b + flags_b + rel_b);
    *d_rel_out = rel;
    *d_flags_out = flags;
    RelLevels lv;
    fill_levels(lv, size, ratio, level_w, level_h, n_levels, n_images);
    const unsigned no = n_images * (n_levels + 1) + n_images * lv.row_base[std::min<uint32_t>(n_levels, kMaxLevels)];
    if (!tables_ready)
        hipLaunchKernelGGL(k_rel_offsets, dim3((no + 255) / 256), dim3(256), 0, s, d_sorted, d_count, cap, lv, offs, rows, flags);
    unsigned* revcnt = nullptr;
    unsigned short* rev = nullptr;
    if (sel_scratch) {
        const SelLayout l = sel_layout(cap, n_images);
        revcnt = (unsigned*)((char*)sel_scratch + l.revcnt);
        rev = (unsigned short*)((char*)sel_scratch + l.rev);
    }
    hipLaunchKernelGGL(k_relations, dim3((cap + REL_WAVES - 1) / REL_WAVES), dim3(64 * REL_WAVES), 0, s, d_sorted, d_count, cap, lv, offs, rows, rel, flags,
                       revcnt, rev);
}

static size_t sort_temp(uint32_t cap, unsigned end_bit) {
    size_t bytes = 0;
    (void)rocprim::radix_sort_pairs(nullptr, bytes, (unsigned long long*)nullptr, (unsigned long long*)nullptr, (unsigned*)nullptr,
                                    (unsigned*)nullptr, cap, 0, end_bit, nullptr);
    return bytes;
}
static KeyBits key_bits(uint64_t max_px, uint32_t n_levels, uint32_t n_images) {
    KeyBits kb;
    kb.idx_bits = bits_for(max_px);
    kb.level_bits = bits_for(n_levels);
    kb.total = kb.idx_bits + kb.level_bits + bits_for((unsigned long long)n_images + 1);
    return kb;
}
uint32_t sort_small_capacity() { return SORT_SMALL_N; }
bool sort_candidates_rows(hipStream_t s, const Candidate* d_cand, uint32_t cap, const uint32_t* d_count, const uint32_t* level_w,
                          const uint32_t* level_h, uint32_t n_levels, Candidate* d_sorted, uint32_t* d_zero, void* rel_scratch) {
    if (cap > SORT_SMALL_N || n_levels == 0 || n_levels > (uint32_t)kMaxLevels || rows_per_image(level_h, n_levels) > SORT_SMALL_ROWS) return false;
    RelLevels lv;
    std::vector<float> none(n_levels, 0.0f);
    fill_levels(lv, none.data(), none.data(), level_w, level_h, n_levels, 1);
    unsigned *offs = nullptr, *rows = nullptr, *flags = nullptr;
    if (rel_scratch) {
        const size_t offs_b = up256((size_t)(n_levels + 1) * 4), flags_b = up256(4), rel_b = up256((size_t)cap * (kRel1 + kRel2) * sizeof(uint16_t));
        offs = (unsigned*)rel_scratch;
        flags = (unsigned*)((char*)rel_scratch + offs_b);
        rows = (unsigned*)((char*)rel_scratch + offs_b + flags_b + rel_b);
    }
    hipLaunchKernelGGL(k_sort_rows, dim3(1), dim3(1024), 0, s, d_cand, cap, d_count, lv, d_sorted, d_zero, offs, rows, flags);
    return true;
}
size_t sort_candidates_buckets_scratch(uint32_t cap) {
    return up256((size_t)(SORT_BUCKETS_MAX + 1) * 4) * 2 + up256((size_t)cap * 4) * 3 + 256;
}
size_t sort_candidates_buckets_counters() { return up256((size_t)(SORT_BUCKETS_MAX + 1) * 4); }
bool sort_candidates_buckets(hipStream_t s, const Candidate* d_cand, uint32_t cap, const uint32_t* d_count, const uint32_t* level_w,
                             const uint32_t* level_h, uint32_t n_levels, uint32_t n_images, void* scratch, size_t* counters_zero,
                             Candidate* d_sorted, uint32_t* d_zero, void* rel_scratch) {
    if (n_levels == 0 || n_levels > (uint32_t)kMaxLevels || cap == 0) return false;
    const uint64_t nb64 = (uint64_t)n_images * rows_per_image(level_h, n_levels);
    if (nb64 > SORT_BUCKETS_MAX) return false;
    const unsigned nb = (unsigned)nb64;
    RelLevels lv;
    std::vector<float> none(n_levels, 0.0f);
    fill_levels(lv, none.data(), none.data(), level_w, level_h, n_levels, n_images);
    char* p = (char*)scratch;
    const size_t cb = up256((size_t)(SORT_BUCKETS_MAX + 1) * 4), lb = up256((size_t)cap * 4);
    unsigned* cnt = (unsigned*)p;
    unsigned* start = (unsigned*)(p + cb);
    unsigned* bucket_of = (unsigned*)(p + 2 * cb);
    unsigned* slot_of = (unsigned*)(p + 2 * cb + lb);
    unsigned* row_keys = (unsigned*)(p + 2 * cb + 2 * lb);
    const bool known_zero = *counters_zero >= cb;
    *counters_zero = 0;
    if (!known_zero && hipMemsetAsync(cnt, 0, cb, s) != hipSuccess) return false;
    unsigned *offs = nullptr, *flags = nullptr;
    if (rel_scratch) {
        const size_t offs_b = up256((size_t)n_images * (n_levels + 1) * 4), flags_b = up256((size_t)n_images * 4),
                     rel_b = up256((size_t)cap * (kRel1 + kRel2) * sizeof(uint16_t));
        offs = (unsigned*)rel_scratch;
        flags = (unsigned*)((char*)rel_scratch + offs_b);
        start = (unsigned*)((char*)rel_scratch + offs_b + flags_b + rel_b);
    }
    const unsigned gb = (cap + 255) / 256;
    hipLaunchKernelGGL(k_bucket_count, dim3(gb), dim3(256), 0, s, d_cand, cap, d_count, lv, cnt, bucket_of, slot_of);
    hipLaunchKernelGGL(k_bucket_scan, dim3(1), dim3(1024), 0, s, cnt, nb, start, d_count, cap, lv, offs, flags);
    hipLaunchKernelGGL(k_bucket_place, dim3(gb), dim3(256), 0, s, d_cand, cap, d_count, (const unsigned*)start, (const unsigned*)bucket_of,
                       (const unsigned*)slot_of, row_keys);
    hipLaunchKernelGGL(k_bucket_rank, dim3(gb), dim3(256), 0, s, d_cand, cap, d_count, (const unsigned*)start, (const unsigned*)bucket_of,
                       (const unsigned*)row_keys, d_sorted, d_zero);
    if (hipPeekAtLastError() == hipSuccess) *counters_zero = cb;
    return true;
}
size_t sort_candidates_scratch(uint32_t cap, uint64_t max_px, uint32_t n_levels, uint32_t n_images) {
    const KeyBits kb = key_bits(max_px, n_levels, n_images);
    const size_t a = ((size_t)cap * 8 + 255) / 256 * 256, b = ((size_t)cap * 4 + 255) / 256 * 256;
    return 2 * a + 2 * b + sort_temp(cap, kb.total) + 256;
}
bool sort_candidates_device(hipStream_t s, const Candidate* d_cand, uint32_t cap, const uint32_t* d_count, uint64_t max_px,
                            uint32_t n_levels, uint32_t n_images, void* scratch, Candidate* d_sorted, uint32_t* d_zero) {
    if (cap == 0) return true;
    const KeyBits kb = key_bits(max_px, n_levels, n_images);
    if (kb.total > 63) return false;
    const size_t a = ((size_t)cap * 8 + 255) / 256 * 256, b = ((size_t)cap * 4 + 255) / 256 * 256;
    char* p = (char*)scratch;
    unsigned long long* k_in = (unsigned long long*)p;
    unsigned long long* k_out = (unsigned long long*)(p + a);
    unsigned* p_in = (unsigned*)(p + 2 * a);
    unsigned* p_out = (unsigned*)(p + 2 * a + b);
    void* tmp = p + 2 * a + 2 * b;
    size_t tmp_bytes = sort_temp(cap, kb.total);
    const unsigned nb = (cap + 255) / 256;
    hipLaunchKernelGGL(k_candidate_keys, dim3(nb), dim3(256), 0, s, d_cand, cap, d_count, kb, k_in, p_in);
    if (rocprim::radix_sort_pairs(tmp, tmp_bytes, k_in, k_out, p_in, p_out, cap, 0, kb.total, s) != hipSuccess) return false;
    hipLaunchKernelGGL(k_candidate_gather, dim3(nb), dim3(256), 0, s, d_cand, cap, d_count, p_out, d_sorted, d_zero);
    return true;
}

}
}
```

Measured before the change: 15390.

## Embed level plane pointers in KpParam and restructure orientation kernel sampling

```diff
diff --git a/akaze-rust_amd/csrc/akz_extract.hpp b/akaze-rust_amd/csrc/akz_extract.hpp
--- a/akaze-rust_amd/csrc/akz_extract.hpp
+++ b/akaze-rust_amd/csrc/akz_extract.hpp
@@ -73,9 +73,22 @@
         tab.lv[l] = {r->planes[l][AKZ_LT], r->planes[l][AKZ_LX], r->planes[l][AKZ_LY], r->plan[l].w, r->plan[l].h, (uint64_t)r->plan[l].w * r->plan[l].h};
     return tab;
 }
-inline KpParam kp_param(float x, float y, float size, uint32_t octave, uint32_t level, uint32_t img) {
+inline KpParam kp_param(const LevelTable& tab, float x, float y, float size, uint32_t octave, uint32_t level, uint32_t img) {
     const float ratio = (float)(1u << octave);
-    return KpParam{x / ratio, y / ratio, std::round(0.5f * size / ratio), level, img, {0, 0, 0}};
+    const LevelPtrs& lv = tab.lv[level];
+    const uint64_t off = (uint64_t)img * lv.stride;
+    KpParam p{};
+    p.xf = x / ratio;
+    p.yf = y / ratio;
+    p.scale = std::round(0.5f * size / ratio);
+    p.level = level;
+    p.w = lv.w;
+    p.h = lv.h;
+    p.img = img;
+    p.lx = lv.lx + off;
+    p.ly = lv.ly + off;
+    p.lt = lv.lt + off;
+    return p;
 }
 
 inline size_t align_up(size_t v, size_t a) { return (v + a - 1) / a * a; }
diff --git a/akaze-rust_amd/csrc/akz_extract_finish.cpp b/akaze-rust_amd/csrc/akz_extract_finish.cpp
--- a/akaze-rust_amd/csrc/akz_extract_finish.cpp
+++ b/akaze-rust_amd/csrc/akz_extract_finish.cpp
@@ -192,7 +192,7 @@
         mir = launch::MldbMirror{c->pin[PIN_LIST].p, f.d_sel_hdr, c->pin[PIN_SEL_HDR].p, f.n * 64u, f.host_rows() ? (uint8_t*)c->pin[PIN_ROWS].p : nullptr};
         f.mirrored = true;
     }
-    launch::mldb_counted(f.s, f.tab, (const KpParam*)c->kp_in.p, f.d_sel_total, 0, f.mldb_spec, &((SelKpHost*)c->sel_recs.p)->sums, 2,
+    launch::mldb_counted(f.s, (const KpParam*)c->kp_in.p, f.d_sel_total, 0, f.mldb_spec, &((SelKpHost*)c->sel_recs.p)->sums, 2,
                          f.libm_dev == 1, nullptr, (uint32_t)r->cfg.descriptor_channels, r->d_desc64, f.mirrored ? &mir : nullptr);
     AKZ_HIP_TRY(hipGetLastError());
     return AKZ_OK;
@@ -248,9 +248,9 @@
     AKZ_TRY(ensure(c, c->sel_recs, (size_t)cap * sizeof(SelKpHost)));
     AKZ_TRY(ensure(c, c->kp_in, (size_t)cap * sizeof(KpParam)));
     launch::select_device(s, d_sorted, cap, f.d_count, f.lsize.data(), f.lratio.data(), lw.data(), lh.data(), L, n, c->rel_scratch.p, selp,
-                          r->d_k, c->sel_recs.p, (KpParam*)c->kp_in.p, &f.d_sel_hdr, &f.d_sel_total);
+                          r->d_k, f.tab, c->sel_recs.p, (KpParam*)c->kp_in.p, &f.d_sel_hdr, &f.d_sel_total);
     AKZ_TRY(hold_behind_next_fed(c, f.job, s));
-    launch::orientation_counted(s, f.tab, (const KpParam*)c->kp_in.p, f.d_sel_total, cap, f.wmask, f.nwin, &((SelKpHost*)c->sel_recs.p)->sums, 2);
+    launch::orientation_counted(s, (const KpParam*)c->kp_in.p, f.d_sel_total, cap, f.wmask, f.nwin, &((SelKpHost*)c->sel_recs.p)->sums, 2);
     AKZ_HIP_TRY(hipGetLastError());
     f.dev_sel = true;
     return enqueue_device_descriptors(f);
@@ -279,7 +279,7 @@
         c->sel_skip_shape = f.shape;
     }
     if (f.dev_sel && f.libm_dev && f.total_kp > f.mldb_spec) {
-        launch::mldb_counted(s, f.tab, (const KpParam*)c->kp_in.p, f.d_sel_total, f.mldb_spec, (uint32_t)f.total_kp, &((SelKpHost*)c->sel_recs.p)->sums, 2,
+        launch::mldb_counted(s, (const KpParam*)c->kp_in.p, f.d_sel_total, f.mldb_spec, (uint32_t)f.total_kp, &((SelKpHost*)c->sel_recs.p)->sums, 2,
                              f.libm_dev == 1, nullptr, (uint32_t)r->cfg.descriptor_channels, r->d_desc64);
         AKZ_HIP_TRY(hipGetLastError());
     }
@@ -530,7 +530,7 @@
         OrientOut* d_oo = (OrientOut*)c->kp_out.p;
         AKZ_HIP_TRY(hipMemcpyAsync(d_kp, params, total_kp * sizeof(KpParam), hipMemcpyHostToDevice, s));
         AKZ_TRY(hold_behind_next_fed(c, f.job, s));
-        launch::orientation(s, f.tab, d_kp, (uint32_t)total_kp, f.wmask, f.nwin, d_oo);
+        launch::orientation(s, d_kp, (uint32_t)total_kp, f.wmask, f.nwin, d_oo);
         AKZ_HIP_TRY(hipGetLastError());
         oo = (OrientOut*)c->pin[PIN_COUNT_SUMS].p;
         AKZ_HIP_TRY(hipMemcpyAsync(oo, d_oo, total_kp * sizeof(OrientOut), hipMemcpyDeviceToHost, s));
@@ -565,7 +565,7 @@
         AKZ_TRY(slab_acquire(c, total_kp * 64, &blk, &r->desc_block_bytes));
         r->d_desc64 = (uint8_t*)blk;
     }
-    launch::mldb(s, f.tab, d_kp, (const float*)c->cosi.p, (uint32_t)total_kp, (uint32_t)r->cfg.descriptor_channels, r->d_desc64);
+    launch::mldb(s, d_kp, (const float*)c->cosi.p, (uint32_t)total_kp, (uint32_t)r->cfg.descriptor_channels, r->d_desc64);
     AKZ_HIP_TRY(hipGetLastError());
     if (f.host_rows()) {
         AKZ_TRY(ensure_pinned(c, c->pin[PIN_ROWS], total_kp * 64));
@@ -589,7 +589,7 @@
         c->pool().run(f.n, [&](size_t img) {
             for (size_t i = 0; i < f.hk[img].size(); ++i) {
                 const HostKeypoint& k = f.hk[img][i];
-                params[r->desc_off[img] + i] = kp_param(k.x, k.y, k.size, k.octave, k.class_id, (uint32_t)img);
+                params[r->desc_off[img] + i] = kp_param(f.tab, k.x, k.y, k.size, k.octave, k.class_id, (uint32_t)img);
             }
         });
     }
diff --git a/akaze-rust_amd/csrc/akz_internal.hpp b/akaze-rust_amd/csrc/akz_internal.hpp
--- a/akaze-rust_amd/csrc/akz_internal.hpp
+++ b/akaze-rust_amd/csrc/akz_internal.hpp
@@ -108,13 +108,19 @@
     float v, xp, xm, yp, ym;
     uint32_t img;
 };
-struct KpParam {
+struct alignas(64) KpParam {
     float xf, yf;
     float scale;
     uint32_t level;
+    uint32_t w, h;
     uint32_t img;
-    uint32_t _pad[3];
-};
+    uint32_t _pad0;
+    const float* lx;
+    const float* ly;
+    const float* lt;
+    uint64_t _pad1;
+};
+static_assert(sizeof(KpParam) == 64, "one 64-byte line per keypoint");
 struct OrientOut {
     float sum_x, sum_y;
     uint32_t found;
@@ -270,18 +276,17 @@
 uint32_t* select_device_revcnt(void* sel_scratch, uint32_t cap, uint32_t n_images);
 void select_device(hipStream_t s, const Candidate* d_sorted, uint32_t cap, const uint32_t* d_count, const float* size, const float* ratio,
                    const uint32_t* level_w, const uint32_t* level_h, uint32_t n_levels, uint32_t n_images, const void* rel_scratch,
-                   void* sel_scratch, const double* d_k, void* d_recs, KpParam* d_pars, uint32_t** d_hdr_out, uint32_t** d_total_out);
+                   void* sel_scratch, const double* d_k, const LevelTable& planes, void* d_recs, KpParam* d_pars, uint32_t** d_hdr_out,
+                   uint32_t** d_total_out);
 void nms(hipStream_t s, const float* ldet, uint32_t w, uint32_t h, uint32_t n, uint64_t img_stride, uint32_t level,
          float thr, float border_m, Candidate* d_cand, uint32_t cap, uint32_t* d_count);
 void mask_candidates(hipStream_t s, const Candidate* d_in, Candidate* d_out, uint32_t cap, uint32_t* d_cnt, const uint8_t* d_mask,
                      uint64_t row_pitch, uint64_t frame_stride, const uint32_t* level_w, const uint32_t* level_h,
                      const uint32_t* level_octave, uint32_t n_levels, uint32_t n_images);
-void orientation(hipStream_t s, const LevelTable& lt, const KpParam* d_kp, uint32_t nkp,
-                 unsigned long long window_mask, uint32_t n_windows, OrientOut* d_out);
-void orientation_counted(hipStream_t s, const LevelTable& lt, const KpParam* d_kp, const uint32_t* d_nkp, uint32_t max_kp,
-                         unsigned long long window_mask, uint32_t n_windows, OrientOut* d_out, uint32_t out_stride);
-void mldb(hipStream_t s, const LevelTable& lt, const KpParam* d_kp, const float* d_cosi, uint32_t nkp,
-          uint32_t channels, uint8_t* d_desc64);
+void orientation(hipStream_t s, const KpParam* d_kp, uint32_t nkp, unsigned long long window_mask, uint32_t n_windows, OrientOut* d_out);
+void orientation_counted(hipStream_t s, const KpParam* d_kp, const uint32_t* d_nkp, uint32_t max_kp, unsigned long long window_mask,
+                         uint32_t n_windows, OrientOut* d_out, uint32_t out_stride);
+void mldb(hipStream_t s, const KpParam* d_kp, const float* d_cosi, uint32_t nkp, uint32_t channels, uint8_t* d_desc64);
 struct MldbMirror {
     void* host_recs;
     const void* d_hdr;
@@ -289,7 +294,7 @@
     uint32_t hdr_bytes;
     uint8_t* host_desc;
 };
-void mldb_counted(hipStream_t s, const LevelTable& lt, const KpParam* d_kp, const uint32_t* d_nkp, uint32_t first, uint32_t last, OrientOut* d_sums,
+void mldb_counted(hipStream_t s, const KpParam* d_kp, const uint32_t* d_nkp, uint32_t first, uint32_t last, OrientOut* d_sums,
                   uint32_t sums_stride, bool libm_fma, uint32_t* d_flag, uint32_t channels, uint8_t* d_desc64, const MldbMirror* mirror = nullptr);
 void libm_eval(hipStream_t s, const float* a, const float* b, float* out3, uint64_t n, bool fma, uint32_t* d_flag);
 uint32_t match_num_chunks(uint32_t n0, uint32_t n1);
diff --git a/akaze-rust_amd/csrc/akz_kernels.hip b/akaze-rust_amd/csrc/akz_kernels.hip
--- a/akaze-rust_amd/csrc/akz_kernels.hip
+++ b/akaze-rust_amd/csrc/akz_kernels.hip
@@ -645,14 +645,17 @@
     }
 }
 
-__constant__ float c_gauss25[7][7] = {
+struct Gauss25 {
+    float v[7][7];
+};
+constexpr Gauss25 kGauss25 = {{
     {0.02546481f, 0.02350698f, 0.01849125f, 0.01239505f, 0.00708017f, 0.00344629f, 0.00142946f},
     {0.02350698f, 0.02169968f, 0.01706957f, 0.01144208f, 0.00653582f, 0.00318132f, 0.00131956f},
     {0.01849125f, 0.01706957f, 0.01342740f, 0.00900066f, 0.00514126f, 0.00250252f, 0.00103800f},
     {0.01239505f, 0.01144208f, 0.00900066f, 0.00603332f, 0.00344629f, 0.00167749f, 0.00069579f},
     {0.00708017f, 0.00653582f, 0.00514126f, 0.00344629f, 0.00196855f, 0.00095820f, 0.00039744f},
     {0.00344629f, 0.00318132f, 0.00250252f, 0.00167749f, 0.00095820f, 0.00046640f, 0.00019346f},
-    {0.00142946f, 0.00131956f, 0.00103800f, 0.00069579f, 0.00039744f, 0.00019346f, 0.00008024f}};
+    {0.00142946f, 0.00131956f, 0.00103800f, 0.00069579f, 0.00039744f, 0.00019346f, 0.00008024f}}};
 
 struct OriTable {
     signed char a[112], b[112];
@@ -670,89 +673,102 @@
     for (; idx < 112; ++idx) { t.a[idx] = 0; t.b[idx] = 0; }
     return t;
 }
-__constant__ OriTable c_ori = make_ori_table();
-struct OriOrder {
-    unsigned char k[112];
+constexpr int ORI_KPB = 32, ORI_NS = 109, ORI_NT = 256;
+constexpr int ORI_LPK = 8, ORI_SPL = 14, ORI_ROWS = ORI_LPK * ORI_SPL;
+constexpr int ORI_LROW = 2 * ORI_KPB + 2;
+static_assert(ORI_KPB * ORI_LPK == ORI_NT && ORI_ROWS >= ORI_NS, "eight lanes per keypoint cover its samples");
+struct alignas(16) OriPlan {
+    unsigned short ab[ORI_LPK][16];
+    float wgt[ORI_LPK][16];
+    unsigned char row[ORI_ROWS];
 };
-constexpr OriOrder make_ori_order() {
-    OriOrder o{};
+constexpr OriPlan make_ori_plan() {
+    OriPlan p{};
     const OriTable t = make_ori_table();
     int n = 0;
     for (int b = -6; b <= 6; ++b)
         for (int a = -6; a <= 6; ++a)
-            for (int k = 0; k < 109; ++k)
-                if (t.a[k] == a && t.b[k] == b) o.k[n++] = (unsigned char)k;
-    for (; n < 112; ++n) o.k[n] = 0;
-    return o;
-}
-__constant__ OriOrder c_ori_rows = make_ori_order();
+            for (int k = 0; k < ORI_NS; ++k)
+                if (t.a[k] == a && t.b[k] == b) {
+                    p.ab[n % ORI_LPK][n / ORI_LPK] = (unsigned short)(((unsigned)a & 0xffu) | (((unsigned)b & 0xffu) << 8));
+                    p.row[k] = (unsigned char)n;
+                    p.wgt[n % ORI_LPK][n / ORI_LPK] = kGauss25.v[a < 0 ? -a : a][b < 0 ? -b : b];
+                    ++n;
+                }
+    return p;
+}
+__constant__ const OriPlan c_ori_plan = make_ori_plan();
 
 __device__ __forceinline__ unsigned xcd_contiguous_group(unsigned b, unsigned nb) {
     return (b & 7u) * (nb >> 3) + (b >> 3);
 }
 
-constexpr int ORI_KPB = 32, ORI_NS = 109, ORI_NT = 256;
+typedef const float __attribute__((address_space(1)))* GlobalF32;
+__device__ __forceinline__ GlobalF32 as_global(const float* p) { return (GlobalF32)p; }
+
 __global__ void __launch_bounds__(ORI_NT)
-k_orientation(LevelTable tab, const KpParam* __restrict__ kps, unsigned nkp, const unsigned* __restrict__ d_nkp,
-              unsigned long long window_mask, unsigned n_windows, OrientOut* __restrict__ out, unsigned out_stride) {
-    __shared__ float s_rx[ORI_KPB * ORI_NS];
-    __shared__ float s_ry[ORI_KPB * ORI_NS + 16];
+k_orientation(const KpParam* __restrict__ kps, unsigned nkp, const unsigned* __restrict__ d_nkp, unsigned long long window_mask,
+              unsigned n_windows, OrientOut* __restrict__ out, unsigned out_stride) {
+    __shared__ float s_t[ORI_NS * ORI_LROW];
     if (d_nkp) nkp = min(nkp, *d_nkp);
     const unsigned base = xcd_contiguous_group(blockIdx.x, gridDim.x) * ORI_KPB;
     if (base >= nkp) return;
-    constexpr int ORI_IT = (ORI_KPB * ORI_NS + ORI_NT - 1) / ORI_NT, ORI_UB = 7;
-    static_assert(ORI_IT % ORI_UB == 0, "whole batches");
-    for (int it0 = 0; it0 < ORI_IT; it0 += ORI_UB) {
-        float vx[ORI_UB], vy[ORI_UB], gw[ORI_UB];
-        unsigned slot[ORI_UB];
-#pragma unroll
-        for (int u = 0; u < ORI_UB; ++u) {
-            const unsigned idx = threadIdx.x + (unsigned)(it0 + u) * ORI_NT;
-            const unsigned j = idx / ORI_NS, k = c_ori_rows.k[idx - j * ORI_NS];
-            vx[u] = 0.0f; vy[u] = 0.0f; gw[u] = 0.0f;
-            slot[u] = j * ORI_NS + k;
-            if (idx < ORI_KPB * ORI_NS && base + j < nkp) {
-                const KpParam kp = kps[base + j];
-                const LevelPtrs lv = tab.lv[kp.level];
-                const float* lx = lv.lx + (size_t)kp.img * lv.stride;
-                const float* ly = lv.ly + (size_t)kp.img * lv.stride;
-                const int a = c_ori.a[k], b = c_ori.b[k];
-                const float fy = roundf(kp.yf + (float)b * kp.scale);
-                const float fx = roundf(kp.xf + (float)a * kp.scale);
-                const int iy = clampi(fy > 0.0f ? (int)fy : 0, 0, (int)lv.h - 1);
-                const int ix = clampi(fx > 0.0f ? (int)fx : 0, 0, (int)lv.w - 1);
-                gw[u] = c_gauss25[a < 0 ? -a : a][b < 0 ? -b : b];
-                const size_t p = (size_t)iy * lv.w + ix;
-                vx[u] = lx[p];
-                vy[u] = ly[p];
-            }
-        }
-#pragma unroll
-        for (int u = 0; u < ORI_UB; ++u) {
-            const unsigned idx = threadIdx.x + (unsigned)(it0 + u) * ORI_NT;
-            const unsigned j = idx / ORI_NS;
-            if (idx < ORI_KPB * ORI_NS) {
-                const bool have = base + j < nkp;
-                s_rx[slot[u]] = have ? gw[u] * vx[u] : 0.0f;
-                s_ry[slot[u]] = have ? gw[u] * vy[u] : 0.0f;
-            }
-        }
+    const unsigned j = threadIdx.x / ORI_LPK, l = threadIdx.x % ORI_LPK, kpi = base + j;
+    if (kpi < nkp) {
+    const KpParam kp = kps[kpi];
+    const GlobalF32 lx = as_global(kp.lx), ly = as_global(kp.ly);
+    const uint4* abv = reinterpret_cast<const uint4*>(c_ori_plan.ab[l]);
+    const uint4 ab0 = abv[0], ab1 = abv[1];
+    const unsigned ab[8] = {ab0.x, ab0.y, ab0.z, ab0.w, ab1.x, ab1.y, ab1.z, ab1.w};
+    __builtin_amdgcn_sched_barrier(0);
+    float2 v[ORI_SPL];
+#pragma unroll
+    for (int s = 0; s < ORI_SPL; ++s) {
+        const unsigned e = (ab[s >> 1] >> (16 * (s & 1))) & 0xffffu;
+        const int a = (int)(signed char)(e & 0xffu), b = (int)(signed char)(e >> 8);
+        const float fy = roundf(kp.yf + (float)b * kp.scale);
+        const float fx = roundf(kp.xf + (float)a * kp.scale);
+        const int iy = clampi(fy > 0.0f ? (int)fy : 0, 0, (int)kp.h - 1);
+        const int ix = clampi(fx > 0.0f ? (int)fx : 0, 0, (int)kp.w - 1);
+        const unsigned p = (unsigned)iy * kp.w + (unsigned)ix;
+        v[s].x = lx[p];
+        v[s].y = ly[p];
+        __builtin_amdgcn_sched_barrier(0);
+    }
+    const float* wgt = c_ori_plan.wgt[l];
+    float* dst = s_t + l * ORI_LROW + 2 * j;
+#pragma unroll
+    for (int s = 0; s < ORI_SPL; ++s) {
+        const float gw = wgt[s], rx = gw * v[s].x, ry = gw * v[s].y;
+        const bool taken = ry > 0.0f;
+        if (s * ORI_LPK + (int)l < ORI_NS) *reinterpret_cast<float2*>(dst + s * ORI_LPK * ORI_LROW) = float2{taken ? rx : -0.0f, taken ? ry : -0.0f};
+    }
     }
     __syncthreads();
     if (threadIdx.x >= 64) return;
-    const unsigned lane = threadIdx.x, j = lane >> 1;
+    const unsigned lane = threadIdx.x, jj = lane >> 1;
     const bool is_y = (lane & 1u) != 0;
-    const float* py = s_ry + j * ORI_NS;
-    const float* pa = is_y ? py : s_rx + j * ORI_NS;
-    float t[ORI_NS];
-#pragma unroll
-    for (int k = 0; k < ORI_NS; ++k) t[k] = py[k] > 0.0f ? pa[k] : -0.0f;
+    const float* src = s_t + lane;
     float sum = 0.0f, maxv = 0.0f, bx = 0.0f, by = 0.0f;
     unsigned found = 0;
     for (unsigned wdw = 0; wdw < n_windows; ++wdw) {
+        __asm__ volatile("" ::: "memory");
         if ((window_mask >> wdw) & 1ull) {
-#pragma unroll
-            for (int k = 0; k < ORI_NS; ++k) sum = sum + t[k];
+            constexpr int CH = 16, NCH = (ORI_NS + CH - 1) / CH;
+            float buf[2][CH];
+#pragma unroll
+            for (int i = 0; i < CH; ++i) buf[0][i] = src[c_ori_plan.row[i] * ORI_LROW];
+#pragma unroll
+            for (int c = 0; c < NCH; ++c) {
+                __builtin_amdgcn_sched_barrier(0);
+#pragma unroll
+                for (int i = 0; i < CH; ++i)
+                    if ((c + 1) * CH + i < ORI_NS) buf[(c + 1) & 1][i] = src[c_ori_plan.row[(c + 1) * CH + i] * ORI_LROW];
+                __builtin_amdgcn_sched_barrier(0);
+#pragma unroll
+                for (int i = 0; i < CH; ++i)
+                    if (c * CH + i < ORI_NS) sum = sum + buf[c & 1][i];
+            }
         }
         const float other = __shfl_xor(sum, 1, 64);
         const float sx = is_y ? other : sum, sy = is_y ? sum : other;
@@ -764,10 +780,10 @@
             found = 1;
         }
     }
-    if (!is_y && base + j < nkp) {
+    if (!is_y && base + jj < nkp) {
         OrientOut o;
         o.sum_x = bx; o.sum_y = by; o.found = found; o.angle_bits = 0;
-        out[(size_t)(base + j) * out_stride] = o;
+        out[(size_t)(base + jj) * out_stride] = o;
     }
 }
 
@@ -837,39 +853,37 @@
         if (bad && da.flag) atomicOr(da.flag, 1u);
         if (hm.recs) {
             const uint4* rec = reinterpret_cast<const uint4*>(da.sums) + (size_t)kpi * 2u - 1u;
-            uint4 r0 = rec[0], r1 = rec[1];
-            r1.w = __float_as_uint(ang);
+            const uint4 r0 = rec[0], r1 = rec[1];
             hm.recs[(size_t)kpi * 2u] = r0;
-            hm.recs[(size_t)kpi * 2u + 1u] = r1;
+            hm.recs[(size_t)kpi * 2u + 1u] = make_uint4(r1.x, r1.y, r1.z, __float_as_uint(ang));
         }
     }
     return float2{co, si};
 }
+__device__ __forceinline__ void wave_lds_sync() {
+    __builtin_amdgcn_fence(__ATOMIC_RELEASE, "wavefront");
+    __builtin_amdgcn_wave_barrier();
+    __builtin_amdgcn_fence(__ATOMIC_ACQUIRE, "wavefront");
+}
 __global__ void __launch_bounds__(64 * MLDB_KPB)
-k_mldb(LevelTable tab, const KpParam* __restrict__ kps, const float2* __restrict__ cosi, unsigned nkp, const unsigned* __restrict__ d_nkp,
+k_mldb(const KpParam* __restrict__ kps, const float2* __restrict__ cosi, unsigned nkp, const unsigned* __restrict__ d_nkp,
        DeviceAngles da, unsigned channels, uint8_t* __restrict__ desc64, unsigned first, MldbHostMirror hm) {
     __shared__ float s_win[MLDB_KPB][3][MLDB_NS + 7];
     __shared__ float s_val[MLDB_KPB][3][32];
     if (hm.recs && blockIdx.x == 0)
         for (unsigned i = threadIdx.x; i < hm.hdr_vec; i += 64 * MLDB_KPB) hm.hdr_host[i] = hm.hdr[i];
     if (d_nkp) nkp = min(nkp, *d_nkp);
-    const unsigned lane = threadIdx.x & 63u, wv = threadIdx.x >> 6;
-    const unsigned group0 = first + xcd_contiguous_group(blockIdx.x, gridDim.x) * MLDB_KPB;
-    const unsigned kpi = group0 + wv;
-    if (group0 >= nkp) return;
-    const bool live = kpi < nkp;
-    KpParam kp = kps[live ? kpi : 0];
-    const float2 cs = da.sums ? device_angle(da, live ? kpi : 0, live && lane == 0, hm) : cosi[live ? kpi : 0];
-    const LevelPtrs lv = tab.lv[__builtin_amdgcn_readfirstlane(kp.level)];
-    const size_t ioff = (size_t)kp.img * lv.stride;
-    const float* Lt = lv.lt + ioff;
-    const float* Lx = lv.lx + ioff;
-    const float* Ly = lv.ly + ioff;
+    const unsigned lane = threadIdx.x & 63u, wv = __builtin_amdgcn_readfirstlane(threadIdx.x >> 6);
+    const unsigned kpi = first + xcd_contiguous_group(blockIdx.x, gridDim.x) * MLDB_KPB + wv;
+    if (kpi >= nkp) return;
+    const KpParam kp = kps[kpi];
+    const float2 cs = da.sums ? device_angle(da, kpi, lane == 0, hm) : cosi[kpi];
+    const GlobalF32 Lt = as_global(kp.lt), Lx = as_global(kp.lx), Ly = as_global(kp.ly);
     const float co = cs.x, si = cs.y, scale = kp.scale;
     unsigned short bits3[8];
 #pragma unroll
     for (int r = 0; r < 8; ++r) bits3[r] = c_bits3.e[r * 64 + (int)lane];
-    if (live) {
+    {
         constexpr int NIT = (MLDB_NS + 63) / 64;
         const bool k_fast = fabsf(co) >= fabsf(si);
         unsigned pidx[NIT];
@@ -883,9 +897,9 @@
             const float lf = (float)l + 0.5f, kf = (float)k + 0.5f;
             const float sample_y = kp.yf + (lf * co * scale + kf * si * scale);
             const float sample_x = kp.xf + (-lf * si * scale + kf * co * scale);
-            const int y1 = clampi((int)roundf(sample_y), 0, (int)lv.h - 1);
-            const int x1 = clampi((int)roundf(sample_x), 0, (int)lv.w - 1);
-            pidx[it] = (unsigned)y1 * (unsigned)lv.w + (unsigned)x1;
+            const int y1 = clampi((int)roundf(sample_y), 0, (int)kp.h - 1);
+            const int x1 = clampi((int)roundf(sample_x), 0, (int)kp.w - 1);
+            pidx[it] = (unsigned)y1 * kp.w + (unsigned)x1;
             widx[it] = kk * MLDB_LAT + ll;
         }
         float vt[NIT], vx[NIT], vy[NIT];
@@ -914,9 +928,9 @@
             s_win[wv][2][widx[it]] = v2;
         }
     }
-    __syncthreads();
-    const unsigned cl = lane & 31u, ckp = 2u * wv + (lane >> 5);
-    if (wv < MLDB_KPB / 2 && cl < 29 && group0 + ckp < nkp) {
+    wave_lds_sync();
+    const unsigned cl = lane, ckp = wv;
+    if (cl < 29) {
         const int g = cl < 4 ? 0 : (cl < 13 ? 1 : 2);
         const int step = g == 0 ? 10 : (g == 1 ? 7 : 5), ng = g + 2;
         const int ci = (int)cl - (g == 0 ? 0 : (g == 1 ? 4 : 13));
@@ -949,7 +963,7 @@
         s_val[ckp][1][cl] = dx / ns;
         s_val[ckp][2][cl] = dy / ns;
     }
-    __syncthreads();
+    wave_lds_sync();
     const unsigned seg0 = 6u * channels, seg1 = seg0 + 36u * channels, total = seg1 + 120u * channels;
     unsigned long long words[8];
 #pragma unroll
@@ -969,7 +983,7 @@
         }
         words[r] = __ballot(bit);
     }
-    if (live && lane < 8) {
+    if (lane < 8) {
         unsigned long long wvw = words[0];
 #pragma unroll
         for (int r = 1; r < 8; ++r)
@@ -1316,30 +1330,28 @@
     hipLaunchKernelGGL(k_nms, grid2d((w + 3) / 4, h, n), dim3(BX, BY), 0, s, ldet_p, (int)w, (int)h, (size_t)img_stride,
                        level, thr, border_m, d_cand, cap, d_count);
 }
-void orientation(hipStream_t s, const LevelTable& lt, const KpParam* d_kp, uint32_t nkp,
-                 unsigned long long window_mask, uint32_t n_windows, OrientOut* d_out) {
+void orientation(hipStream_t s, const KpParam* d_kp, uint32_t nkp, unsigned long long window_mask, uint32_t n_windows, OrientOut* d_out) {
     if (nkp == 0) return;
     const uint32_t groups = (nkp + ORI_KPB - 1) / ORI_KPB;
-    hipLaunchKernelGGL(k_orientation, dim3((groups + 7u) / 8u * 8u), dim3(ORI_NT), 0, s, lt, d_kp, nkp, (const unsigned*)nullptr,
-                       window_mask, n_windows, d_out, 1u);
-}
-void orientation_counted(hipStream_t s, const LevelTable& lt, const KpParam* d_kp, const uint32_t* d_nkp, uint32_t max_kp,
-                         unsigned long long window_mask, uint32_t n_windows, OrientOut* d_out, uint32_t out_stride) {
+    hipLaunchKernelGGL(k_orientation, dim3((groups + 7u) / 8u * 8u), dim3(ORI_NT), 0, s, d_kp, nkp, (const unsigned*)nullptr, window_mask, n_windows,
+                       d_out, 1u);
+}
+void orientation_counted(hipStream_t s, const KpParam* d_kp, const uint32_t* d_nkp, uint32_t max_kp, unsigned long long window_mask,
+                         uint32_t n_windows, OrientOut* d_out, uint32_t out_stride) {
     if (max_kp == 0) return;
     const uint32_t groups = (max_kp + ORI_KPB - 1) / ORI_KPB;
-    hipLaunchKernelGGL(k_orientation, dim3((groups + 7u) / 8u * 8u), dim3(ORI_NT), 0, s, lt, d_kp, max_kp, d_nkp, window_mask, n_windows,
-                       d_out, out_stride);
-}
-
-void mldb(hipStream_t s, const LevelTable& lt, const KpParam* d_kp, const float* d_cosi, uint32_t nkp,
-          uint32_t channels, uint8_t* d_desc64) {
+    hipLaunchKernelGGL(k_orientation, dim3((groups + 7u) / 8u * 8u), dim3(ORI_NT), 0, s, d_kp, max_kp, d_nkp, window_mask, n_windows, d_out,
+                       out_stride);
+}
+
+void mldb(hipStream_t s, const KpParam* d_kp, const float* d_cosi, uint32_t nkp, uint32_t channels, uint8_t* d_desc64) {
     if (nkp == 0) return;
     const uint32_t groups = (nkp + MLDB_KPB - 1) / MLDB_KPB;
-    hipLaunchKernelGGL(k_mldb, dim3((groups + 7u) / 8u * 8u), dim3(64 * MLDB_KPB), 0, s, lt, d_kp,
-                       reinterpret_cast<const float2*>(d_cosi), nkp, (const unsigned*)nullptr, DeviceAngles{nullptr, 0u, 0u, nullptr}, channels,
-                       d_desc64, 0u, MldbHostMirror{nullptr, nullptr, nullptr, 0u, nullptr});
-}
-void mldb_counted(hipStream_t s, const LevelTable& lt, const KpParam* d_kp, const uint32_t* d_nkp, uint32_t first, uint32_t last, OrientOut* d_sums,
+    hipLaunchKernelGGL(k_mldb, dim3((groups + 7u) / 8u * 8u), dim3(64 * MLDB_KPB), 0, s, d_kp, reinterpret_cast<const float2*>(d_cosi), nkp,
+                       (const unsigned*)nullptr, DeviceAngles{nullptr, 0u, 0u, nullptr}, channels, d_desc64, 0u,
+                       MldbHostMirror{nullptr, nullptr, nullptr, 0u, nullptr});
+}
+void mldb_counted(hipStream_t s, const KpParam* d_kp, const uint32_t* d_nkp, uint32_t first, uint32_t last, OrientOut* d_sums,
                   uint32_t sums_stride, bool libm_fma, uint32_t* d_flag, uint32_t channels, uint8_t* d_desc64, const MldbMirror* mirror) {
     first = first / MLDB_KPB * MLDB_KPB;
     MldbHostMirror hm{nullptr, nullptr, nullptr, 0u, nullptr};
@@ -1347,7 +1359,7 @@
         hm = MldbHostMirror{(uint4*)mirror->host_recs, (const uint4*)mirror->d_hdr, (uint4*)mirror->host_hdr, mirror->hdr_bytes / 16u, mirror->host_desc};
     if (last <= first && !hm.recs) return;
     const uint32_t groups = last > first ? (last - first + MLDB_KPB - 1) / MLDB_KPB : 1u;
-    hipLaunchKernelGGL(k_mldb, dim3((groups + 7u) / 8u * 8u), dim3(64 * MLDB_KPB), 0, s, lt, d_kp, (const float2*)nullptr, last, d_nkp,
+    hipLaunchKernelGGL(k_mldb, dim3((groups + 7u) / 8u * 8u), dim3(64 * MLDB_KPB), 0, s, d_kp, (const float2*)nullptr, last, d_nkp,
                        DeviceAngles{d_sums, sums_stride, libm_fma ? 1u : 0u, d_flag}, channels, d_desc64, first, hm);
 }
 void libm_eval(hipStream_t s, const float* a, const float* b, float* out3, uint64_t n, bool fma, uint32_t* d_flag) {
diff --git a/akaze-rust_amd/csrc/akz_result.cpp b/akaze-rust_amd/csrc/akz_result.cpp
--- a/akaze-rust_amd/csrc/akz_result.cpp
+++ b/akaze-rust_amd/csrc/akz_result.cpp
@@ -203,8 +203,8 @@
             set_error("akz_result_describe_keypoints: keypoint class_id / octave out of range");
             return AKZ_ERR_INVALID_ARG;
         }
-        params[i] = kp_param(k.x, k.y, k.size, k.octave, (uint32_t)k.class_id, (uint32_t)img);
-        if (own_octave) params[n_kp + i] = kp_param(k.x, k.y, k.size, r->plan[(size_t)k.class_id].octave, (uint32_t)k.class_id, (uint32_t)img);
+        params[i] = kp_param(tab, k.x, k.y, k.size, k.octave, (uint32_t)k.class_id, (uint32_t)img);
+        if (own_octave) params[n_kp + i] = kp_param(tab, k.x, k.y, k.size, r->plan[(size_t)k.class_id].octave, (uint32_t)k.class_id, (uint32_t)img);
     }
     AKZ_TRY(ensure(c, c->kp_in, n_par * sizeof(KpParam)));
     AKZ_TRY(ensure(c, c->kp_out, n_kp * sizeof(OrientOut)));
@@ -217,7 +217,7 @@
         uint32_t nwin = 0;
         orientation_windows(&wmask, &nwin);
         OrientOut* d_oo = (OrientOut*)c->kp_out.p;
-        launch::orientation(s, tab, own_octave ? d_kp + n_kp : d_kp, (uint32_t)n_kp, wmask, nwin, d_oo);
+        launch::orientation(s, own_octave ? d_kp + n_kp : d_kp, (uint32_t)n_kp, wmask, nwin, d_oo);
         AKZ_HIP_TRY(hipGetLastError());
         OrientOut* oo = (OrientOut*)c->pin[PIN_COUNT_SUMS].p;
         AKZ_HIP_TRY(hipMemcpyAsync(oo, d_oo, n_kp * sizeof(OrientOut), hipMemcpyDeviceToHost, s));
@@ -234,7 +234,7 @@
     AKZ_HIP_TRY(hipMemcpyAsync(c->cosi.p, cosi, n_kp * 2 * sizeof(float), hipMemcpyHostToDevice, s));
     AKZ_TRY(ensure(c, c->match_a, n_kp * 64));
     uint8_t* d_rows = (uint8_t*)c->match_a.p;
-    launch::mldb(s, tab, d_kp, (const float*)c->cosi.p, (uint32_t)n_kp, (uint32_t)r->cfg.descriptor_channels, d_rows);
+    launch::mldb(s, d_kp, (const float*)c->cosi.p, (uint32_t)n_kp, (uint32_t)r->cfg.descriptor_channels, d_rows);
     AKZ_HIP_TRY(hipGetLastError());
     AKZ_TRY(ensure_pinned(c, c->pin[PIN_ROWS], n_kp * 64));
     uint8_t* rows = (uint8_t*)c->pin[PIN_ROWS].p;
diff --git a/akaze-rust_amd/csrc/akz_sort.hip b/akaze-rust_amd/csrc/akz_sort.hip
--- a/akaze-rust_amd/csrc/akz_sort.hip
+++ b/akaze-rust_amd/csrc/akz_sort.hip
@@ -373,6 +373,9 @@
     OrientOut sums;
 };
 static_assert(sizeof(SelKp) == 32, "akz_api.cpp fetches 32-byte records");
+struct SelPlanes {
+    const float *lx[kMaxLevels], *ly[kMaxLevels], *lt[kMaxLevels];
+};
 struct SelOut {
     unsigned* hdr;
     SelKp* recs;
@@ -407,7 +410,7 @@
 __global__ void __launch_bounds__(SEL_NT) k_select(const Candidate* __restrict__ sorted, RelLevels lv, const unsigned* __restrict__ offs,
                                                    const SelRow* __restrict__ rows, const unsigned char* __restrict__ state0,
                                                    const unsigned* __restrict__ img_flags, const unsigned* __restrict__ row_table,
-                                                   SelOut out) {
+                                                   SelOut out, SelPlanes planes) {
     __shared__ unsigned short s_word[SEL_MAX_CANDS];
     __shared__ unsigned s_bits[SEL_MAX_CANDS / 32];
     __shared__ unsigned s_pref[SEL_MAX_CANDS / 32];
@@ -667,13 +670,21 @@
             sel::KpRec rec;
             rec.level = l;
             (void)sel::refine(lx, ly, cd.v, cd.xp, cd.xm, cd.yp, cd.ym, ratio, &rec);
+            const unsigned ph = lv.h[l];
+            const size_t ioff = (size_t)img * ((size_t)w * ph);
             KpParam p;
             p.xf = rec.x / ratio;
             p.yf = rec.y / ratio;
             p.scale = roundf(0.5f * s_size[l] / ratio);
             p.level = l;
+            p.w = w;
+            p.h = ph;
             p.img = img;
-            p._pad[0] = p._pad[1] = p._pad[2] = 0u;
+            p._pad0 = 0u;
+            p.lx = planes.lx[l] + ioff;
+            p.ly = planes.ly[l] + ioff;
+            p.lt = planes.lt[l] + ioff;
+            p._pad1 = 0ull;
             out.recs[img0 + at].rec = rec;
             out.pars[img0 + at] = p;
         }
@@ -764,7 +775,8 @@
 }
 void select_device(hipStream_t s, const Candidate* d_sorted, uint32_t cap, const uint32_t* d_count, const float* size, const float* ratio,
                    const uint32_t* level_w, const uint32_t* level_h, uint32_t n_levels, uint32_t n_images, const void* rel_scratch,
-                   void* sel_scratch, const double* d_k, void* d_recs, KpParam* d_pars, uint32_t** d_hdr_out, uint32_t** d_total_out) {
+                   void* sel_scratch, const double* d_k, const LevelTable& planes, void* d_recs, KpParam* d_pars, uint32_t** d_hdr_out,
+                   uint32_t** d_total_out) {
     const SelLayout l = sel_layout(cap, n_images);
     char* p = (char*)sel_scratch;
     const size_t offs_b = up256((size_t)n_images * (n_levels + 1) * 4), flags_b = up256((size_t)n_images * 4);
@@ -786,8 +798,14 @@
     out.d_k = d_k;
     out.pars = one ? d_pars : (KpParam*)(p + l.pars_tmp);
     out.total = one ? total : nullptr;
+    SelPlanes sp;
+    for (int l = 0; l < kMaxLevels; ++l) {
+        sp.lx[l] = planes.lv[l].lx;
+        sp.ly[l] = planes.lv[l].ly;
+        sp.lt[l] = planes.lv[l].lt;
+    }
     hipLaunchKernelGGL(k_select, dim3(n_images), dim3(SEL_NT), 0, s, d_sorted, lv, offs, (const SelRow*)(p + l.rows),
-                       (const unsigned char*)(p + l.state0), (const unsigned*)flags, row_table, out);
+                       (const unsigned char*)(p + l.state0), (const unsigned*)flags, row_table, out, sp);
     if (!one)
         hipLaunchKernelGGL(k_sel_pack, dim3(n_images, 4), dim3(256), 0, s, offs, n_levels, n_images, (const unsigned*)out.hdr,
                            (const SelKp*)out.recs, (const KpParam*)out.pars, (SelKp*)d_recs, d_pars, total);
```

Result: no change. 15460, median of 6 (+0.4%).
